# cvangysel/SERT

Hardware: AMD Instinct MI355X
Metric: training_pairs_per_sec (higher is better)
Workload: dtype f32; 1 GPU; C2 LSE: VectorSpaceLanguageModel (NCE z=10, Adam) V_w=100000 V_e=1000 d=128 window=10 batch=65536; global_batch=65536, per_gpu_batch=65536, parallelism=dp1, id_dtype=uint32, seed=0, instance_weights=1, dataset_instances=4194304, dataset_batches=64

## Files before the change

### include/sert_hip_debug.h

```cpp
#ifndef SERT_HIP_DEBUG_H
#define SERT_HIP_DEBUG_H

#include "sert_hip.h"

#ifdef __cplusplus
extern "C" {
#endif

int sert_debug_update_counts(sert_model* m, int64_t* out, int n);

int sert_debug_tail_counts(sert_model* m, int64_t* out, int n);

int sert_debug_poison_scratch(sert_model* m);

int sert_debug_row_lists(const uint32_t* allbits, int world, int rank, int64_t num_batches, int64_t bit_words,
                         int64_t rows_per_rank, int64_t vocab, int64_t batch, int32_t* serve_cnt,
                         int32_t* fetch_cnt, int32_t* serve_rows, int32_t* fetch_rows, int32_t* union_rows,
                         int32_t* ptr, int32_t* ent, int64_t capacity, int64_t* sizes);

int sert_debug_word_index_sum(const void* ids, int id_bytes, int64_t num_batches, int B, int n, int vocab, int row_groups,
                              int dense_heavy, int64_t batch, const float* src, int d, float divisor, float* grad_out,
                              int64_t* stats);

int sert_debug_ll_rank_distributions(int device, const float* P, const int64_t* offsets, int64_t num_queries, int32_t V,
                                     int32_t k, int32_t* idx_out, float* score_out, float* joint_entropy_out,
                                     float* token_entropy_out, int32_t* status_out);

int sert_bench_gemm(int device, int ta, int tb, int epi, int M, int N, int K, int splits,
                    int iters, double* avg_us);

int sert_debug_gemm(int device, int ta, int tb, int epi, int M, int N, int K, const float* A, const float* B,
                    const float* bias, float* C);

int sert_debug_gemm_splitk(int device, int M, int N, int K, int splits, const float* A, const float* B, float* out);

int sert_debug_gemm_longk(int device, int tb, int M, int N, int K, int splits, const float* A, const float* B, float* C);

enum { SERT_MEMBENCH_COPY = 0, SERT_MEMBENCH_READ = 1, SERT_MEMBENCH_GATHER = 2, SERT_MEMBENCH_OPTIMIZER = 3 };
int sert_bench_memory(int device, int kind, size_t bytes, size_t table_bytes, int row_bytes,
                      int window, size_t gap_bytes, int blocks, int iters, double* avg_us);

struct sert_reval;
int sert_debug_reval_chunks(struct sert_reval* r);

#ifdef __cplusplus
}
#endif
#endif
```

### sert_amd/_capi.py

```python
import ctypes
import os

import numpy as np

_HERE = os.path.dirname(os.path.abspath(__file__))
LIB_PATH = os.environ.get('SERT_LIB') or os.path.join(_HERE, 'libsert_hip.so')

KIND_LOGLINEAR, KIND_VECTORSPACE, KIND_VECTORSPACE_SOFTMAX = 0, 1, 2
SPLIT_TRAIN, SPLIT_VALIDATE = 0, 1
LL_STATUS_DEVICE, LL_STATUS_HOST = 0, 1
REVAL_NDCG, REVAL_MAP, REVAL_RECIP_RANK, REVAL_P5, REVAL_NUM_REL_RET, REVAL_NUM_METRICS = 0, 1, 2, 3, 4, 5

T_RW, T_RE, T_W, T_B = 0, 1, 2, 3
T_STATE0_RW, T_STATE0_RE, T_STATE0_W, T_STATE0_B = 4, 5, 6, 7
T_STATE1_RW, T_STATE1_RE, T_STATE1_W, T_STATE1_B = 8, 9, 10, 11
T_GRAD_RW, T_GRAD_RE, T_GRAD_W, T_GRAD_B = 12, 13, 14, 15
T_ACT_H, T_ACT_T, T_ACT_DA, T_ACT_DH, T_ACT_ROWLOSS = 16, 17, 18, 19, 20

COMM_ID_BYTES = 128

EXPORTS = [
    'sert_create', 'sert_destroy', 'sert_last_error', 'sert_device_info', 'sert_device_count',
    'sert_set_tensor', 'sert_get_tensor', 'sert_tensor_size', 'sert_set_step', 'sert_get_step',
    'sert_set_eval_draws', 'sert_get_eval_draws', 'sert_negatives_of_step',
    'sert_upload_dataset', 'sert_train_batch', 'sert_hint_next_batch', 'sert_train_batches',
    'sert_eval_batch', 'sert_eval_batches',
    'sert_predict_project', 'sert_predict_tokens', 'sert_ll_rank_queries', 'sert_score_topk',
    'sert_reval_create', 'sert_reval_run', 'sert_reval_destroy',
    'sert_scorer_create', 'sert_scorer_destroy', 'sert_scorer_topk', 'sert_scorer_scores',
    'sert_host_alloc', 'sert_host_free',
    'sert_comm_unique_id', 'sert_comm_init', 'sert_comm_init_host', 'sert_comm_destroy', 'sert_comm_stats',
    'sert_synchronize', 'sert_timing_enable', 'sert_timing_reset', 'sert_timing_count',
    'sert_timing_name', 'sert_timing_avg_us', 'sert_timing_launches', 'sert_bench_gemm', 'sert_debug_gemm', 'sert_debug_gemm_splitk', 'sert_debug_gemm_longk', 'sert_bench_memory', 'sert_debug_row_lists', 'sert_debug_word_index_sum',
    'sert_debug_update_counts', 'sert_debug_tail_counts', 'sert_debug_poison_scratch', 'sert_debug_ll_rank_distributions', 'sert_debug_reval_chunks',
    'sert_profile_range_push', 'sert_profile_range_pop',
]


_F32P, _I64P = ctypes.POINTER(ctypes.c_float), ctypes.POINTER(ctypes.c_int64)
ALLTOALL_FN = ctypes.CFUNCTYPE(ctypes.c_int, ctypes.c_void_p, _F32P, _I64P, _I64P, _F32P, _I64P, _I64P)


class SertConfig(ctypes.Structure):
    _fields_ = [
        ('struct_size', ctypes.c_uint32),
        ('kind', ctypes.c_int32),
        ('batch_size', ctypes.c_int32),
        ('global_batch_size', ctypes.c_int32),
        ('window_size', ctypes.c_int32),
        ('vocab_size', ctypes.c_int32),
        ('num_entities', ctypes.c_int32),
        ('word_dim', ctypes.c_int32),
        ('entity_dim', ctypes.c_int32),
        ('num_negatives', ctypes.c_int32),
        ('id_bytes', ctypes.c_int32),
        ('device', ctypes.c_int32),
        ('keep_grads', ctypes.c_int32),
        ('deterministic', ctypes.c_int32),
        ('inference_only', ctypes.c_int32),
        ('lambda_', ctypes.c_float),
        ('lr', ctypes.c_float),
        ('beta1', ctypes.c_float),
        ('beta2', ctypes.c_float),
        ('eps', ctypes.c_float),
        ('seed', ctypes.c_uint64),
    ]


class SertError(RuntimeError):
    pass


_lib = None


def load():
    global _lib
    if _lib is not None:
        return _lib
    if not os.path.exists(LIB_PATH):
        raise SertError(
            'libsert_hip.so not found at %s; build it with '
            '`python -m sert_amd._build` (hipcc --offload-arch=gfx950). '
            'There is no CPU fallback.' % LIB_PATH)
    lib = ctypes.CDLL(LIB_PATH)
    vp, i32, i64, sz = ctypes.c_void_p, ctypes.c_int32, ctypes.c_int64, ctypes.c_size_t
    fp = ctypes.c_void_p
    lib.sert_create.argtypes = [ctypes.POINTER(SertConfig), ctypes.POINTER(vp)]
    lib.sert_destroy.argtypes = [vp]
    lib.sert_last_error.restype = ctypes.c_char_p
    lib.sert_device_info.argtypes = [ctypes.c_int, ctypes.c_char_p, sz]
    lib.sert_device_count.argtypes = []
    lib.sert_set_tensor.argtypes = [vp, ctypes.c_int, fp, sz]
    lib.sert_get_tensor.argtypes = [vp, ctypes.c_int, fp, sz]
    lib.sert_tensor_size.argtypes = [vp, ctypes.c_int]
    lib.sert_tensor_size.restype = sz
    lib.sert_set_step.argtypes = [vp, i64]
    lib.sert_get_step.argtypes = [vp]
    lib.sert_get_step.restype = i64
    lib.sert_set_eval_draws.argtypes = [vp, i64]
    lib.sert_get_eval_draws.argtypes = [vp]
    lib.sert_get_eval_draws.restype = i64
    lib.sert_negatives_of_step.argtypes = [vp, i64, ctypes.c_int, vp]
    lib.sert_upload_dataset.argtypes = [vp, ctypes.c_int, fp, fp, fp, fp, fp, fp, i64]
    lib.sert_train_batch.argtypes = [vp, i64, fp, ctypes.POINTER(ctypes.c_float)]
    lib.sert_train_batches.argtypes = [vp, fp, i64, fp]
    lib.sert_hint_next_batch.argtypes = [vp, i64]
    lib.sert_eval_batch.argtypes = [vp, ctypes.c_int, i64, fp, ctypes.POINTER(ctypes.c_float)]
    lib.sert_eval_batches.argtypes = [vp, ctypes.c_int, ctypes.c_void_p, i64, ctypes.c_void_p]
    lib.sert_predict_project.argtypes = [vp, fp, i64, fp]
    lib.sert_predict_tokens.argtypes = [vp, fp, i64, fp]
    lib.sert_ll_rank_queries.argtypes = [vp, fp, fp, i64, i32, fp, fp, fp, fp, fp]
    lib.sert_reval_create.argtypes = [vp, fp, fp, i64, fp, fp, fp, fp, fp, i32, ctypes.POINTER(vp)]
    lib.sert_reval_run.argtypes = [vp, fp, fp, fp, fp]
    lib.sert_reval_destroy.argtypes = [vp]
    lib.sert_score_topk.argtypes = [ctypes.c_int, fp, i64, i32, fp, i64, i32, fp, fp]
    lib.sert_scorer_create.argtypes = [ctypes.c_int, fp, i64, i32, ctypes.POINTER(vp)]
    lib.sert_scorer_destroy.argtypes = [vp]
    lib.sert_scorer_topk.argtypes = [vp, fp, i64, i32, fp, fp]
    lib.sert_scorer_scores.argtypes = [vp, fp, i64, fp]
    lib.sert_host_alloc.argtypes = [ctypes.POINTER(vp), sz]
    lib.sert_host_free.argtypes = [vp]
    lib.sert_comm_unique_id.argtypes = [ctypes.c_char_p]
    lib.sert_comm_init.argtypes = [vp, ctypes.c_char_p, ctypes.c_int, ctypes.c_int]
    lib.sert_comm_destroy.argtypes = [vp]
    lib.sert_comm_init_host.argtypes = [vp, ctypes.c_int, ctypes.c_int, ALLTOALL_FN, vp]
    lib.sert_comm_stats.argtypes = [vp, ctypes.POINTER(ctypes.c_double), ctypes.c_int]
    lib.sert_debug_row_lists.argtypes = [fp, ctypes.c_int, ctypes.c_int, i64, i64, i64, i64, i64] + [fp] * 7 + [i64, fp]
    lib.sert_synchronize.argtypes = [vp]
    lib.sert_profile_range_push.argtypes = [ctypes.c_char_p]
    lib.sert_profile_range_pop.argtypes = []
    lib.sert_timing_enable.argtypes = [vp, ctypes.c_int]
    lib.sert_timing_reset.argtypes = [vp]
    lib.sert_timing_count.argtypes = [vp]
    lib.sert_timing_name.argtypes = [vp, ctypes.c_int]
    lib.sert_timing_name.restype = ctypes.c_char_p
    lib.sert_timing_avg_us.argtypes = [vp, ctypes.c_int]
    lib.sert_timing_avg_us.restype = ctypes.c_double
    lib.sert_timing_launches.argtypes = [vp, ctypes.c_int]
    lib.sert_timing_launches.restype = ctypes.c_double
    lib.sert_bench_gemm.argtypes = [ctypes.c_int] * 9 + [ctypes.POINTER(ctypes.c_double)]
    lib.sert_bench_memory.argtypes = [ctypes.c_int, ctypes.c_int, sz, sz, ctypes.c_int, ctypes.c_int, sz, ctypes.c_int,
                                      ctypes.c_int, ctypes.POINTER(ctypes.c_double)]
    _lib = lib
    return lib


def check(rc):
    if rc != 0:
        raise SertError(load().sert_last_error().decode('utf-8', 'replace'))


def _addr(a):
    return None if a is None else a.ctypes.data


def device_count():
    return load().sert_device_count()


def device_info(device=0):
    buf = ctypes.create_string_buffer(512)
    n = load().sert_device_info(device, buf, 512)
    if n < 0:
        raise SertError(load().sert_last_error().decode())
    return buf.value.decode()


def require_gpu():
    n = device_count()
    if n is None or n <= 0:
        raise SertError('no HIP device visible: sert_amd runs on MI355X (gfx950) only; '
                        'there is no CPU fallback.')
    return n


class Engine(object):

    def __init__(self, **cfg):
        lib = load()
        c = SertConfig()
        c.struct_size = ctypes.sizeof(SertConfig)
        for k, v in cfg.items():
            if not hasattr(c, k):
                raise TypeError('unknown sert_config field %r' % k)
            setattr(c, k, v)
        self.cfg = c
# ... 34 lines not shown
        return int(self._lib.sert_get_step(self._h))

    def set_eval_draws(self, n):
        check(self._lib.sert_set_eval_draws(self._h, int(n)))

    def get_eval_draws(self):
        return int(self._lib.sert_get_eval_draws(self._h))

    def negatives_of_step(self, position, evaluation=False):
        out = np.empty((self.cfg.batch_size, self.cfg.num_negatives), dtype=np.int64)
        check(self._lib.sert_negatives_of_step(self._h, int(position), int(bool(evaluation)), out.ctypes.data))
        return out

    def upload_dataset(self, split, x, y_int=None, csr=None, w=None):
        x = np.ascontiguousarray(x)
        n = x.shape[0]
        keep = [x]
        y_addr = ip = ix = da = None
        if y_int is not None:
            y_int = np.ascontiguousarray(y_int, dtype=np.int32)
            keep.append(y_int)
            y_addr = y_int.ctypes.data
        if csr is not None:
            indptr = np.ascontiguousarray(csr.indptr, dtype=np.int64)
            indices = np.ascontiguousarray(csr.indices, dtype=np.int32)
            data = np.ascontiguousarray(csr.data, dtype=np.float32)
            keep += [indptr, indices, data]
            ip, ix, da = indptr.ctypes.data, indices.ctypes.data, data.ctypes.data
        w_addr = None
        if w is not None:
            w = np.ascontiguousarray(w, dtype=np.float32)
            keep.append(w)
            w_addr = w.ctypes.data
        check(self._lib.sert_upload_dataset(self._h, split, x.ctypes.data if n else None,
                                            y_addr, ip, ix, da, w_addr, n))
        del keep

    def train_batch(self, batch_index, negatives=None):
        loss = ctypes.c_float()
        if negatives is not None:
            negatives = np.ascontiguousarray(negatives, dtype=np.int64)
        check(self._lib.sert_train_batch(self._h, int(batch_index), _addr(negatives),
                                         ctypes.byref(loss)))
        return np.float32(loss.value)

    def hint_next_batch(self, next_batch_index):
        check(self._lib.sert_hint_next_batch(
            self._h, -1 if next_batch_index is None else int(next_batch_index)))

    def train_batches(self, batch_indices):
        idx = np.ascontiguousarray(batch_indices, dtype=np.int64)
        out = np.empty(idx.size, dtype=np.float32)
        check(self._lib.sert_train_batches(self._h, idx.ctypes.data, idx.size, out.ctypes.data))
        return out

    def eval_batch(self, split, batch_index, negatives=None):
        loss = ctypes.c_float()
        if negatives is not None:
            negatives = np.ascontiguousarray(negatives, dtype=np.int64)
        check(self._lib.sert_eval_batch(self._h, split, int(batch_index), _addr(negatives),
                                        ctypes.byref(loss)))
        return np.float32(loss.value)

    def eval_batches(self, split, batch_indices):
        idx = np.ascontiguousarray(batch_indices, dtype=np.int64)
        out = np.empty(idx.shape[0], dtype=np.float32)
        if idx.shape[0]:
            check(self._lib.sert_eval_batches(self._h, split, idx.ctypes.data, idx.shape[0], out.ctypes.data))
        return out

    def predict_project(self, avg):
        avg = np.ascontiguousarray(avg, dtype=np.float32)
        q = avg.shape[0]
        out = np.empty((q, self.cfg.entity_dim), dtype=np.float32)
        check(self._lib.sert_predict_project(self._h, avg.ctypes.data, q, out.ctypes.data))
        return out

    def predict_tokens(self, ids):
        ids = np.ascontiguousarray(ids)
        assert ids.dtype.itemsize == self.cfg.id_bytes
        rows = ids.shape[0]
        out = np.empty((rows, self.cfg.window_size, self.cfg.num_entities), dtype=np.float32)
        check(self._lib.sert_predict_tokens(self._h, ids.ctypes.data, rows, out.ctypes.data))
        return out

    def ll_rank_queries(self, token_lists, k=None):
        tokens, offsets = _concat_queries(token_lists)
        return _ll_rank_call(self.cfg.num_entities, offsets, k, lambda kk, outs: self._lib.sert_ll_rank_queries(
            self._h, tokens.ctypes.data, offsets.ctypes.data, offsets.size - 1, kk, *outs), tokens.size)

    def comm_init(self, unique_id, rank, world):
        assert len(unique_id) == COMM_ID_BYTES
        check(self._lib.sert_comm_init(self._h, unique_id, rank, world))

    def comm_init_host(self, rank, world, alltoall):
        def trampoline(_user, send, soff, scnt, recv, roff, rcnt):
            try:
                so = np.ctypeslib.as_array(soff, shape=(world,))
                sc = np.ctypeslib.as_array(scnt, shape=(world,))
                ro = np.ctypeslib.as_array(roff, shape=(world,))
                rc = np.ctypeslib.as_array(rcnt, shape=(world,))
                ns = int((so + sc).max()) if world else 0
                nr = int((ro + rc).max()) if world else 0
                sbuf = np.ctypeslib.as_array(send, shape=(max(ns, 1),))
                rbuf = np.ctypeslib.as_array(recv, shape=(max(nr, 1),))
                alltoall(sbuf, so, sc, rbuf, ro, rc)
                return 0
            except Exception:
                import traceback
                traceback.print_exc()
                return 1
        self._host_alltoall = ALLTOALL_FN(trampoline)
        check(self._lib.sert_comm_init_host(self._h, rank, world, self._host_alltoall, None))

    def comm_stats(self):
        v = (ctypes.c_double * 8)()
        check(self._lib.sert_comm_stats(self._h, v, 8))
        return {'world': int(v[0]), 'exchange': {0: 'none', 1: 'zero1', 2: 'rows'}[int(v[1])],
                'bytes_per_step': float(v[2]), 'zero1_bytes_per_step': float(v[3]),
                'transport': {0: 'none', 1: 'rccl', 2: 'host'}[int(v[4])], 'steps': int(v[5]),
                'rows_fetched_per_batch': float(v[6]), 'rows_served_per_batch': float(v[7])}

    def synchronize(self):
        check(self._lib.sert_synchronize(self._h))

    def timing_enable(self, on=True):
        check(self._lib.sert_timing_enable(self._h, int(on)))

    def timing_launches(self):
        n = self._lib.sert_timing_count(self._h)
        return {self._lib.sert_timing_name(self._h, i).decode():
                self._lib.sert_timing_launches(self._h, i) for i in range(n)}

    def timing_reset(self):
        check(self._lib.sert_timing_reset(self._h))

    def poison_scratch(self):
        self._lib.sert_debug_poison_scratch.argtypes = [ctypes.c_void_p]
        check(self._lib.sert_debug_poison_scratch(self._h))

    def update_counts(self):
        v = (ctypes.c_int64 * 10)()
        self._lib.sert_debug_update_counts.argtypes = [ctypes.c_void_p, ctypes.POINTER(ctypes.c_int64), ctypes.c_int]
        check(self._lib.sert_debug_update_counts(self._h, v, 10))
        names = ('dense', 'lazy', 'skip_32_1', 'skip_64_1', 'skip_32_3', 'skip_64_2', 'skip_64_3', 'skip_64_4', 'skip_full', 'skip_sparse')
        return dict(zip(names, (int(x) for x in v)))

    def tail_counts(self):
        v = (ctypes.c_int64 * 2)()
        self._lib.sert_debug_tail_counts.argtypes = [ctypes.c_void_p, ctypes.POINTER(ctypes.c_int64), ctypes.c_int]
        check(self._lib.sert_debug_tail_counts(self._h, v, 2))
        return {'alone': int(v[0]), 'in_gather': int(v[1])}

    def timings(self):
        n = self._lib.sert_timing_count(self._h)
        return {self._lib.sert_timing_name(self._h, i).decode():
                self._lib.sert_timing_avg_us(self._h, i) for i in range(n)}


def comm_unique_id():
    buf = ctypes.create_string_buffer(COMM_ID_BYTES)
    check(load().sert_comm_unique_id(buf))
    return buf.raw


def _concat_queries(token_lists):
    lengths = np.fromiter((len(t) for t in token_lists), dtype=np.int64, count=len(token_lists))
    offsets = np.zeros(len(token_lists) + 1, dtype=np.int64)
    np.cumsum(lengths, out=offsets[1:])
    tokens = np.ascontiguousarray(np.concatenate([np.asarray(t, dtype=np.int64) for t in token_lists])
                                  if len(token_lists) else np.zeros(0, np.int64), dtype=np.int32)
    return tokens, offsets


def _ll_rank_call(num_entities, offsets, k, call, num_tokens):
    q = offsets.size - 1
    kk = num_entities if k is None or k >= num_entities else int(k)
    idx = np.empty((q, kk), dtype=np.int32)
    score = np.empty((q, kk), dtype=np.float32)
    joint_h = np.empty(q, dtype=np.float32)
    token_h = np.empty(num_tokens, dtype=np.float32)
    status = np.empty(q, dtype=np.int32)
    outs = [a.ctypes.data for a in (idx, score, joint_h, token_h, status)]
    check(call(-1 if k is None else int(k), outs))
    return idx, score, joint_h, token_h, status, offsets


def debug_ll_rank_distributions(distributions, offsets, k=None, device=0):
    lib = load()
    P = np.ascontiguousarray(distributions, dtype=np.float32)
    offsets = np.ascontiguousarray(offsets, dtype=np.int64)
    assert P.ndim == 2 and P.shape[0] == offsets[-1]
    lib.sert_debug_ll_rank_distributions.argtypes = [ctypes.c_int, ctypes.c_void_p, ctypes.c_void_p, ctypes.c_int64,
                                                     ctypes.c_int32, ctypes.c_int32] + [ctypes.c_void_p] * 5
    return _ll_rank_call(P.shape[1], offsets, k, lambda kk, outs: lib.sert_debug_ll_rank_distributions(
        device, P.ctypes.data, offsets.ctypes.data, offsets.size - 1, P.shape[1], kk, *outs), P.shape[0])


def score_topk(entities, projections, k, device=0):
    e = np.ascontiguousarray(entities, dtype=np.float32)
    p = np.ascontiguousarray(projections, dtype=np.float32)
    assert e.ndim == 2 and p.ndim == 2 and e.shape[1] == p.shape[1]
    q = p.shape[0]
    idx = np.empty((q, k), dtype=np.int32)
    val = np.empty((q, k), dtype=np.float32)
    check(load().sert_score_topk(device, e.ctypes.data, e.shape[0], e.shape[1], p.ctypes.data, q,
                                 k, idx.ctypes.data, val.ctypes.data))
    return idx, val


class PinnedBuffer(object):

    def __init__(self, dtype):
        self.dtype = np.dtype(dtype)
        self._ptr = ctypes.c_void_p()
        self._bytes = 0
        self._lib = load()

    def view(self, shape):
        if os.environ.get('SERT_NO_PINNED'):
            return np.empty(shape, dtype=self.dtype)
        need = int(np.prod(shape)) * self.dtype.itemsize
        if need > self._bytes:
            self.free()
            cap = max(need, 1 << 16)
            check(self._lib.sert_host_alloc(ctypes.byref(self._ptr), cap))
            self._bytes = cap
        raw = (ctypes.c_char * max(need, 1)).from_address(self._ptr.value)
        return np.frombuffer(raw, dtype=self.dtype, count=int(np.prod(shape))).reshape(shape)

    def holds(self, array):
        if not self._ptr.value or not isinstance(array, np.ndarray) or not array.flags['C_CONTIGUOUS']:
            return False
        addr = array.ctypes.data
        return self._ptr.value <= addr and addr + array.nbytes <= self._ptr.value + self._bytes

    def free(self):
        if self._ptr.value:
            self._lib.sert_host_free(self._ptr)
            self._ptr = ctypes.c_void_p()
            self._bytes = 0

    def __del__(self):
        try:
            self.free()
        except Exception:
            pass


class Scorer(object):

    MAX_HOST_SCORES = 1 << 26

    def __init__(self, entities, device=0):
        e = np.ascontiguousarray(entities, dtype=np.float32)
        assert e.ndim == 2
        self.num_entities, self.dim = e.shape
        self._lib = load()
        self._h = ctypes.c_void_p()
        check(self._lib.sert_scorer_create(device, e.ctypes.data, e.shape[0], e.shape[1],
                                           ctypes.byref(self._h)))
        self._pin_q, self._pin_idx, self._pin_val = PinnedBuffer(np.float32), PinnedBuffer(np.int32), PinnedBuffer(np.float32)

    def query_buffer(self, num_queries):
        return self._pin_q.view((num_queries, self.dim))

    def _stage(self, projections):
        p = np.asarray(projections, dtype=np.float32)
        if p.ndim == 1:
            p = p.reshape(1, -1)
        assert p.shape[1] == self.dim
        if self._pin_q.holds(p):
            return p
        staged = self._pin_q.view(p.shape)
        np.copyto(staged, p)
        return staged

    def topk(self, projections, k):
        p = self._stage(projections)
        q = p.shape[0]
        idx = self._pin_idx.view((q, k))
        val = self._pin_val.view((q, k))
        check(self._lib.sert_scorer_topk(self._h, p.ctypes.data, q, k, idx.ctypes.data,
                                         val.ctypes.data))
        return idx, val

    def scores(self, projections):
        p = np.ascontiguousarray(projections, dtype=np.float32)
        if p.ndim == 1:
            p = p.reshape(1, -1)
        assert p.shape[1] == self.dim
        out = np.empty((p.shape[0], self.num_entities), dtype=np.float32)
        check(self._lib.sert_scorer_scores(self._h, p.ctypes.data, p.shape[0], out.ctypes.data))
        return out

    def rank(self, projections, k=None):
        if k is not None and k <= min(self.num_entities, 1024):
            return self.topk(projections, k)
        p = np.asarray(projections, dtype=np.float32)
        if p.ndim == 1:
            p = p.reshape(1, -1)
        keep = self.num_entities if k is None else min(k, self.num_entities)
        step = max(1, self.MAX_HOST_SCORES // self.num_entities)
        idx = np.empty((p.shape[0], keep), dtype=np.int32)
        val = np.empty((p.shape[0], keep), dtype=np.float32)
        for lo in range(0, p.shape[0], step):
# ... 179 lines not shown
```

### sert_amd/csrc/host/api_data_train.inc

```

int sert_upload_dataset(sert_model* m, int split, const void* x, const int32_t* y_int,
                        const int64_t* csr_indptr, const int32_t* csr_indices,
                        const float* csr_data, const float* w, int64_t N) {
    if (!m) SERT_FAIL("null model");
    invalidate_speculation(m);
    m->hint_next = -1;
    if (split != SERT_SPLIT_TRAIN && split != SERT_SPLIT_VALIDATE) SERT_FAIL("bad split");
    if (N < 0) SERT_FAIL("negative instance count");
    if (N > 0 && !x) SERT_FAIL("x is null");
    if (N > 0 && !y_int && !(csr_indptr && csr_indices && csr_data)) SERT_FAIL("no labels given");
    if (is_vs(m) && N > 0 && !y_int) SERT_FAIL("vectorspace requires int labels (models.py:933-934)");
    SERT_HIP(hipSetDevice(m->cfg.device));
    if (N > 0) {
        const size_t toks = (size_t)N * m->cfg.window_size;
        const uint32_t Vw = (uint32_t)m->cfg.vocab_size;
        bool ok = true;
        SERT_ID_DISPATCH(m->cfg.id_bytes, {
            const IdT* xi = (const IdT*)x;
            uint32_t mx = 0;
            for (size_t i = 0; i < toks; ++i) mx = std::max<uint32_t>(mx, (uint32_t)xi[i]);
            ok = mx < Vw;
        });
        if (!ok) SERT_FAIL("token id >= vocab_size in x");
        const int32_t Ve = m->cfg.num_entities;
// ... 10 lines not shown
        }
    }
    DataSplit& d = m->split[split];
    free_split(d);
    d.N = N;
    if (N == 0) return 0;
    hipStream_t s = m->stream;
    const size_t xbytes = (size_t)N * m->cfg.window_size * m->cfg.id_bytes;
    SERT_HIP(hipMalloc(&d.x, xbytes));
    SERT_HIP(hipMemcpyAsync(d.x, x, xbytes, hipMemcpyHostToDevice, s));
    if (y_int) {
        d.max_labels_per_row = 1;
        SERT_TRY(dmalloc(&d.y, (size_t)N));
        SERT_HIP(hipMemcpyAsync(d.y, y_int, N * sizeof(int32_t), hipMemcpyHostToDevice, s));
    } else {
        d.nnz = csr_indptr[N];
        for (int64_t r = 0; r < N; ++r)
            d.max_labels_per_row = std::max<int64_t>(d.max_labels_per_row, csr_indptr[r + 1] - csr_indptr[r]);
        SERT_TRY(dmalloc(&d.csr_indptr, (size_t)N + 1));
        SERT_TRY(dmalloc(&d.csr_indices, (size_t)std::max<int64_t>(1, d.nnz)));
        SERT_TRY(dmalloc(&d.csr_data, (size_t)std::max<int64_t>(1, d.nnz)));
        SERT_HIP(hipMemcpyAsync(d.csr_indptr, csr_indptr, (N + 1) * sizeof(int64_t), hipMemcpyHostToDevice, s));
        if (d.nnz) {
            SERT_HIP(hipMemcpyAsync(d.csr_indices, csr_indices, d.nnz * sizeof(int32_t), hipMemcpyHostToDevice, s));
            SERT_HIP(hipMemcpyAsync(d.csr_data, csr_data, d.nnz * sizeof(float), hipMemcpyHostToDevice, s));
        }
    }
    if (split == SERT_SPLIT_TRAIN) {
        SERT_TRY(dmalloc(&d.w, (size_t)N));
        if (w) {
            SERT_HIP(hipMemcpyAsync(d.w, w, N * sizeof(float), hipMemcpyHostToDevice, s));
        } else {
            std::vector<float> ones((size_t)N, 1.0f);
            SERT_HIP(hipMemcpyAsync(d.w, ones.data(), N * sizeof(float), hipMemcpyHostToDevice, s));
            SERT_HIP(hipStreamSynchronize(s));
        }
    }
    if (split == SERT_SPLIT_TRAIN && !m->cfg.inference_only && !is_vs(m))
        SERT_TRY(dmalloc(&d.labfix, (size_t)std::max<int64_t>(1, y_int ? N : d.nnz)));
    if (split == SERT_SPLIT_TRAIN && !m->cfg.inference_only) {
        const int B = m->cfg.batch_size, n = m->cfg.window_size;
        const int64_t nb = N / B;
        WordIndex wi;
        const bool row_is_pos = !is_vs(m);
        bool vs_heavy = false;
        if (is_vs(m) && m->cfg.word_dim % 4 == 0 && m->cfg.word_dim <= 512) {
            const int d4 = m->cfg.word_dim / 4;
            const bool lpi32 = d4 <= 32 || (d4 > 64 && 64 * cdiv(d4, 64) > 32 * cdiv(d4, 32));
            const bool bundle_on = variant_knob("SERT_SEG_BUNDLE") && atoi(variant_knob("SERT_SEG_BUNDLE")) != 0;
            vs_heavy = knob("SERT_DENSE_HEAVY") ? atoi(knob("SERT_DENSE_HEAVY")) != 0 : (lpi32 && !bundle_on);
        }
        const bool dense_heavy = !variant_knob("SERT_NO_DENSE_HEAVY") && (is_vs(m) ? vs_heavy : (m->cfg.num_entities % 4 == 0));
        int row_groups = 1;
        if (is_vs(m) && m->cfg.word_dim % 4 == 0)
            if (const char* e = variant_knob("SERT_SEG_GROUPS")) row_groups = std::min(std::max(1, atoi(e)), std::max(1, B / 64));
        const bool sort_level0 = is_vs(m) && row_groups == 1 && !(variant_knob("SERT_SEG_BUNDLE") && atoi(variant_knob("SERT_SEG_BUNDLE")) != 0) &&
                                 !variant_knob("SERT_SEG_NO_SORT");
        bool ids_ok = true;
        SERT_ID_DISPATCH(m->cfg.id_bytes,
                         ids_ok = build_word_index<IdT>((const IdT*)x, nb, B, n, m->cfg.vocab_size, row_is_pos, wi,
                                                        !is_vs(m), dense_heavy, row_groups, sort_level0));
        if (!ids_ok) SERT_FAIL("token id >= vocab_size in x");
        if (!is_vs(m) && !wi.slots.empty()) {
            const size_t V = (size_t)m->cfg.num_entities;
            SERT_TRY(dmalloc(&d.idx_uwords, std::max<size_t>(1, wi.uwords.size())));
            SERT_TRY(dmalloc(&d.idx_slots, wi.slots.size()));
            SERT_HIP(hipMemcpyAsync(d.idx_uwords, wi.uwords.data(), wi.uwords.size() * sizeof(int32_t), hipMemcpyHostToDevice, s));
            SERT_HIP(hipMemcpyAsync(d.idx_slots, wi.slots.data(), wi.slots.size() * sizeof(int32_t), hipMemcpyHostToDevice, s));
            SERT_TRY(dmalloc(&d.idx_rows_div, wi.rows_div.size()));
            SERT_HIP(hipMemcpyAsync(d.idx_rows_div, wi.rows_div.data(), wi.rows_div.size() * sizeof(int32_t), hipMemcpyHostToDevice, s));
            SERT_HIP(hipStreamSynchronize(s));
            if ((size_t)wi.max_distinct > m->zu_rows) {
                (void)hipFree(m->Zu); (void)hipFree(m->dZu);
                m->Zu = nullptr; m->dZu = nullptr;
                m->zu_rows = (size_t)wi.max_distinct;
                SERT_TRY(dmalloc(&m->Zu, m->zu_rows * V));
                SERT_TRY(dmalloc(&m->dZu, m->zu_rows * V));
            }
            if ((size_t)wi.max_part_rows + 1 > m->zpart_rows) {
                (void)hipFree(m->zpart);
                m->zpart = nullptr;
                m->zpart_rows = (size_t)wi.max_part_rows + 1;
                SERT_TRY(dmalloc(&m->zpart, m->zpart_rows * V));
            }
        }
        if (!wi.rows.empty()) {
            SERT_TRY(dmalloc(&d.idx_rows, wi.rows.size()));
            SERT_HIP(hipMemcpyAsync(d.idx_rows, wi.rows.data(), wi.rows.size() * sizeof(int32_t), hipMemcpyHostToDevice, s));
            SERT_HIP(hipMalloc((void**)&d.idx_items, std::max<size_t>(1, wi.items.size()) * sizeof(SegItem)));
            SERT_HIP(hipMemcpyAsync(d.idx_items, wi.items.data(), wi.items.size() * sizeof(SegItem), hipMemcpyHostToDevice, s));
            if (!wi.heavy.empty()) {
                SERT_HIP(hipMalloc((void**)&d.idx_heavy, wi.heavy.size() * sizeof(int32_t)));
                SERT_HIP(hipMemcpyAsync(d.idx_heavy, wi.heavy.data(), wi.heavy.size() * sizeof(int32_t), hipMemcpyHostToDevice, s));
            }
            const bool bundle = variant_knob("SERT_SEG_BUNDLE") && atoi(variant_knob("SERT_SEG_BUNDLE")) != 0;
            if (!wi.bundles.empty() && bundle && is_vs(m)) {
                SERT_TRY(dmalloc(&d.idx_bundles, wi.bundles.size()));
                SERT_HIP(hipMemcpyAsync(d.idx_bundles, wi.bundles.data(), wi.bundles.size() * sizeof(int32_t), hipMemcpyHostToDevice, s));
            }
            SERT_HIP(hipStreamSynchronize(s));
        }
        if (!wi.touched_bits.empty()) {
            SERT_TRY(dmalloc(&d.idx_touched_bits, wi.touched_bits.size()));
            SERT_HIP(hipMemcpyAsync(d.idx_touched_bits, wi.touched_bits.data(), wi.touched_bits.size() * sizeof(uint32_t),
                                    hipMemcpyHostToDevice, s));
            SERT_HIP(hipStreamSynchronize(s));
            d.bit_words = wi.bit_words;
        }
        if (is_dp(m)) SERT_TRY(xr_build_lists(m, wi.touched_bits, nb, wi.bit_words));
        if (wi.any_dense) {
            SERT_HIP(hipMalloc((void**)&d.idx_dense_counts, wi.dense_counts.size()));
            SERT_HIP(hipMemcpyAsync(d.idx_dense_counts, wi.dense_counts.data(), wi.dense_counts.size(), hipMemcpyHostToDevice, s));
            std::vector<int32_t> hw((size_t)nb * kHeavyMax, 0);
            for (int64_t b = 0; b < nb; ++b)
                for (int h = 0; h < wi.batches[(size_t)b].dense_cnt; ++h) hw[(size_t)b * kHeavyMax + h] = wi.batches[(size_t)b].dense_word[h];
            if (!wi.dense_tok_slot.empty() && variant_knob("SERT_GATHER_HOT") && atoi(variant_knob("SERT_GATHER_HOT")) != 0) {
                SERT_HIP(hipMalloc((void**)&d.idx_tok_slot, wi.dense_tok_slot.size()));
                SERT_HIP(hipMemcpyAsync(d.idx_tok_slot, wi.dense_tok_slot.data(), wi.dense_tok_slot.size(), hipMemcpyHostToDevice, s));
                d.dense_cnt_of.resize((size_t)nb);
                for (int64_t b = 0; b < nb; ++b) d.dense_cnt_of[(size_t)b] = wi.batches[(size_t)b].dense_cnt;
            }
            SERT_TRY(dmalloc(&d.idx_dense_words, hw.size()));
            SERT_HIP(hipMemcpyAsync(d.idx_dense_words, hw.data(), hw.size() * sizeof(int32_t), hipMemcpyHostToDevice, s));
            SERT_HIP(hipStreamSynchronize(s));
            if (!m->hpart)
                SERT_TRY(dmalloc(&m->hpart, (size_t)std::max(cdiv(B, heavy_rows_fused(B)), cdiv(B, kHeavyRowsPerBlock)) * kHeavyMax *
                                               (size_t)(is_vs(m) ? m->cfg.word_dim : m->cfg.num_entities)));
        } else {
            for (auto& bxx : wi.batches) bxx.dense_cnt = 0;
        }
        d.idx_batches = wi.batches;
        if ((size_t)wi.max_part_rows + 1 > m->wpart_rows) {
            (void)hipFree(m->wpart);
            m->wpart_rows = (size_t)wi.max_part_rows + 1;
            SERT_TRY(dmalloc(&m->wpart, m->wpart_rows * m->cfg.word_dim));
        }
    }
    SERT_HIP(hipStreamSynchronize(s));
    return 0;
}

int sert_train_batch(sert_model* m, int64_t batch_index, const int64_t* negatives, float* loss_out) {
    refresh_gemm_choice();
    if (!m) SERT_FAIL("null model");
    SERT_HIP(hipSetDevice(m->cfg.device));
    static const bool no_spin = variant_knob("SERT_NO_SPIN") != nullptr;
    const int64_t hint = m->hint_next;
    m->hint_next = -1;
    m->lazy_next = hint;
    auto prefetch_next = [&]() -> int {
        const DataSplit& ds = m->split[SERT_SPLIT_TRAIN];
        if (will_run_ahead(m, hint)) {
            bool fused = false;
            SERT_TRY(step_forward_backward(m, ds, hint, nullptr, &fused));
            m->spec_fb_batch = hint;
            m->spec_fb_step = m->step;
            return 0;
        }
        if (hint < 0 || m->timing.enabled || m->cfg.keep_grads) return 0;
        if ((hint + 1) * (int64_t)m->cfg.batch_size > ds.N) return 0;
        if (is_vs(m) && !is_fs(m)) {
            if (m->xr_on) SERT_TRY(xr_fetch_params(m, hint));
            SERT_TRY(vs_project(m, ds, hint));
            m->projected_batch = hint;
        } else if (m->xr_on) {
            SERT_TRY(xr_fetch_params(m, hint));
        }
        return 0;
    };
    if (m->timing.enabled || no_spin) {
        SERT_TRY(train_step_async(m, batch_index, negatives, m->d_loss));
        SERT_HIP(hipMemcpyAsync(m->h_loss, m->d_loss, 3 * sizeof(float), hipMemcpyDeviceToHost, m->stream));
        SERT_HIP(hipEventRecord(m->ev_loss, m->stream));
        SERT_TRY(prefetch_next());
        SERT_HIP(hipEventSynchronize(m->ev_loss));
        timing_collect(m);
        if (loss_out) *loss_out = m->h_loss[0];
        return 0;
    }
    static const bool no_fold = variant_knob("SERT_TAIL_IN_GATHER") && atoi(variant_knob("SERT_TAIL_IN_GATHER")) == 0;
    m->tail_defer = !no_fold && !is_dp(m) && is_vs(m) && !is_fs(m) && will_run_ahead(m, hint);
    int rc = train_step_async(m, batch_index, negatives, m->h_loss_dev, true);
    m->tail_defer = false;
    if (rc == 0) rc = prefetch_next();
    flush_pending_tail(m);
    if (rc != 0) return rc;
    const unsigned want = m->loss_seq;
    volatile unsigned* flag = reinterpret_cast<volatile unsigned*>(m->h_loss + 4);
    {
        const auto t_spin0 = std::chrono::steady_clock::now();
        double next_query_ms = 50.0;
        for (unsigned spins = 1; *flag != want; ++spins) {
            if ((spins & 0xfff) != 0) continue;
            const double waited_ms = std::chrono::duration<double, std::milli>(std::chrono::steady_clock::now() - t_spin0).count();
            if (waited_ms < next_query_ms) continue;
            next_query_ms = waited_ms + 50.0;
            const hipError_t q = hipStreamQuery(m->stream);
            if (q == hipSuccess) {
                if (*flag == want) break;
                SERT_FAIL("training step completed without publishing its loss");
            }
            if (q != hipErrorNotReady) SERT_HIP(q);
        }
    }
    __atomic_thread_fence(__ATOMIC_ACQUIRE);
    if (loss_out) *loss_out = m->h_loss[0];
    return 0;
}

int sert_hint_next_batch(sert_model* m, int64_t next_batch_index) {
    if (!m) SERT_FAIL("null model");
    m->hint_next = next_batch_index;
    return 0;
}

int sert_train_batches(sert_model* m, const int64_t* batch_indices, int64_t count, float* losses_out) {
    refresh_gemm_choice();
    if (!m || !batch_indices || count < 0) SERT_FAIL("bad argument");
    m->hint_next = -1;
    SERT_HIP(hipSetDevice(m->cfg.device));
    if (count == 0) return 0;
    if (m->d_losses_cap < count) {
        (void)hipFree(m->d_losses);
        SERT_TRY(dmalloc(&m->d_losses, (size_t)count * 3));
        m->d_losses_cap = count;
    }
    static const bool report_host = variant_knob("SERT_DEBUG_HOST") != nullptr;
    const auto t_host0 = std::chrono::steady_clock::now();
    for (int64_t i = 0; i < count; ++i) {
        m->lazy_next = i + 1 < count ? batch_indices[i + 1] : -1;
        SERT_TRY(train_step_async(m, batch_indices[i], nullptr, m->d_losses + 3 * i));
        if (m->timing.enabled) {
            SERT_HIP(hipStreamSynchronize(m->stream));
            timing_collect(m);
        }
    }
    if (report_host) {
        const double us = std::chrono::duration<double, std::micro>(std::chrono::steady_clock::now() - t_host0).count();
        fprintf(stderr, "[sert] host enqueue: %.1f us/step over %lld steps\n", us / (double)count, (long long)count);
    }
    std::vector<float> tmp((size_t)count * 3);
    SERT_HIP(hipMemcpyAsync(tmp.data(), m->d_losses, count * 3 * sizeof(float), hipMemcpyDeviceToHost, m->stream));
    SERT_HIP(hipStreamSynchronize(m->stream));
    if (losses_out)
        for (int64_t i = 0; i < count; ++i) losses_out[i] = tmp[3 * i];
    return 0;
}

static int eval_step_async(sert_model* m, const DataSplit& ds, int64_t batch_index, const int64_t* negatives,
                           float* dst) {
    const int B = m->cfg.batch_size;
    SERT_TRY(settle_entity_update(m));
    SERT_TRY(ensure_rw_current(m, -1));
    if (is_fs(m)) {
        SERT_TRY(fs_forward<false>(m, ds, batch_index));
    } else if (is_vs(m)) {
        SERT_TRY(vs_negatives(m, negatives, (uint64_t)(m->eval_draws++) * 2 + 1, m->stream));
        SERT_TRY(vs_project(m, ds, batch_index));
        SERT_TRY(vs_loss<false>(m, ds, batch_index));
    } else {
        SERT_TRY(ll_forward<false>(m, ds, batch_index));
    }
    const int nb = std::min(kOptBlocks, cdiv(B, 256));
    hipLaunchKernelGGL(sum_partial, dim3(nb), dim3(256), 0, m->stream, m->rowloss, (size_t)B, m->red_loss);
    hipLaunchKernelGGL(finalize_loss, dim3(1), dim3(256), 0, m->stream, m->red_loss, nb, m->red_loss, 0,
                       1.0f / (float)B, 0.0f, dst);
    return 0;
}

static int eval_check_args(sert_model* m, int split) {
    if (!m) SERT_FAIL("null model");
    if (split != SERT_SPLIT_TRAIN && split != SERT_SPLIT_VALIDATE) SERT_FAIL("bad split");
    if (m->cfg.inference_only) SERT_FAIL("model was created inference_only");
    return 0;
}

int sert_eval_batch(sert_model* m, int split, int64_t batch_index, const int64_t* negatives, float* loss_out) {
    refresh_gemm_choice();
    SERT_TRY(eval_check_args(m, split));
    invalidate_speculation(m);
    SERT_HIP(hipSetDevice(m->cfg.device));
    SERT_TRY(ensure_full_rw(m));
    const DataSplit& ds = m->split[split];
    const int B = m->cfg.batch_size;
    if (batch_index < 0 || (batch_index + 1) * (int64_t)B > ds.N) SERT_FAIL("batch_index out of range");
    SERT_TRY(eval_step_async(m, ds, batch_index, negatives, m->d_loss));
    SERT_HIP(hipMemcpyAsync(m->h_loss, m->d_loss, 3 * sizeof(float), hipMemcpyDeviceToHost, m->stream));
    SERT_HIP(hipStreamSynchronize(m->stream));
    float v = m->h_loss[0];
    if (is_dp(m)) {
        float* tmp = m->d_loss + 3;
        SERT_HIP(hipMemcpyAsync(tmp, m->d_loss, sizeof(float), hipMemcpyDeviceToDevice, m->stream));
        if (m->host_ar) SERT_TRY(host_allreduce(m, tmp, 1, m->stream));
        else            SERT_NCCL(g_rccl.AllReduce(tmp, tmp, 1, 7, 0, m->comm, m->stream));
        SERT_HIP(hipMemcpyAsync(m->h_loss, tmp, sizeof(float), hipMemcpyDeviceToHost, m->stream));
        SERT_HIP(hipStreamSynchronize(m->stream));
        v = m->h_loss[0] / (float)m->world;
    }
    timing_collect(m);
    if (loss_out) *loss_out = v;
    return 0;
}

int sert_eval_batches(sert_model* m, int split, const int64_t* batch_indices, int64_t count, float* losses_out) {
    refresh_gemm_choice();
    SERT_TRY(eval_check_args(m, split));
    if (!batch_indices || count < 0) SERT_FAIL("bad argument");
// ... 103 lines not shown
```

### sert_amd/csrc/host/api_debug.inc

```

int sert_debug_poison_scratch(sert_model* m) {
    if (!m) SERT_FAIL("null argument");
    if (m->spec_fb_batch >= 0) SERT_FAIL("a run-ahead step is in flight (sert_hint_next_batch): its gradients live in the scratch");
    SERT_HIP(hipSetDevice(m->cfg.device));
    SERT_HIP(hipDeviceSynchronize());
    if (!m->gflat) return 0;
    std::vector<uint32_t> h(m->gflat_alloc, 0x7fc00000u);
    if (m->run_start) {
        const size_t V4 = round_up((size_t)m->cfg.num_entities, 4);
        for (size_t i = 0; i < V4; ++i) { h[m->gflat_count + i] = 0u; h[m->gflat_count + V4 + i] = 1u; }
    }
    SERT_HIP(hipMemcpy(m->gflat, h.data(), h.size() * sizeof(uint32_t), hipMemcpyHostToDevice));
    return 0;
}

int sert_debug_update_counts(sert_model* m, int64_t* out, int n) {
    if (!m || !out || n < 1 || n > 10) SERT_FAIL("bad argument");
    for (int i = 0; i < n; ++i) out[i] = m->upd_counts[i];
    return 0;
}

int sert_debug_tail_counts(sert_model* m, int64_t* out, int n) {
    if (!m || !out || n < 1 || n > 2) SERT_FAIL("bad argument");
    for (int i = 0; i < n; ++i) out[i] = m->tail_counts[i];
    return 0;
}

int sert_debug_row_lists(const uint32_t* allbits, int world, int rank, int64_t num_batches, int64_t bit_words,
                         int64_t rows_per_rank, int64_t vocab, int64_t batch, int32_t* serve_cnt, int32_t* fetch_cnt,
                         int32_t* serve_rows, int32_t* fetch_rows, int32_t* union_rows, int32_t* ptr, int32_t* ent,
                         int64_t capacity, int64_t* sizes) {
    if (!allbits || world < 1 || rank < 0 || rank >= world || batch < 0 || batch >= num_batches || !sizes)
        SERT_FAIL("bad argument");
    RowExchangeLists L;
    build_row_exchange(allbits, world, rank, num_batches, bit_words, rows_per_rank, vocab, L);
    const RowExchangeBatch& xb = L.batches[(size_t)batch];
    sizes[0] = xb.serve_total; sizes[1] = xb.fetch_total; sizes[2] = xb.nunion; sizes[3] = xb.nent; sizes[4] = L.max_xfer_rows;
    if (std::max<int64_t>(std::max(xb.serve_total, xb.fetch_total), std::max(xb.nunion + 1, xb.nent)) > capacity)
        SERT_FAIL("capacity too small");
    for (int q = 0; q < world; ++q) { serve_cnt[q] = xb.serve_cnt[(size_t)q]; fetch_cnt[q] = xb.fetch_cnt[(size_t)q]; }
    std::copy_n(L.serve_rows.begin() + xb.serve_off, xb.serve_total, serve_rows);
    std::copy_n(L.fetch_rows.begin() + xb.fetch_off, xb.fetch_total, fetch_rows);
    std::copy_n(L.union_rows.begin() + xb.union_off, xb.nunion, union_rows);
    std::copy_n(L.ptr.begin() + xb.ptr_off, xb.nunion + 1, ptr);
    std::copy_n(L.ent.begin() + xb.ent_off, xb.nent, ent);
    return 0;
}

int sert_debug_word_index_sum(const void* ids, int id_bytes, int64_t num_batches, int B, int n, int vocab, int row_groups,
                              int dense_heavy, int64_t batch, const float* src, int d, float divisor, float* grad_out,
                              int64_t* stats) {
    if (!ids || !src || !grad_out || !stats || num_batches <= 0 || B <= 0 || n <= 0 || vocab <= 0 || d <= 0 || batch < 0 ||
        batch >= num_batches || (id_bytes != 1 && id_bytes != 2 && id_bytes != 4))
        SERT_FAIL("bad argument");
    WordIndex wi;
    bool ok = true;
    SERT_ID_DISPATCH(id_bytes, ok = build_word_index<IdT>((const IdT*)ids, num_batches, B, n, vocab, false, wi,
                                                          false, (dense_heavy & 1) != 0, row_groups,
                                                          (dense_heavy & 2) != 0));
    if (!ok) SERT_FAIL("token id >= vocab");
    const BatchIndex& bx = wi.batches[(size_t)batch];
    if (((dense_heavy & 2) != 0 && row_groups <= 1 && bx.nlevels >= 1 && bx.item_cnt[0] > 0) != bx.slot_is_row) SERT_FAIL("slot_is_row not as asked");
    if (bx.slot_is_row) {
        const SegItem* l0 = wi.items.data() + bx.item_off[0];
        const int32_t* r0 = wi.rows.data() + bx.rows_off;
        for (int32_t k = 0; k < bx.item_cnt[0]; ++k) {
            if (l0[k].slot != r0[l0[k].begin]) SERT_FAIL("a level-0 item's slot is not its first row");
            if (k > 0 && l0[k].end - l0[k].begin > l0[k - 1].end - l0[k - 1].begin) SERT_FAIL("level 0 is not sorted by length");
        }
    }
    std::fill(grad_out, grad_out + (size_t)vocab * d, 0.f);
    std::vector<float> part((size_t)std::max<int64_t>(1, bx.part_rows) * d, 0.f);
    int64_t items_total = 0, finals = 0;
    for (int l = 0; l < bx.nlevels; ++l) {
        const SegItem* items = wi.items.data() + bx.item_off[l];
        const float* in = l == 0 ? src : part.data() + (size_t)bx.part_off[l - 1] * d;
        const int32_t* rows = l == 0 ? wi.rows.data() + bx.rows_off : nullptr;
        float* pout = part.data() + (size_t)bx.part_off[l] * d;
        std::vector<int32_t> order;
        if (l == 0 && bx.row_groups > 1) {
            for (int x = 0; x < 8; ++x)
                for (int k = 0; k < bx.xcd_cnt[x]; ++k) order.push_back(bx.xcd_off[x] + k);
            if ((int32_t)order.size() != bx.item_cnt[0]) SERT_FAIL("XCD lists do not cover level 0");
        } else {
            for (int32_t k = 0; k < bx.item_cnt[l]; ++k) order.push_back(k);
        }
        for (int32_t k : order) {
            const SegItem& it = items[k];
            if (it.end - it.begin > kSegChunk && l < kSegMaxLevels - 1) SERT_FAIL("an item longer than a chunk");
            ++items_total;
            float* dst = it.dst >= 0 ? grad_out + (size_t)it.dst * d : pout + (size_t)(-(it.dst + 1)) * d;
            if (it.dst >= 0) ++finals;
            for (int c = 0; c < d; ++c) {
                float a = 0.f;
                if (l == 0 && bx.slot_is_row && it.end - it.begin == 1) a += in[(size_t)it.slot * d + c];
                else
                for (int32_t e = it.begin; e < it.end; ++e) a += in[(size_t)(rows ? rows[e] : e) * d + c];
                dst[c] = it.dst >= 0 ? a / divisor : a;
            }
        }
    }
    for (int h = 0; h < bx.dense_cnt; ++h) {
        const uint8_t* dc = wi.dense_counts.data() + (size_t)(batch * B) * kHeavyMax;
        for (int c = 0; c < d; ++c) {
            float a = 0.f;
            for (int i = 0; i < B; ++i) a += (float)dc[(size_t)i * kHeavyMax + h] * src[(size_t)i * d + c];
            grad_out[(size_t)bx.dense_word[h] * d + c] = a / divisor;
        }
    }
    stats[0] = bx.nlevels; stats[1] = items_total; stats[2] = bx.part_rows; stats[3] = finals; stats[4] = bx.dense_cnt;
    stats[5] = bx.row_groups; stats[6] = bx.item_cnt[0]; stats[7] = bx.num_distinct;
    return 0;
}

int sert_profile_range_push(const char* name) {
    roctx_load();
    if (!name) SERT_FAIL("null range name");
    return g_roctx.push ? (g_roctx.push(name) < 0 ? 1 : 0) : 0;
}
int sert_profile_range_pop(void) {
    roctx_load();
    return g_roctx.pop ? (g_roctx.pop() < 0 ? 1 : 0) : 0;
}

int sert_synchronize(sert_model* m) {
    if (!m) SERT_FAIL("null model");
    SERT_HIP(hipSetDevice(m->cfg.device));
    SERT_HIP(hipStreamSynchronize(m->stream));
    SERT_HIP(hipStreamSynchronize(m->stream2));
    if (m->stream3) SERT_HIP(hipStreamSynchronize(m->stream3));
    if (m->comm_stream) SERT_HIP(hipStreamSynchronize(m->comm_stream));
    return 0;
}

int sert_timing_enable(sert_model* m, int on) {
    if (!m) SERT_FAIL("null model");
    if (on < 0 || on > 2) SERT_FAIL("timing mode: 0 = off, 1 = every group alone on one queue, 2 = in the step");
    SERT_HIP(hipSetDevice(m->cfg.device));
    if (m->instep.on && on != 2) {
        SERT_HIP(hipDeviceSynchronize());
        instep_harvest(m, true);
    }
    if (on == 2 && !m->instep.created) {
        for (int i = 0; i < InStep::kRing; ++i)
            for (int k = 0; k < 2; ++k) SERT_HIP(hipEventCreate(&m->instep.ev[i][k]));
        m->instep.created = true;
    }
    m->timing.enabled = on == 1;
    m->instep.on = on == 2;
    m->instep.cur_group = -1;
    return 0;
}
int sert_timing_reset(sert_model* m) {
    if (!m) SERT_FAIL("null model");
    for (int g = 0; g < TG_COUNT; ++g) { m->timing.total_us[g] = 0; m->timing.samples[g] = 0; m->timing.used[g] = false; }
    if (m->instep.created) {
        SERT_HIP(hipSetDevice(m->cfg.device));
        SERT_HIP(hipDeviceSynchronize());
        instep_harvest(m, true);
        for (int g = 0; g < TG_COUNT; ++g) { m->instep.total_us[g] = 0; m->instep.launches[g] = 0; }
        m->instep.steps = 0;
    }
    return 0;
}
int sert_timing_count(sert_model*) { return TG_COUNT; }
const char* sert_timing_name(sert_model*, int i) { return (i >= 0 && i < TG_COUNT) ? kTimingNames[i] : ""; }
double sert_timing_avg_us(sert_model* m, int i) {
    if (!m || i < 0 || i >= TG_COUNT) return 0.0;
    if (m->instep.steps > 0) {
        if (m->instep.head < m->instep.tail) {
            (void)hipSetDevice(m->cfg.device);
            (void)hipDeviceSynchronize();
            instep_harvest(m, true);
        }
        return m->instep.total_us[i] / (double)m->instep.steps;
    }
    if (m->timing.samples[i] == 0) return 0.0;
// ... 233 lines not shown
```

### sert_amd/csrc/host/api_model.inc

```

const char* sert_last_error(void) { return g_last_error.c_str(); }

int sert_device_count(void) {
    int n = 0;
    if (hipGetDeviceCount(&n) != hipSuccess) return -1;
    return n;
}

int sert_device_info(int device, char* buf, size_t buflen) {
    hipDeviceProp_t p;
    if (hipGetDeviceProperties(&p, device) != hipSuccess) {
        g_last_error = "hipGetDeviceProperties failed";
        return -1;
    }
    return snprintf(buf, buflen, "%s %s: %d CUs, %.0f MHz, %.1f GiB, LDS/block %zu KiB", p.name,
                    p.gcnArchName, p.multiProcessorCount, p.clockRate / 1000.0,
                    p.totalGlobalMem / (1024.0 * 1024.0 * 1024.0), p.sharedMemPerBlock / 1024);
}

static int create_resources(sert_model* m);
static int layout_gradients(sert_model* m);

static int shard_setup(sert_model* m) {
    if (m->cfg.inference_only) SERT_FAIL("model was created inference_only");
// ... 5 lines not shown
    SERT_HIP(hipStreamSynchronize(m->stream2));
    if (m->stream3) SERT_HIP(hipStreamSynchronize(m->stream3));
    float** P[4] = {&m->rw, &m->re, &m->W, &m->b};
    float** S0[4] = {&m->s0_rw, &m->s0_re, &m->s0_w, &m->s0_b};
    float** S1[4] = {&m->s1_rw, &m->s1_re, &m->s1_w, &m->s1_b};
    const size_t n[4] = {m->n_rw, m->n_re, m->n_w, m->n_b};
    for (int i = 0; i < 4; ++i) {
        if (!m->pt_big[i]) continue;
        const size_t unit = (size_t)m->world * (size_t)m->ar_chunks;
        size_t sc = round_up((n[i] + unit - 1) / unit, 64);
        if (i == 0 && m->xr_mode) {
            m->xr_rows_per_rank = (int64_t)round_up(cdiv((int64_t)m->cfg.vocab_size, m->world), 16);
            sc = (size_t)m->xr_rows_per_rank * (size_t)m->cfg.word_dim;
        }
        const size_t pad = sc * unit;
        float *np = nullptr, *ns0 = nullptr, *ns1 = nullptr;
        SERT_TRY(dzalloc(&np, pad, s));
        SERT_HIP(hipMemcpyAsync(np, *P[i], n[i] * sizeof(float), hipMemcpyDeviceToDevice, s));
        SERT_TRY(dzalloc(&ns0, sc * m->ar_chunks, s));
        SERT_TRY(dzalloc(&ns1, sc * m->ar_chunks, s));
        for (int c = 0; c < m->ar_chunks; ++c) {
            const size_t off = (size_t)c * sc * m->world + (size_t)m->rank * sc;
            if (off >= n[i]) continue;
            const size_t cnt = std::min(sc, n[i] - off);
            SERT_HIP(hipMemcpyAsync(ns0 + (size_t)c * sc, *S0[i] + off, cnt * sizeof(float), hipMemcpyDeviceToDevice, s));
            SERT_HIP(hipMemcpyAsync(ns1 + (size_t)c * sc, *S1[i] + off, cnt * sizeof(float), hipMemcpyDeviceToDevice, s));
        }
        SERT_HIP(hipStreamSynchronize(s));
        (void)hipFree(*P[i]); (void)hipFree(*S0[i]); (void)hipFree(*S1[i]);
        *P[i] = np; *S0[i] = ns0; *S1[i] = ns1;
        m->pt_pad[i] = pad;
        m->pt_sc[i] = sc;
        m->pt_sharded[i] = true;
    }
    return layout_gradients(m);
}

static int sharded_state_io(sert_model* m, int i, int k, float* host_out, const float* host_in) {
    const ParamTensor t = param_tensor(m, i);
    float* st = k == 0 ? t.s0 : t.s1;
    const size_t sc = m->pt_sc[i], pad = m->pt_pad[i], n = t.n;
    hipStream_t s = m->stream;
    if (host_in) {
        for (int c = 0; c < m->ar_chunks; ++c) {
            const size_t off = piece_off(m, i, c);
            SERT_HIP(hipMemsetAsync(st + (size_t)c * sc, 0, sc * sizeof(float), s));
            if (off < n)
                SERT_HIP(hipMemcpyAsync(st + (size_t)c * sc, host_in + off, std::min(sc, n - off) * sizeof(float),
                                        hipMemcpyHostToDevice, s));
        }
        SERT_HIP(hipStreamSynchronize(s));
        return 0;
    }
    if (m->comm_dead) SERT_FAIL("the communicator of this data-parallel model was destroyed");
    float* full = nullptr;
    SERT_TRY(dzalloc(&full, pad, s));
    for (int c = 0; c < m->ar_chunks; ++c)
        SERT_HIP(hipMemcpyAsync(full + piece_off(m, i, c), st + (size_t)c * sc, sc * sizeof(float), hipMemcpyDeviceToDevice, s));
    int rc = 0;
    if (m->host_ar) {
        for (int c = 0; c < m->ar_chunks && rc == 0; ++c) rc = host_allgather(m, full + (size_t)c * slab_elems(m, i), sc, s);
    } else {
        for (int c = 0; c < m->ar_chunks && rc == 0; ++c)
            if (g_rccl.AllGather(full + piece_off(m, i, c), full + (size_t)c * slab_elems(m, i), sc, 7, m->comm, s) != 0)
                rc = fail(__FILE__, __LINE__, "ncclAllGather failed (optimiser state)");
    }
    if (rc == 0 && hipMemcpyAsync(host_out, full, n * sizeof(float), hipMemcpyDeviceToHost, s) != hipSuccess)
        rc = fail(__FILE__, __LINE__, "copy of the gathered optimiser state failed");
    (void)hipStreamSynchronize(s);
    (void)hipFree(full);
    return rc;
}

static int create_intra_events(sert_model* m, bool device_scope) {
    hipEvent_t* evs[] = {&m->ev_join3, &m->ev_step_done, &m->ev_neg, &m->ev_opt_fork,
                         &m->ev_dense, &m->ev_small, &m->ev_re, &m->ev_fork, &m->ev_join};
    const unsigned flags = hipEventDisableTiming | (device_scope ? (unsigned)hipEventDisableSystemFence : 0u);
    for (hipEvent_t* e : evs) {
        if (*e) { SERT_HIP(hipEventDestroy(*e)); *e = nullptr; }
        SERT_HIP(hipEventCreateWithFlags(e, flags));
    }
    m->events_device_scope = device_scope;
    return 0;
}

int sert_create(const sert_config* cfg, sert_model** out) {
    if (!cfg || !out) SERT_FAIL("null argument");
    if (cfg->struct_size != sizeof(sert_config)) SERT_FAIL("sert_config size mismatch (ABI)");
    if (cfg->kind != SERT_KIND_LOGLINEAR && cfg->kind != SERT_KIND_VECTORSPACE &&
        cfg->kind != SERT_KIND_VECTORSPACE_SOFTMAX)
        SERT_FAIL("bad kind");
    if (cfg->batch_size <= 0 || cfg->window_size <= 0 || cfg->vocab_size <= 0 ||
        cfg->num_entities <= 0 || cfg->word_dim <= 0)
        SERT_FAIL("sizes must be positive");
    if (cfg->global_batch_size < cfg->batch_size) SERT_FAIL("global_batch_size < batch_size");
    if (cfg->id_bytes != 1 && cfg->id_bytes != 2 && cfg->id_bytes != 4) SERT_FAIL("id_bytes must be 1, 2 or 4");
    if (cfg->kind != SERT_KIND_LOGLINEAR) {
        if (cfg->entity_dim <= 0 || cfg->entity_dim > 512) SERT_FAIL("entity_dim must be in [1, 512]");
        if (cfg->num_negatives < 0) SERT_FAIL("num_negatives must be >= 0");
    }
    SERT_HIP(hipSetDevice(cfg->device));
    sert_model* m = new sert_model();
    m->cfg = *cfg;
    const int rc = create_resources(m);
    if (rc != 0) {
        const std::string why = g_last_error;
        sert_destroy(m);
        g_last_error = why;
        return rc;
    }
    *out = m;
    return 0;
}

static int layout_gradients(sert_model* m) {
    const bool vs = is_vs(m);
    const size_t V = m->cfg.num_entities;
    size_t off[5];
    size_t cur = 0;
    auto place = [&](int i) { off[i] = cur; cur += round_up(m->pt_pad[i], 4); };
    place(0);
    m->ar_split = cur;
    for (int i = 1; i < 4; ++i) if (m->pt_sharded[i]) place(i);
    m->rest_off = m->pt_sharded[0] ? cur : 0;
    for (int i = 1; i < 4; ++i) if (!m->pt_sharded[i]) place(i);
    off[4] = cur;
    m->gflat_count = off[4] + 4;
    m->gflat_alloc = m->gflat_count + (vs ? 2 * round_up(V, 4) : 0);
    if (m->gflat) { SERT_HIP(hipStreamSynchronize(m->stream)); (void)hipFree(m->gflat); m->gflat = nullptr; }
    SERT_TRY(dzalloc(&m->gflat, m->gflat_alloc, m->stream));
    if (vs) {
        m->run_start = (int32_t*)(m->gflat + m->gflat_count);
        m->run_end = m->run_start + round_up(V, 4);
    }
    m->g_rw = m->gflat + off[0];
    m->g_re = m->n_re ? m->gflat + off[1] : nullptr;
    m->g_w = m->gflat + off[2];
    m->g_b = m->gflat + off[3];
    m->g_loss = m->gflat + off[4];
    m->g_sq = m->g_loss + 1;
    return 0;
}

static int create_resources(sert_model* m) {
    const auto& c = m->cfg;
    SERT_HIP(hipStreamCreateWithFlags(&m->stream, hipStreamNonBlocking));
    SERT_HIP(hipStreamCreateWithFlags(&m->stream2, hipStreamNonBlocking));
    {
        const char* e3 = knob("SERT_STREAMS");
        if (e3 && atoi(e3) >= 3) SERT_HIP(hipStreamCreateWithFlags(&m->stream3, hipStreamNonBlocking));
    }
    m->proj_fused = variant_knob("SERT_PROJ_FUSED") && atoi(variant_knob("SERT_PROJ_FUSED")) != 0;
    m->lazy_skip = !(knob("SERT_LAZY_SKIP") && atoi(knob("SERT_LAZY_SKIP")) == 0);
    m->lazy_max = knob("SERT_LAZY_MAX") ? (float)atof(knob("SERT_LAZY_MAX")) : 0.5f;
    {
        int cus = 0;
        if (hipDeviceGetAttribute(&cus, hipDeviceAttributeMultiprocessorCount, m->cfg.device) != hipSuccess || cus <= 0) cus = 256;
        m->num_cus = cus;
    }
    const char* fence_env = knob("SERT_EVENT_FENCE");
    SERT_TRY(create_intra_events(m, !(fence_env && !strcmp(fence_env, "system"))));
    SERT_HIP(hipEventCreateWithFlags(&m->ev_loss, hipEventDisableTiming));
    const size_t B = c.batch_size, n = c.window_size, dw = c.word_dim, V = c.num_entities;
    const bool vs = is_vs(m);
    const size_t de = vs ? c.entity_dim : 0;
    m->n_rw = (size_t)c.vocab_size * dw;
    m->n_re = vs ? V * de : 0;
    m->n_w = vs ? dw * de : dw * V;
    m->n_b = vs ? de : V;
    hipStream_t s = m->stream;
    {
        const size_t n[4] = {m->n_rw, m->n_re, m->n_w, m->n_b};
        for (int i = 0; i < 4; ++i) {
            m->pt_pad[i] = n[i];
            m->pt_big[i] = n[i] > 0 && (i == 0 || (i < 3 && n[i] > ((size_t)1 << 22)));
            m->pt_sharded[i] = false;
        }
    }
    SERT_TRY(dzalloc(&m->rw, m->n_rw, s));  SERT_TRY(dzalloc(&m->re, m->n_re, s));
    SERT_TRY(dzalloc(&m->W, m->n_w, s));    SERT_TRY(dzalloc(&m->b, m->n_b, s));
    if (!c.inference_only) {
        SERT_TRY(dzalloc(&m->s0_rw, m->n_rw, s)); SERT_TRY(dzalloc(&m->s0_re, m->n_re, s));
        SERT_TRY(dzalloc(&m->s0_w, m->n_w, s));   SERT_TRY(dzalloc(&m->s0_b, m->n_b, s));
        SERT_TRY(dzalloc(&m->s1_rw, m->n_rw, s)); SERT_TRY(dzalloc(&m->s1_re, m->n_re, s));
        SERT_TRY(dzalloc(&m->s1_w, m->n_w, s));   SERT_TRY(dzalloc(&m->s1_b, m->n_b, s));
        static const bool no_lazy = variant_knob("SERT_NO_LAZY") != nullptr;
        if (!no_lazy && c.word_dim % 4 == 0) {
            SERT_TRY(dzalloc(&m->rw_last[0], (size_t)c.vocab_size, s));
            SERT_TRY(dzalloc(&m->rw_last[1], (size_t)c.vocab_size, s));
            m->rw_pred_stride = (unsigned)round_up((size_t)c.vocab_size, 64);
            SERT_TRY(dzalloc(&m->rw_pred, (size_t)kLazyK * m->rw_pred_stride, s));
        }
        SERT_TRY(layout_gradients(m));
        SERT_TRY(dzalloc(&m->rowloss, B, s));
        size_t part = 0;
        if (vs) {
            SERT_TRY(dzalloc(&m->H, B * dw, s));  SERT_TRY(dzalloc(&m->T, B * de, s));
            if (c.kind == SERT_KIND_VECTORSPACE && !c.inference_only) SERT_TRY(dzalloc(&m->T_alt, B * de, s));
            SERT_TRY(dzalloc(&m->DA, B * de, s)); SERT_TRY(dzalloc(&m->DH, B * dw, s));
            SERT_TRY(dzalloc(&m->neg, std::max<size_t>(4, B * c.num_negatives), s));
            SERT_TRY(dzalloc(&m->neg_alt, std::max<size_t>(4, B * c.num_negatives), s));
            SERT_TRY(dzalloc(&m->neg_stage, std::max<size_t>(4, B * c.num_negatives), s));
            part = (size_t)1024 * (dw * de + de);
            if (c.kind == SERT_KIND_VECTORSPACE_SOFTMAX) {
                {
                    const char* em = variant_knob("SERT_FS_TILE_MB");
                    const size_t cap = (size_t)(em && atoi(em) > 0 ? atoi(em) : 1700) << 20;
                    size_t tile = B;
                    if (B * V * sizeof(float) > cap) tile = std::max<size_t>(256, (cap / (V * sizeof(float))) / 256 * 256);
                    const char* er = knob("SERT_FS_TILE_ROWS");
                    if (er && atoi(er) > 0) tile = (size_t)atoi(er);
                    m->fs_tile = (int)std::min<size_t>(B, tile);
                }
                SERT_TRY(dzalloc(&m->Z, (size_t)m->fs_tile * V, s));
                SERT_TRY(dzalloc(&m->DH2, B * de, s));
                const size_t tiles = (size_t)cdiv(de, GN) * cdiv(V, GM);
                const size_t sp = std::max<size_t>(1, cdiv(1024, tiles)) + 1;
                part = std::max(part, sp * V * de);
            }
            const size_t total = B * (c.num_negatives + 1);
            {
                const bool force_sort = knob("SERT_EGRAD_SORT") && atoi(knob("SERT_EGRAD_SORT")) != 0;
                m->egrad_force_sort = force_sort;
                m->egrad_ranges = variant_knob("SERT_EGRAD_RANGES") && atoi(variant_knob("SERT_EGRAD_RANGES")) != 0;
                const size_t c1 = c.num_negatives + 1;
                if (!force_sort && c.kind == SERT_KIND_VECTORSPACE && V <= 2048 && de % 4 == 0 && de <= 128 &&
                    total < ((size_t)1 << 27) && c1 <= (size_t)kElSubPairs) {
                    m->eg_er_shift = 4;
                    m->eg_ranges = cdiv(V, 16);
                    m->eg_sub_rows = (int)std::min<size_t>(256, kElSubPairs / c1);
                    while (m->eg_sub_rows > 32 && (size_t)B < (size_t)64 * m->eg_sub_rows) m->eg_sub_rows /= 2;
                    m->eg_num_sub = cdiv(B, m->eg_sub_rows);
                    m->eg_subs_per_group = (int)std::max<size_t>(1, (((size_t)2 << 20) / (de * sizeof(float))) / m->eg_sub_rows);
                    static const int want_groups = variant_knob("SERT_EG_GROUPS") ? std::max(1, atoi(variant_knob("SERT_EG_GROUPS"))) : 16;
                    m->eg_subs_per_group = std::max(1, std::min(m->eg_subs_per_group, m->eg_num_sub / want_groups));
                    m->eg_groups = cdiv(m->eg_num_sub, m->eg_subs_per_group);
                }
                if (m->eg_groups > 0) {
                    SERT_TRY(dzalloc(&m->epart, (size_t)m->eg_groups * V * de, s));
                    SERT_TRY(dzalloc(&m->eg_entries, total, s));
                    SERT_TRY(dzalloc(&m->eg_offs, (size_t)m->eg_num_sub * (m->eg_ranges + 1), s));
                }
            }
            SERT_TRY(dzalloc(&m->cand, total, s));        SERT_TRY(dzalloc(&m->cand_sorted, total + 1, s));
            SERT_TRY(dzalloc(&m->cand_early, total, s));
            SERT_TRY(dzalloc(&m->pair_sorted, total, s));
            SERT_TRY(dzalloc(&m->coef, total, s));
            const size_t chunks = (total + kEChunk - 1) / kEChunk;
            SERT_TRY(dzalloc(&m->ehead, chunks * de, s)); SERT_TRY(dzalloc(&m->etail, chunks * de, s));
            m->sort_bits = 1;
            while ((1ll << m->sort_bits) < (long long)V) ++m->sort_bits;
            const size_t tiles = (total + kSortTile - 1) / kSortTile;
            SERT_TRY(dzalloc(&m->sort_hist, (size_t)kSortMaxBins * tiles, s));
            SERT_TRY(dzalloc(&m->sort_bin_total, (size_t)kSortMaxBins, s));
            if (m->sort_bits > kSortMaxBits) {
                SERT_TRY(dzalloc(&m->sort_k_tmp, total, s));
                SERT_TRY(dzalloc(&m->sort_v_tmp, total, s));
            }
        } else {
#define SERT_LL_ATTR(NT)                                                                                  \
    SERT_HIP(hipFuncSetAttribute((const void*)ll_fused_row<true, NT>, hipFuncAttributeMaxDynamicSharedMemorySize, 150 * 1024)); \
    SERT_HIP(hipFuncSetAttribute((const void*)ll_fused_row<false, NT>, hipFuncAttributeMaxDynamicSharedMemorySize, 150 * 1024))
            SERT_LL_ATTR(512);
            SERT_HIP(hipFuncSetAttribute((const void*)ll_row_from_table<512>, hipFuncAttributeMaxDynamicSharedMemorySize, 150 * 1024));
#undef SERT_LL_ATTR
            SERT_TRY(dzalloc(&m->G, B * n * dw, s));  SERT_TRY(dzalloc(&m->Z, B * n * V, s));
            SERT_TRY(dzalloc(&m->J, B * V, s));       SERT_TRY(dzalloc(&m->DG, B * n * dw, s));
            const size_t nseg = cdiv(V, kLlSeg);
            SERT_TRY(dzalloc(&m->ll_tokstat, B * n * nseg, s)); SERT_TRY(dzalloc(&m->ll_lse, B * n, s));
            SERT_TRY(dzalloc(&m->ll_jstat, B * nseg, s));       SERT_TRY(dzalloc(&m->ll_rowinfo, B, s));
            SERT_TRY(dzalloc(&m->ll_rpart, B * n * nseg, s));   SERT_TRY(dzalloc(&m->ll_r, B * n, s));
            SERT_TRY(dzalloc(&m->ll_rsum, B * n, s));
            const size_t tiles = (size_t)cdiv(V, GN) * cdiv(dw, GM);
            const size_t splits = std::max<size_t>(1, cdiv(1024, tiles)) + 1;
            part = splits * (dw * V + V);
        }
        m->part_count = part;
        SERT_TRY(dzalloc(&m->part, part, s));
        SERT_TRY(dzalloc(&m->red_loss, std::max<size_t>((size_t)kOptBlocks, (B + 15) / 16), s));
        SERT_TRY(dzalloc(&m->red_sq, (size_t)8 * kOptBlocks, s));
        SERT_TRY(dzalloc(&m->re_sq, (size_t)4 * kOptBlocks, s));
        SERT_TRY(dzalloc(&m->sq_scratch, (size_t)8 * kOptBlocks, s));
        SERT_TRY(dzalloc(&m->d_loss, (size_t)4, s));
        if (vs) {
            SERT_TRY(dzalloc(&m->tail_blk, (size_t)4 * (cdiv((int64_t)(m->n_w + m->n_b), 64) + 1), s));
        }
    }
    SERT_HIP(hipHostMalloc((void**)&m->h_loss, 8 * sizeof(float), hipHostMallocMapped | hipHostMallocCoherent));
    memset(m->h_loss, 0, 8 * sizeof(float));
    SERT_HIP(hipHostGetDevicePointer((void**)&m->h_loss_dev, m->h_loss, 0));
    {
        const char* e = knob("SERT_STREAMS");
        const int v = e ? atoi(e) : 0;
        if (v >= 1 && v <= 3) m->nstreams = v;
    }
    for (int g = 0; g < TG_COUNT; ++g)
        for (int k = 0; k < 2; ++k) SERT_HIP(hipEventCreate(&m->timing.ev[g][k]));
    m->timing.created = true;
    SERT_HIP(hipStreamSynchronize(s));
    return 0;
}

static void free_split(DataSplit& d) {
    (void)hipFree(d.x); (void)hipFree(d.y); (void)hipFree(d.csr_indptr);
    (void)hipFree(d.csr_indices); (void)hipFree(d.csr_data); (void)hipFree(d.w); (void)hipFree(d.labfix);
    (void)hipFree(d.idx_rows); (void)hipFree(d.idx_items);
// ... 149 lines not shown
```

### sert_amd/csrc/host/lazy_segsum.inc

```

static void optimizer_args(const sert_model* m, int64_t t, AdamArgs* aa, AdadeltaArgs* da);
static LazyArgs lazy_args(sert_model* m, int64_t t_prev, int update) {
    LazyArgs lz;
    lz.last_in = m->rw_stale ? m->rw_last[m->rw_last_cur] : nullptr;
    lz.last_out = m->rw_last[m->rw_last_cur ^ 1];
    lz.next_bits = nullptr;
    lz.t_prev = (int)t_prev;
    lz.write_all = 1;
    lz.update = update;
    for (int k = 0; k <= kLazyK; ++k) {
        AdamArgs aa; AdadeltaArgs da;
        optimizer_args(m, std::max<int64_t>(1, t_prev + 1 - k), &aa, &da);
        lz.a_of[k] = aa.a_t;
    }
    return lz;
}
static int ensure_rw_current(sert_model* m, int64_t batch, int64_t t_applied) {
    if (!m->rw_stale) return 0;
    if (batch >= 0 && batch == m->rw_ready_batch) return 0;
    if (t_applied < 0) t_applied = m->step;
    AdamArgs aa; AdadeltaArgs da;
    optimizer_args(m, std::max<int64_t>(1, t_applied), &aa, &da);
    const LazyArgs lz = lazy_args(m, t_applied, 0);
    const int64_t max_nb = m->n_rw >= ((size_t)1 << 24) ? 2 * kOptBlocks : kOptBlocks;
    const int nb = (int)std::min<int64_t>(max_nb, cdiv(cdiv(m->n_rw, 4), 256));
    if (is_vs(m))
        hipLaunchKernelGGL((dense_update_lazy<true>), dim3(nb), dim3(256), 0, m->stream, m->rw, (const float*)m->g_rw, m->s0_rw, m->s1_rw,
                           m->n_rw, aa, da, m->sq_scratch, (const uint32_t*)nullptr, (unsigned)m->cfg.word_dim, lz);
    else
        hipLaunchKernelGGL((dense_update_lazy<false>), dim3(nb), dim3(256), 0, m->stream, m->rw, (const float*)m->g_rw, m->s0_rw, m->s1_rw,
                           m->n_rw, aa, da, m->sq_scratch, (const uint32_t*)nullptr, (unsigned)m->cfg.word_dim, lz);
    m->rw_last_cur ^= 1;
    m->rw_stale = false;
    m->rw_ready_batch = -1;
    return 0;
}

static int settle_entity_update(sert_model* m) {
    if (m->re_pending) {
        SERT_HIP(hipStreamWaitEvent(m->stream, m->ev_re, 0));
        m->re_pending = false;
    }
    return 0;
}

struct TensorRef {
    float* ptr;
    size_t count;
};
static TensorRef tensor_ref(sert_model* m, int which) {
    const size_t B = m->cfg.batch_size;
    switch (which) {
        case SERT_T_RW: return {m->rw, m->n_rw};
        case SERT_T_RE: return {m->re, m->n_re};
        case SERT_T_W: return {m->W, m->n_w};
        case SERT_T_B: return {m->b, m->n_b};
        case SERT_T_STATE0_RW: return {m->s0_rw, m->n_rw};
        case SERT_T_STATE0_RE: return {m->s0_re, m->n_re};
        case SERT_T_STATE0_W: return {m->s0_w, m->n_w};
        case SERT_T_STATE0_B: return {m->s0_b, m->n_b};
        case SERT_T_STATE1_RW: return {m->s1_rw, m->n_rw};
        case SERT_T_STATE1_RE: return {m->s1_re, m->n_re};
        case SERT_T_STATE1_W: return {m->s1_w, m->n_w};
        case SERT_T_STATE1_B: return {m->s1_b, m->n_b};
        case SERT_T_GRAD_RW: return {m->g_rw, m->n_rw};
        case SERT_T_GRAD_RE: return {m->g_re, m->n_re};
        case SERT_T_GRAD_W: return {m->g_w, m->n_w};
        case SERT_T_GRAD_B: return {m->g_b, m->n_b};
        case SERT_T_ACT_H: return {m->H, m->H ? B * m->cfg.word_dim : 0};
        case SERT_T_ACT_T: return {m->T, m->T ? B * m->cfg.entity_dim : 0};
        case SERT_T_ACT_DA: return {m->DA, m->DA ? B * m->cfg.entity_dim : 0};
        case SERT_T_ACT_DH: return {m->DH, m->DH ? B * m->cfg.word_dim : 0};
        case SERT_T_ACT_ROWLOSS: return {m->rowloss, B};
        default: return {nullptr, 0};
    }
}

#define SERT_ID_DISPATCH(id_bytes, ...)                                  \
    do {                                                                 \
        if ((id_bytes) == 1) { typedef uint8_t IdT; __VA_ARGS__; }       \
        else if ((id_bytes) == 2) { typedef uint16_t IdT; __VA_ARGS__; } \
        else { typedef uint32_t IdT; __VA_ARGS__; }                      \
    } while (0)


static int word_grad_segsum(sert_model* m, const DataSplit& ds, int64_t batch_index,
                            const float* src, float divisor) {
    const int d = m->cfg.word_dim;
    if ((size_t)batch_index >= ds.idx_batches.size()) SERT_FAIL("batch has no word index");
    const BatchIndex& bx = ds.idx_batches[(size_t)batch_index];
    unsigned char* touched = nullptr;
    static const bool no_fused_upper = variant_knob("SERT_SEG_NO_FUSED_UPPER") != nullptr;
    const bool fused_upper = !no_fused_upper && bx.fused_upper_ok && ds.idx_heavy && d % 4 == 0 &&
                             bx.nlevels == 3 && bx.item_cnt[1] > 0;
    bool heavy_fused = false, heavy_combined = false;
    PlusJob hjob = PlusJob();
    if (bx.dense_cnt > 0 && is_vs(m) && d % 4 == 0) {
        const int B = m->cfg.batch_size, d4 = d / 4;
        static const bool no_fuse = variant_knob("SERT_HEAVY_NO_FUSE") != nullptr;
        const bool lpi32 = d4 <= 32 || (d4 > 64 && 64 * cdiv(d4, 64) > 32 * cdiv(d4, 32));
        const bool bundled = bx.bundle_cnt > 0 && ds.idx_bundles;
        heavy_fused = !no_fuse && lpi32 && bx.nlevels >= 1 && bx.item_cnt[0] > 0 && bx.row_groups == 1 && !bundled;
        const uint4* cnt = ds.idx_dense_counts + (size_t)batch_index * B;
        if (heavy_fused) {
            hjob.kind = 1; hjob.rpb = heavy_rows_fused(B); hjob.extra = cdiv(B, hjob.rpb); hjob.src = src; hjob.cnt16 = cnt; hjob.part = m->hpart;
            hjob.words = (const int32_t*)ds.idx_dense_words + (size_t)batch_index * kHeavyMax;
            hjob.nheavy = bx.dense_cnt; hjob.nblocks = hjob.extra; hjob.B = B;
        } else {
        const int nblk = cdiv(B, kHeavyRowsPerBlock);
        const size_t lds = (size_t)4 * kHeavyMax * 32 * sizeof(float4);
        hipLaunchKernelGGL(segsum_heavy, dim3(nblk * cdiv(d4, 32)), dim3(1024), lds, m->stream, src, cnt, B, d, m->hpart);
        hipLaunchKernelGGL(segsum_heavy_combine, dim3(bx.dense_cnt, cdiv(d4, 32)), dim3(256), 0, m->stream,
                           (const float*)m->hpart, nblk, d, (const int32_t*)ds.idx_dense_words + (size_t)batch_index * kHeavyMax,
                           bx.dense_cnt, m->g_rw, divisor);
        }
    }
    auto heavy_combine_job = [&]() { PlusJob j = hjob; j.kind = 2; j.extra = bx.dense_cnt; j.src = m->hpart; return j; };
    for (int l = 0; l < bx.nlevels; ++l) {
        const int nitems = bx.item_cnt[l];
        if (nitems == 0) continue;
        if (fused_upper && l == 1) {
            const int nb_normal = cdiv(nitems, 32);
            hipLaunchKernelGGL(segsum_upper_fused, dim3(nb_normal + bx.heavy_cnt, cdiv(d / 4, 32)), dim3(1024), 0, m->stream,
                               m->wpart + (size_t)bx.part_off[0] * d, ds.idx_items + bx.item_off[1], nitems, nb_normal,
                               ds.idx_heavy + bx.heavy_off, m->g_rw, d, divisor);
            break;
        }
        const float* in = (l == 0) ? src : m->wpart + (size_t)bx.part_off[l - 1] * d;
        const int32_t* rows = (l == 0) ? ds.idx_rows + bx.rows_off : nullptr;
        const int4* items = ds.idx_items + bx.item_off[l];
        float* pout = m->wpart + (size_t)bx.part_off[l] * d;
        if (heavy_fused && l <= 1) {
            PlusJob j = l == 0 ? hjob : heavy_combine_job();
            j.slot_is_row = (l == 0 && bx.slot_is_row) ? 1 : 0;
            hipLaunchKernelGGL(segsum_rows_plus, dim3(j.extra + cdiv(nitems, 8), cdiv(d / 4, 32)), dim3(256), 0, m->stream, in, rows, items,
                               nitems, m->g_rw, pout, d, divisor, j);
            if (l == 1) heavy_combined = true;
            continue;
        }
#ifdef SERT_VARIANTS
        if (l == 0 && d % 4 == 0 && bx.bundle_cnt > 0 && ds.idx_bundles && bx.row_groups == 1) {
            hipLaunchKernelGGL(segsum_rows_bundled, dim3(cdiv(bx.bundle_cnt, 8), cdiv(d / 4, 32)), dim3(256), 0, m->stream, in, rows,
                               items, (const int32_t*)ds.idx_bundles + bx.bundle_off, (int)bx.bundle_cnt, m->g_rw, pout, d, divisor);
            continue;
        }
#endif
        if (d % 4 == 0) {
            const int ch = d / 4;
            const bool seg32y = ch > 64 && ch * (64 * cdiv(ch, 64)) > ch * (32 * cdiv(ch, 32));
            XcdLists xl = XcdLists();
            xl.slot_is_row = (l == 0 && bx.slot_is_row) ? 1 : 0;
            int longest = 0;
            if (l == 0 && bx.row_groups > 1) {
                xl.on = 1;
                for (int x = 0; x < 8; ++x) { xl.off[x] = bx.xcd_off[x]; xl.cnt[x] = bx.xcd_cnt[x]; longest = std::max(longest, bx.xcd_cnt[x]); }
            }
            const int ipb = (d / 4 <= 32 || seg32y) ? 8 : 4;
            const int gx = xl.on ? 8 * cdiv(longest, ipb) : cdiv(nitems, ipb);
            if (d / 4 <= 32)
                hipLaunchKernelGGL((segsum_rows<32>), dim3(gx), dim3(256), 0, m->stream,
                                   in, rows, items, nitems, m->g_rw, pout, d, divisor, touched, 1, nullptr, nullptr, DenseSlots(), xl);
            else if (seg32y)
                hipLaunchKernelGGL((segsum_rows<32>), dim3(gx, cdiv(d / 4, 32)), dim3(256), 0, m->stream,
                                   in, rows, items, nitems, m->g_rw, pout, d, divisor, touched, 1, nullptr, nullptr, DenseSlots(), xl);
            else
                hipLaunchKernelGGL((segsum_rows<64>), dim3(gx, cdiv(d / 4, 64)), dim3(256), 0, m->stream,
                                   in, rows, items, nitems, m->g_rw, pout, d, divisor, touched, 1, nullptr, nullptr, DenseSlots(), xl);
        } else {
            hipLaunchKernelGGL((segsum_rows_scalar<false>), dim3(cdiv(nitems, 4), cdiv(d, 64)), dim3(256), 0, m->stream, in,
                               rows, items, nitems, m->g_rw, pout, d, divisor, touched);
        }
    }
    if (heavy_fused && !heavy_combined) {
        const PlusJob j = heavy_combine_job();
        hipLaunchKernelGGL(segsum_rows_plus, dim3(j.extra, cdiv(d / 4, 32)), dim3(256), 0, m->stream, (const float*)nullptr,
                           (const int32_t*)nullptr, (const int4*)nullptr, 0, m->g_rw, (float*)nullptr, d, divisor, j);
    }
    return 0;
}

static int dzu_from_dj(sert_model* m, const DataSplit& ds, int64_t batch_index) {
    const int V = m->cfg.num_entities;
    const BatchIndex& bx = ds.idx_batches[(size_t)batch_index];
    static const bool split_odd = variant_knob("SERT_LL_DZU_SPLIT") != nullptr;
    const bool fused_odd = V % 4 != 0 && !split_odd;
    for (int l = 0; l < bx.nlevels && !fused_odd; ++l) {
        const int nitems = bx.item_cnt[l];
        if (nitems == 0) continue;
        const int32_t* rows = (l == 0) ? ds.idx_rows + bx.rows_off : nullptr;
        const int4* items = ds.idx_items + bx.item_off[l];
        const float* in = (l == 0) ? m->ll_r : m->ll_rpart + (size_t)bx.part_off[l - 1];
        float* pout = m->ll_rpart + (size_t)bx.part_off[l];
        hipLaunchKernelGGL(segsum_scalar_wave, dim3(cdiv(nitems, 4)), dim3(256), 0, m->stream, in, rows, items, nitems,
                           m->ll_rsum, pout);
    }
    static const bool ll_no_fuse = variant_knob("SERT_HEAVY_NO_FUSE") != nullptr;
    const bool ll_heavy_fused = !ll_no_fuse && V % 4 == 0 && bx.dense_cnt > 0 && bx.nlevels >= 1 && bx.item_cnt[0] > 0;
    bool ll_heavy_combined = false;
    PlusJobLL ll_job = PlusJobLL();
    if (ll_heavy_fused) {
        const int B = m->cfg.batch_size;
        ll_job.j.kind = 1; ll_job.j.rpb = heavy_rows_fused(B); ll_job.j.extra = cdiv(B, ll_job.j.rpb); ll_job.j.src = m->J;
        ll_job.j.cnt16 = ds.idx_dense_counts + (size_t)batch_index * B; ll_job.j.part = m->hpart;
        ll_job.j.nheavy = bx.dense_cnt; ll_job.j.nblocks = ll_job.j.extra; ll_job.j.B = B;
        ll_job.logp = m->Zu; ll_job.rsum = m->ll_rsum;
    }
    for (int l = 0; l < bx.nlevels; ++l) {
        const int nitems = bx.item_cnt[l];
        if (nitems == 0) continue;
        const int32_t* rows = (l == 0) ? ds.idx_rows_div + bx.rows_off : nullptr;
        const int4* items = ds.idx_items + bx.item_off[l];
        const float* in = (l == 0) ? m->J : m->zpart + (size_t)bx.part_off[l - 1] * V;
        float* pout = m->zpart + (size_t)bx.part_off[l] * V;
        if (V % 4 == 0 && bx.dense_cnt > 0) {
            DenseSlots dsl;
            dsl.n = bx.dense_cnt;
            for (int h = 0; h < kHeavyMax; ++h) dsl.slot[h] = h < bx.dense_cnt ? bx.dense_slot[h] : -2;
            if (ll_heavy_fused && l <= 1) {
                PlusJobLL j = ll_job;
                j.dense = dsl;
                if (l == 1) { j.j.kind = 2; j.j.extra = bx.dense_cnt; j.j.src = m->hpart; ll_heavy_combined = true; }
                hipLaunchKernelGGL(segsum_rows_plus_ll, dim3(j.j.extra + cdiv(nitems, 4), cdiv(V / 4, 64)), dim3(256), 0, m->stream, in,
                                   rows, items, nitems, m->dZu, pout, V, dsl, j);
                continue;
            }
            hipLaunchKernelGGL((segsum_rows<64, true, true, true>), dim3(cdiv(nitems, 4), cdiv(V / 4, 64)), dim3(256), 0,
                               m->stream, in, rows, items, nitems, m->dZu, pout, V, 1.0f,
                               (unsigned char*)nullptr, 1, (const float*)m->Zu,
                               (const float*)m->ll_rsum, dsl);
        } else if (V % 4 == 0) {
            hipLaunchKernelGGL((segsum_rows<64, true, true>), dim3(cdiv(nitems, 4), cdiv(V / 4, 64)), dim3(256), 0,
                               m->stream, in, rows, items, nitems, m->dZu, pout, V, 1.0f,
                               (unsigned char*)nullptr, 1, (const float*)m->Zu,
                               (const float*)m->ll_rsum);
        } else if (fused_odd) {
            hipLaunchKernelGGL((segsum_rows_scalar<true, true>), dim3(cdiv(nitems, 4), cdiv(V, 64)), dim3(256), 0, m->stream, in,
                               rows, items, nitems, m->dZu, pout, V, 1.0f, (unsigned char*)nullptr, 1, (const float*)m->Zu,
                               (const float*)((l == 0) ? m->ll_r : m->ll_rpart + (size_t)bx.part_off[l - 1]),
                               (l == 0) ? (const int32_t*)(ds.idx_rows + bx.rows_off) : (const int32_t*)nullptr,
                               m->ll_rsum, m->ll_rpart + (size_t)bx.part_off[l]);
        } else {
            hipLaunchKernelGGL((segsum_rows_scalar<true>), dim3(cdiv(nitems, 4), cdiv(V, 64)), dim3(256), 0, m->stream, in,
                               rows, items, nitems, m->dZu, pout, V, 1.0f, (unsigned char*)nullptr, 1);
        }
    }
    if (ll_heavy_fused && !ll_heavy_combined) {
        PlusJobLL j = ll_job;
        j.dense.n = bx.dense_cnt;
        for (int h = 0; h < kHeavyMax; ++h) j.dense.slot[h] = h < bx.dense_cnt ? bx.dense_slot[h] : -2;
        j.j.kind = 2; j.j.extra = bx.dense_cnt; j.j.src = m->hpart;
        hipLaunchKernelGGL(segsum_rows_plus_ll, dim3(j.j.extra, cdiv(V / 4, 64)), dim3(256), 0, m->stream, (const float*)nullptr,
                           (const int32_t*)nullptr, (const int4*)nullptr, 0, m->dZu, (float*)nullptr, V, j.dense, j);
    }
    if (V % 4 == 0 && bx.dense_cnt > 0 && !ll_heavy_fused) {
        const int B = m->cfg.batch_size, d4 = V / 4;
        const int nblk = cdiv(B, kHeavyRowsPerBlock);
        const uint4* cnt = ds.idx_dense_counts + (size_t)batch_index * B;
        static const bool attr_set = hipFuncSetAttribute((const void*)segsum_heavy_wide, hipFuncAttributeMaxDynamicSharedMemorySize,
                                                         2 * kHeavyMax * 128 * (int)sizeof(float4)) == hipSuccess;
        if (!attr_set) SERT_FAIL("cannot reserve the LDS of segsum_heavy_wide");
        hipLaunchKernelGGL(segsum_heavy_wide, dim3(nblk * cdiv(d4, 128)), dim3(512), (size_t)2 * kHeavyMax * 128 * sizeof(float4), m->stream,
                           (const float*)m->J, cnt, B, V, m->hpart);
        DenseSlots dsl;
        dsl.n = bx.dense_cnt;
        for (int h = 0; h < kHeavyMax; ++h) dsl.slot[h] = h < bx.dense_cnt ? bx.dense_slot[h] : -2;
        hipLaunchKernelGGL(segsum_heavy_combine_ll, dim3(bx.dense_cnt, cdiv(d4, 32)), dim3(256), 0, m->stream,
                           (const float*)m->hpart, nblk, V, dsl, m->dZu, (const float*)m->Zu, (const float*)m->ll_rsum);
    }
    if (V % 4 != 0 && !fused_odd)
        hipLaunchKernelGGL(ll_dzu_combine, dim3(grid_for((int64_t)m->ll_U * V)), dim3(256), 0, m->stream, m->dZu,
                           (const float*)m->Zu, (const float*)m->ll_rsum, (int64_t)m->ll_U, V);
    return 0;
}

static int entity_key_sort(sert_model* m, int total, hipStream_t st, const int32_t* keys = nullptr) {
    const int tiles = cdiv(total, kSortTile);
    const int bits = m->sort_bits;
    const int passes = cdiv(bits, kSortMaxBits);
    const int width = cdiv(bits, passes);
    const int32_t* kin = keys ? keys : m->cand;
    const int32_t* vin = nullptr;
    for (int p = 0; p < passes; ++p) {
        const int shift = p * width;
        const int nb = std::min(width, bits - shift);
        const bool to_final = ((passes - 1 - p) % 2) == 0;
        int32_t* kout = to_final ? m->cand_sorted : m->sort_k_tmp;
        int32_t* vout = to_final ? m->pair_sorted : m->sort_v_tmp;
        hipLaunchKernelGGL(csort_hist, dim3(tiles), dim3(256), 0, st, kin, total, shift, 1 << nb,
                           tiles, m->sort_hist, p == 0 ? m->run_start : (int32_t*)nullptr,
                           p == 0 ? (int)(2 * round_up(m->cfg.num_entities, 4)) : 0);
        hipLaunchKernelGGL(csort_scan_bins, dim3(cdiv(1 << nb, 4)), dim3(256), 0, st,
                           m->sort_hist, 1 << nb, tiles, m->sort_bin_total);
        hipLaunchKernelGGL(csort_scatter, dim3(tiles), dim3(256), 0, st, kin, vin, kout, vout,
                           total, shift, nb, tiles, m->sort_hist, m->sort_bin_total);
        kin = kout;
        vin = vout;
    }
    return 0;
}

template <bool TA, bool TB>
static int gemm_long_k(sert_model* m, hipStream_t s, const float* A, const float* Bm, float* C, int M,
                       int N, int K, int lda, int ldb, const int32_t* rowmap = nullptr, float* mapped_C = nullptr,
                       bool* mapped = nullptr) {
    if (mapped) *mapped = false;
    const int tiles = cdiv(M, GM) * cdiv(N, GN);
    int splits = 1;
    if (tiles < 512 && K >= 4096) splits = std::min(cdiv(1024, tiles), K / 1024);
    else if (tiles < 256 && K >= 512) splits = std::min(cdiv(1024, tiles), K / 128);
    if (!TA && K >= 4096 && gemm_x3_enabled()) {
        const int t3 = cdiv(M, N <= 128 ? 128 : 256) * cdiv(N, N <= 128 ? 128 : 320);
        const int s3 = std::max(1, std::min(cdiv(512, t3), K / 1024));
        if (s3 > 1 && x3_shape_ok(false, TB, A, Bm, M, N, K, lda, ldb, s3)) splits = s3;
    }
    if (splits <= 1) {
        launch_gemm<TA, TB, EPI_STORE>(s, A, Bm, C, nullptr, M, N, K, lda, ldb, N, 1, 0, 0, nullptr, nullptr, 0, rowmap, mapped_C,
                                       mapped);
        return 0;
    }
    const int kper = (int)round_up(cdiv(K, splits), GK);
    splits = cdiv(K, kper);
    const size_t mn = (size_t)M * N;
    if (mn * splits > m->skbuf_count) {
        SERT_HIP(hipStreamSynchronize(s));
        if (m->skbuf) (void)hipFree(m->skbuf);
        m->skbuf = nullptr;
        m->skbuf_count = mn * splits;
        SERT_TRY(dmalloc(&m->skbuf, m->skbuf_count));
    }
// ... 8 lines not shown
```

### sert_amd/csrc/host/optimizer_and_loss.inc

```

static int reduce_rowloss(sert_model* m, hipStream_t st) {
    const int B = m->cfg.batch_size;
    int nb = std::min(kOptBlocks, cdiv(B, 256));
    m->loss_from_rows = false;
    if (is_vs(m) && !is_fs(m) && m->nce_loss_partials > 0) nb = m->nce_loss_partials;
    else if (!is_dp(m) && B <= 8192) {
        m->loss_from_rows = true;
        nb = B;
    } else hipLaunchKernelGGL(sum_partial, dim3(nb), dim3(256), 0, st, m->rowloss, (size_t)B, m->red_loss);
    if (is_dp(m))
        hipLaunchKernelGGL(partials_to_scalar, dim3(1), dim3(256), 0, st, m->red_loss, nb, m->g_loss);
    m->n_loss_partials = nb;
    return 0;
}

static void launch_stream_opt(sert_model* m, hipStream_t st, float* p, float* g, float* s0, float* s1, size_t count,
                              int nb, const AdamArgs& aa, const AdadeltaArgs& da, float* sq,
                              const uint32_t* bits, unsigned row_len, float* sq_new = nullptr) {
    const bool keep = m->cfg.keep_grads != 0;
    const int rows_mode = kRowsAll;
    if (is_vs(m)) {
        if (keep) hipLaunchKernelGGL((adam_l2<true>), dim3(nb), dim3(256), 0, st, p, g, s0, s1, count, aa, sq, bits, row_len, rows_mode, sq_new);
        else      hipLaunchKernelGGL((adam_l2<false>), dim3(nb), dim3(256), 0, st, p, g, s0, s1, count, aa, sq, bits, row_len, rows_mode, sq_new);
    } else {
        if (keep) hipLaunchKernelGGL((adadelta_l2<true>), dim3(nb), dim3(256), 0, st, p, g, s0, s1, count, da, sq, bits, row_len, rows_mode);
        else      hipLaunchKernelGGL((adadelta_l2<false>), dim3(nb), dim3(256), 0, st, p, g, s0, s1, count, da, sq, bits, row_len, rows_mode);
    }
}

static void optimizer_args(const sert_model* m, int64_t t, AdamArgs* aa, AdadeltaArgs* da) {
    const auto& c = m->cfg;
    const float l2k = c.lambda_ > 0.f ? c.lambda_ / (float)c.global_batch_size : 0.f;
    *aa = AdamArgs{l2k, 0.f, c.beta1, c.beta2, c.eps};
    *da = AdadeltaArgs{l2k, c.lr, c.beta1, c.eps};
    if (is_vs(m)) {
        const float tf = (float)t;
        aa->a_t = c.lr * sqrtf(1.0f - powf(c.beta2, tf)) / (1.0f - powf(c.beta1, tf));
    }
}

static int launch_lazy_word_update(sert_model* m, const ParamTensor& t, const uint32_t* tf, const uint32_t* next_bits, const int nb,
                                   const AdamArgs& aa, const AdadeltaArgs& da, float* sq) {
    const auto& c = m->cfg;
    LazyArgs lz = lazy_args(m, m->step - 1, 1);
    int nb_skip = 0;
    lz.next_bits = next_bits;
    lz.write_all = (next_bits == nullptr || m->step % kLazyK == 0) ? 1 : 0;
    const unsigned d4 = (unsigned)c.word_dim / 4;
    if (m->lazy_skip && m->rw_pred && d4 <= 256) {
        const int64_t u = m->step;
        const bool sparse = next_bits && m->rw_pred_ok && u < m->rw_pred_T;
        lz.write_all = sparse ? 0 : 1;
        if (!sparse) m->rw_pred_T = u + kLazyK;
        SkipArgs sk;
        sk.pred = m->rw_pred;
        sk.stride = m->rw_pred_stride;
        sk.npred = next_bits ? (int)(m->rw_pred_T - 1 - u) : 0;
        for (int j = 0; j < kLazyK; ++j) {
            AdamArgs a2; AdadeltaArgs d2;
            optimizer_args(m, u + 1 + j, &a2, &d2);
            sk.a_fut[j] = a2.a_t;
        }
        m->rw_pred_ok = next_bits != nullptr;
        const unsigned nrows = (unsigned)c.vocab_size;
        static const int skip_blocks_knob = variant_knob("SERT_SKIP_BLOCKS") ? atoi(variant_knob("SERT_SKIP_BLOCKS")) : 0;
        const int nb_dense = nb;
        const int nb = std::max(1, std::min<int>(skip_blocks_knob > 0 ? std::min(skip_blocks_knob, 4 * kOptBlocks) : nb_dense,
                                                 (int)cdiv(nrows, 8u)));
        nb_skip = nb;
#define SERT_SKIP_LAUNCH(ADAM, LPR, CPL)                                                                                   \
    hipLaunchKernelGGL((dense_update_skip<ADAM, LPR, CPL>), dim3(nb), dim3(256), 0, m->stream, t.p, (const float*)t.g, t.s0, \
           t.s1, nrows, aa, da, sq, tf, (unsigned)c.word_dim, lz, sk)
        static const int skip_32x3_knob = variant_knob("SERT_SKIP_32X3") ? atoi(variant_knob("SERT_SKIP_32X3")) : -1;
        const bool skip_32x3 = skip_32x3_knob >= 0 ? skip_32x3_knob != 0 : t.n < ((size_t)1 << 26);
#define SERT_SKIP_SHAPE(ADAM)                                                                   \
    do {                                                                                        \
        if (d4 <= 32) { SERT_SKIP_LAUNCH(ADAM, 32, 1); ++m->upd_counts[2]; }                    \
        else if (d4 <= 64) { SERT_SKIP_LAUNCH(ADAM, 64, 1); ++m->upd_counts[3]; }               \
        else if (d4 <= 96 && skip_32x3) { SERT_SKIP_LAUNCH(ADAM, 32, 3); ++m->upd_counts[4]; }  \
        else if (d4 <= 128) { SERT_SKIP_LAUNCH(ADAM, 64, 2); ++m->upd_counts[5]; }              \
        else if (d4 <= 192) { SERT_SKIP_LAUNCH(ADAM, 64, 3); ++m->upd_counts[6]; }              \
        else { SERT_SKIP_LAUNCH(ADAM, 64, 4); ++m->upd_counts[7]; }                             \
        ++m->upd_counts[sparse ? 9 : 8];                                                        \
    } while (0)
        if (is_vs(m)) SERT_SKIP_SHAPE(true);
        else SERT_SKIP_SHAPE(false);
#undef SERT_SKIP_SHAPE
#undef SERT_SKIP_LAUNCH
    } else {
    ++m->upd_counts[1];
    if (is_vs(m))
        hipLaunchKernelGGL((dense_update_lazy<true>), dim3(nb), dim3(256), 0, m->stream, t.p, (const float*)t.g, t.s0, t.s1, t.n,
                           aa, da, sq, tf, (unsigned)c.word_dim, lz);
    else
        hipLaunchKernelGGL((dense_update_lazy<false>), dim3(nb), dim3(256), 0, m->stream, t.p, (const float*)t.g, t.s0, t.s1, t.n,
                           aa, da, sq, tf, (unsigned)c.word_dim, lz);
    }
    m->rw_last_cur ^= 1;
    m->rw_stale = !lz.write_all;
    m->rw_ready_batch = lz.write_all ? -1 : m->lazy_next;
    return nb_skip > 0 ? nb_skip : nb;
}

static int optimizer_and_loss(sert_model* m, float* loss_dst, bool publish = false,
                              const uint32_t* bits = nullptr, const uint32_t* next_bits = nullptr) {
    const int n_loss_partials = m->n_loss_partials;
    const auto& c = m->cfg;
    const float l2k = c.lambda_ > 0.f ? c.lambda_ / (float)c.global_batch_size : 0.f;
    m->step += 1;
    AdamArgs aa; AdadeltaArgs da;
    optimizer_args(m, m->step, &aa, &da);
    int n_sq = 0;
    const bool exchanged = m->comm && !m->timing.enabled;
    const bool side_small = !is_dp(m) && !m->timing.enabled && m->nstreams >= 2 && (is_vs(m) || m->ll_dw_side);
    hipStream_t ss = side_small ? m->stream2 : m->stream;
    if (side_small && m->lazy_join && fork_late_mode(m)) {
    } else if (side_small && m->lazy_join) {
        SERT_HIP(hipStreamWaitEvent(ss, m->ev_dense, 0));
    } else if (side_small) {
        SERT_HIP(hipEventRecord(m->ev_opt_fork, m->stream));
        SERT_HIP(hipStreamWaitEvent(ss, m->ev_opt_fork, 0));
    }
    bool any_ag = false;
    const int tail_splits = m->tail_splits;
    m->tail_splits = 0;
    static const bool no_defer = knob("SERT_RE_DEFER") && atoi(knob("SERT_RE_DEFER")) == 0;
    const bool defer_re = !no_defer && m->side_heavy && side_small && tail_splits > 0 && m->pt_big[1] && is_vs(m) && !c.keep_grads;
    const bool defer_small = !no_defer && !defer_re && side_small && tail_splits > 0 && !m->pt_big[1] && is_vs(m) && !is_fs(m) &&
                             !c.keep_grads && m->lazy_join && fork_late_mode(m) && m->n_re > 0;
    const int re_cur = (int)(m->step & 1), re_nxt = re_cur ^ 1;
    const size_t re_cap = (size_t)2 * kOptBlocks;
    bool small_needs_join = !defer_small;
    int re_sq_lo = 0, re_nb = 0;
    for (int i = 0; i < 4; ++i) {
        if (!m->pt_big[i]) continue;
        const ParamTensor t = param_tensor(m, i);
        if (t.n == 0) continue;
        const int tg = i == 0 ? TG_OPT_WORD : TG_OPTIMIZER;
        if (i == 1 && defer_re) {
            const int64_t max_nb = t.n >= ((size_t)1 << 24) ? 2 * kOptBlocks : kOptBlocks;
            re_nb = (int)std::min<int64_t>(max_nb, cdiv(cdiv(t.n, 4), 256));
            re_sq_lo = n_sq;
            n_sq += re_nb;
            continue;
        }
        if (!(is_dp(m) && m->pt_sharded[i])) {
            ScopedTimer tm(m, tg);
            const int64_t max_nb = t.n >= ((size_t)1 << 24) ? 2 * kOptBlocks : kOptBlocks;
            const int nb = (int)std::min<int64_t>(max_nb, cdiv(cdiv(t.n, 4), 256));
            const uint32_t* tf = (i == 0 && m->use_touched) ? bits : nullptr;
            const float lazy_max = (next_bits && m->lazy_skip) ? m->lazy_max : std::min(m->lazy_max, 0.35f);
            static const bool lazy_small = variant_knob("SERT_LAZY_SMALL_TABLES") != nullptr;
            if (i == 0 && tf && m->rw_last[0] && !c.keep_grads && c.word_dim % 4 == 0 &&
                m->cur_touched_frac <= lazy_max && (t.n >= ((size_t)1 << 22) || lazy_small)) {
                n_sq += launch_lazy_word_update(m, t, tf, next_bits, nb, aa, da, m->red_sq + n_sq);
                continue;
            }
            if (i == 0) m->rw_pred_ok = false;
            if (i == 0) ++m->upd_counts[0];
            if (i == 0) SERT_TRY(ensure_rw_current(m, -1, m->step - 1));
            const bool on_side = side_small && ((i == 1 && m->side_heavy) || (i >= 2 && m->ll_dw_side));
            launch_stream_opt(m, on_side ? ss : m->stream, t.p, t.g, t.s0, t.s1, t.n, nb, aa, da,
                              m->red_sq + n_sq, tf,
                              i == 0 ? (unsigned)c.word_dim : 1u);
            n_sq += nb;
            continue;
        }
        const size_t sc = m->pt_sc[i];
        const int nch = m->ar_chunks;
        const bool by_rows = (i == 0) && m->xr_on;
        {
            ScopedTimer tm(m, tg);
            for (int ch = 0; ch < nch; ++ch) {
                if (exchanged && m->rs_issued[i]) SERT_HIP(hipStreamWaitEvent(m->stream, m->ev_rs_done[i][by_rows ? 0 : ch], 0));
                const size_t off = piece_off(m, i, ch);
                const int nb = (int)std::min<int64_t>(std::max(1, kOptBlocks / nch), cdiv(cdiv(sc, 4), 256));
                const uint32_t* ub = by_rows ? m->xr_ubits + (size_t)m->xr_batch * (size_t)m->xr->owned_bit_words : nullptr;
                launch_stream_opt(m, m->stream, t.p + off, t.g + off, t.s0 + (size_t)ch * sc, t.s1 + (size_t)ch * sc, sc,
                                  nb, aa, da, m->sq_scratch, ub, by_rows ? (unsigned)c.word_dim : 1u);
                if (by_rows) {
                    if (m->ev_word_updated) SERT_HIP(hipEventRecord(m->ev_word_updated, m->stream));
                    m->rw_full = false;
                    m->xr_fetched_batch = -1;
                    continue;
                }
                m->comm_bytes_moved += 8.0 * (double)sc * (double)(m->world - 1);
                if (exchanged) {
                    SERT_HIP(hipEventRecord(m->ev_opt_done[i][ch], m->stream));
                    SERT_HIP(hipStreamWaitEvent(m->comm_stream, m->ev_opt_done[i][ch], 0));
                    SERT_NCCL(g_rccl.AllGather(t.p + off, t.p + (size_t)ch * slab_elems(m, i), sc,  7,
                                               m->comm, m->comm_stream));
                    any_ag = true;
                }
            }
        }
        m->rs_issued[i] = false;
        if (by_rows) {
        } else if (m->host_ar) {
            ScopedTimer tm(m, TG_ALLGATHER);
            for (int ch = 0; ch < nch; ++ch) SERT_TRY(host_allgather(m, t.p + (size_t)ch * slab_elems(m, i), sc, m->stream));
        } else if (m->comm && m->timing.enabled) {
            ScopedTimer tm(m, TG_ALLGATHER);
            for (int ch = 0; ch < nch; ++ch)
                SERT_NCCL(g_rccl.AllGather(t.p + piece_off(m, i, ch), t.p + (size_t)ch * slab_elems(m, i), sc, 7, m->comm,
                                           m->stream));
        }
    }
    if (exchanged) SERT_HIP(hipStreamWaitEvent(m->stream, m->ev_ar_done, 0));
    if (side_small && egrad_writes_every_row(m) && c.kind == SERT_KIND_VECTORSPACE && !is_fs(m) && c.num_negatives > 0 && !c.keep_grads &&
        m->neg_alt_step != m->step) {
        const int64_t count = (int64_t)c.batch_size * c.num_negatives;
        hipLaunchKernelGGL(vs_sample_negatives, dim3(grid_for((count + 3) / 4)), dim3(256), 0, ss, m->neg_alt, count,
                           (int64_t)m->rank * count, (uint32_t)c.num_entities, c.seed, (uint64_t)m->step * 2);
        m->neg_alt_step = m->step;
    }
    const bool split_small = side_small && m->lazy_join && fork_late_mode(m);
    auto small_tensors = [&](hipStream_t ss, unsigned mask) {
        ScopedTimer t(m, TG_OPTIMIZER);
        SmallTensors st;
        int k = 0, blocks = 0;
        for (int i = 1; i < 4; ++i) {
            const ParamTensor t2 = param_tensor(m, i);
            if (m->pt_big[i] || t2.n == 0 || !((mask >> i) & 1u)) continue;
            st.p[k] = t2.p; st.g[k] = t2.g; st.s0[k] = t2.s0; st.s1[k] = t2.s1; st.count[k] = t2.n;
            const bool parts = (i == 1) && m->re_in_parts;
            st.gparts[k] = parts ? m->epart : nullptr;
            st.ngroups[k] = parts ? m->eg_groups : 0;
            st.gstride[k] = parts ? (unsigned long long)m->n_re : 0ull;
            st.l2k[k] = t2.l2 ? l2k : 0.f;
            st.first_block[k] = blocks;
            blocks += (int)std::min<int64_t>(512, cdiv(t2.n, 256));
            ++k;
        }
        for (int i = k; i < 3; ++i) { st.p[i] = st.g[i] = st.s0[i] = st.s1[i] = nullptr; st.count[i] = 0; st.l2k[i] = 0.f; st.gparts[i] = nullptr; st.ngroups[i] = 0; st.gstride[i] = 0; }
        for (int i = k; i <= 3; ++i) st.first_block[i] = blocks;
        float* sq = m->red_sq + n_sq;
        float* sq_new = nullptr;
        if (defer_small && mask == 0x2u && blocks > 0) {
            re_sq_lo = n_sq;
            re_nb = blocks;
            sq_new = m->re_sq + re_nxt * re_cap;
            if (m->re_sq_for[re_cur] != m->step) {
                hipLaunchKernelGGL(sumsq_like_small, dim3(blocks), dim3(256), 0, ss, (const float*)m->re, m->n_re, l2k,
                                   m->re_sq + re_cur * re_cap);
                m->re_sq_for[re_cur] = m->step;
                small_needs_join = true;
            }
        }
        if (blocks > 0) {
            const bool keep = c.keep_grads != 0;
            if (is_vs(m) && sq_new) {
                hipLaunchKernelGGL((optimizer_small<true, false>), dim3(blocks), dim3(256), 0, ss, st, aa, da, sq, sq_new);
            } else if (is_vs(m)) {
                if (keep) hipLaunchKernelGGL((optimizer_small<true, true>), dim3(blocks), dim3(256), 0, ss, st, aa, da, sq);
                else      hipLaunchKernelGGL((optimizer_small<true, false>), dim3(blocks), dim3(256), 0, ss, st, aa, da, sq);
            } else {
                if (keep) hipLaunchKernelGGL((optimizer_small<false, true>), dim3(blocks), dim3(256), 0, ss, st, aa, da, sq);
                else      hipLaunchKernelGGL((optimizer_small<false, false>), dim3(blocks), dim3(256), 0, ss, st, aa, da, sq);
            }
        }
        n_sq += blocks;
    };
    if (tail_splits > 0) {
        small_tensors(ss, 0x2u);
    } else if (split_small) {
        small_tensors(m->stream, 0xCu);
        small_tensors(ss, 0x2u);
    } else {
        small_tensors(ss, 0xEu);
    }
    if (defer_re && m->re_sq_for[re_cur] != m->step) {
        hipLaunchKernelGGL(sumsq_like_adam, dim3(re_nb), dim3(256), 0, ss, (const float*)m->re, m->n_re, m->re_sq + re_cur * re_cap);
        m->re_sq_for[re_cur] = m->step;
    }
    if (side_small && small_needs_join) {
        SERT_HIP(hipEventRecord(m->ev_small, ss));
        SERT_HIP(hipStreamWaitEvent(m->stream, m->ev_small, 0));
    }
    if (defer_small && re_nb > 0) {
        m->re_sq_for[re_nxt] = m->step + 1;
        SERT_HIP(hipEventRecord(m->ev_re, ss));
        m->re_pending = true;
    }
    if (defer_re) {
        const ParamTensor t = param_tensor(m, 1);
        launch_stream_opt(m, ss, t.p, t.g, t.s0, t.s1, t.n, re_nb, aa, da, m->red_sq + re_sq_lo, nullptr, 1u,
                          m->re_sq + re_nxt * re_cap);
        m->re_sq_for[re_nxt] = m->step + 1;
        SERT_HIP(hipEventRecord(m->ev_re, ss));
        m->re_pending = true;
    }
    {
        ScopedTimer t(m, TG_FINALIZE);
        const float inv_batch = 1.0f / (float)c.global_batch_size;
        const float reg_scale = c.lambda_ > 0.f ? c.lambda_ / (2.0f * (float)c.global_batch_size) : 0.f;
        const float* lp = is_dp(m) ? m->g_loss : (m->loss_from_rows ? m->rowloss : m->red_loss);
        const int nl = is_dp(m) ? 1 : n_loss_partials;
        unsigned* flag = publish ? reinterpret_cast<unsigned*>(loss_dst + 4) : nullptr;
        if (tail_splits > 0) {
            if (m->dw_side_first) SERT_HIP(hipStreamWaitEvent(m->stream, m->ev_dense, 0));
            TailArgs ta;
            ta.part = m->part; ta.splits = tail_splits; ta.stride = m->tail_stride;
            ta.W = m->W; ta.b = m->b; ta.s0_w = m->s0_w; ta.s1_w = m->s1_w; ta.s0_b = m->s0_b; ta.s1_b = m->s1_b;
            ta.g_w = m->g_w; ta.g_b = m->g_b;
            ta.n_w = (unsigned)m->n_w; ta.n_b = (unsigned)m->n_b;
            ta.aa = aa;
            ta.loss_partials = lp; ta.n_loss = nl;
            ta.sq_partials = m->red_sq; ta.n_sq = n_sq;
            const bool alt = defer_re || (defer_small && re_nb > 0);
            ta.sq_alt = alt ? m->re_sq + re_cur * re_cap : nullptr;
// ... 168 lines not shown
```

### sert_amd/csrc/kernels_opt.h

```cpp
#pragma once
#include "common.h"

namespace sert {

#ifndef SERT_OPT_BLOCKS
#define SERT_OPT_BLOCKS 2048
#endif
constexpr int kOptBlocks = SERT_OPT_BLOCKS;

struct AdamArgs {
    float l2k;
    float a_t;
    float b1, b2, eps;
};

__device__ __forceinline__ float sq_acc(float acc, float x) { return __builtin_fmaf(x, x, acc); }

__device__ __forceinline__ void adam_elem(float& p, float& g, float& m, float& v, const AdamArgs& a,
                                          float omb1, float omb2, float& ss, float& ss_new) {
#pragma clang fp contract(off)
    const float pv = p;
    const float l2 = a.l2k * pv;
    const float gv = g + l2;
    ss = sq_acc(ss, pv);
// ... 144 lines not shown
                                                   float* __restrict__ delta, size_t count,
                                                   AdadeltaArgs a,
                                                   float* __restrict__ sumsq_partial,
                                                   const uint32_t* __restrict__ bits = nullptr,
                                                   unsigned row_len = 1, int rows_mode = kRowsAll) {
    __shared__ float red[4];
    float ss = 0.f;
    const float omr = 1.0f - a.rho;
    const size_t n4 = count >> 2;
    float4* p4 = reinterpret_cast<float4*>(p);
    float4* g4 = reinterpret_cast<float4*>(g);
    float4* a4 = reinterpret_cast<float4*>(accu);
    float4* d4 = reinterpret_cast<float4*>(delta);
    const size_t per = (n4 + gridDim.x - 1) / gridDim.x;
    const size_t lo = (size_t)blockIdx.x * per;
    const size_t hi = lo + per < n4 ? lo + per : n4;
    for (size_t i = lo + threadIdx.x; i < hi; i += blockDim.x) {
        const bool hit = !bits || row_bit(bits, ((unsigned)i << 2) / row_len);
        if (rows_mode != kRowsAll && hit != (rows_mode == kRowsTouched)) continue;
        float4 pp = p4[i], aa = a4[i], dd = d4[i];
        float4 gg = make_float4(0.f, 0.f, 0.f, 0.f);
        if (hit) gg = g4[i];
        adadelta_elem(pp.x, gg.x, aa.x, dd.x, a, omr, ss);
        adadelta_elem(pp.y, gg.y, aa.y, dd.y, a, omr, ss);
        adadelta_elem(pp.z, gg.z, aa.z, dd.z, a, omr, ss);
        adadelta_elem(pp.w, gg.w, aa.w, dd.w, a, omr, ss);
        p4[i] = pp; a4[i] = aa; d4[i] = dd;
        if (STORE_G) g4[i] = gg;
    }
    if (blockIdx.x == 0 && !bits) {
        const size_t i = (n4 << 2) + threadIdx.x;
        if (i < count) {
            float pp = p[i], gg = g[i], aa = accu[i], dd = delta[i];
            adadelta_elem(pp, gg, aa, dd, a, omr, ss);
            p[i] = pp; accu[i] = aa; delta[i] = dd;
            if (STORE_G) g[i] = gg;
        }
    }
    const float tot = block_sum_256(ss, red);
    if (threadIdx.x == 0) sumsq_partial[blockIdx.x] = tot;
}

#ifndef SERT_LAZY_K
#define SERT_LAZY_K 4
#endif
constexpr int kLazyK = SERT_LAZY_K;
struct LazyArgs {
    const int32_t* last_in;
    int32_t* last_out;
    const uint32_t* next_bits;
    int t_prev;
    int write_all;
    int update;
    float a_of[kLazyK + 1];
};
__device__ __forceinline__ float lazy_step_size(const LazyArgs& lz, int k) {
    float r = lz.a_of[1];
#pragma unroll
    for (int j = 2; j <= kLazyK; ++j) r = (k == j) ? lz.a_of[j] : r;
    return r;
}

template <bool ADAM>
__global__ __launch_bounds__(256) void dense_update_lazy(float* __restrict__ p, const float* __restrict__ g,
                                                         float* __restrict__ s0, float* __restrict__ s1, size_t count,
                                                         AdamArgs a, AdadeltaArgs da, float* __restrict__ sumsq_partial,
                                                         const uint32_t* __restrict__ bits, unsigned row_len, const LazyArgs lz) {
    __shared__ float red[4];
    float ss = 0.f;
    const float omb1 = 1.0f - a.b1, omb2 = 1.0f - a.b2, omr = 1.0f - da.rho;
    const size_t n4 = count >> 2;
    float4* p4 = reinterpret_cast<float4*>(p);
    const float4* g4 = reinterpret_cast<const float4*>(g);
    typedef float nt_f4 __attribute__((ext_vector_type(4)));
    const size_t per = (n4 + gridDim.x - 1) / gridDim.x;
    const size_t lo = (size_t)blockIdx.x * per;
    const size_t hi = lo + per < n4 ? lo + per : n4;
    for (size_t i = lo + threadIdx.x; i < hi; i += blockDim.x) {
        const unsigned e0 = (unsigned)i << 2;
        const unsigned row = e0 / row_len;
        const bool first_piece = e0 - row * row_len == 0u;
        const int last = lz.last_in ? lz.last_in[row] : lz.t_prev;
        const int lag = lz.t_prev - last;
        const bool hit = lz.update && row_bit(bits, row);
        const bool need = lz.update ? (hit || lz.write_all || (lz.next_bits && row_bit(lz.next_bits, row))) : (lag > 0);
        if (first_piece) lz.last_out[row] = lz.update ? (need ? lz.t_prev + 1 : last) : lz.t_prev;
        if (!lz.update && lag == 0) continue;
        float4 pp = p4[i];
        const nt_f4 mr = __builtin_nontemporal_load(reinterpret_cast<const nt_f4*>(s0) + i);
        const nt_f4 vr = __builtin_nontemporal_load(reinterpret_cast<const nt_f4*>(s1) + i);
        float4 mm = make_float4(mr.x, mr.y, mr.z, mr.w), vv = make_float4(vr.x, vr.y, vr.z, vr.w);
        for (int k = lag; k >= 1; --k) {
            float z0 = 0.f, z1 = 0.f, z2 = 0.f, z3 = 0.f, sd = 0.f, sn = 0.f;
            if (ADAM) {
                AdamArgs ak = a;
                ak.a_t = lazy_step_size(lz, k);
                adam_elem(pp.x, z0, mm.x, vv.x, ak, omb1, omb2, sd, sn);
                adam_elem(pp.y, z1, mm.y, vv.y, ak, omb1, omb2, sd, sn);
                adam_elem(pp.z, z2, mm.z, vv.z, ak, omb1, omb2, sd, sn);
                adam_elem(pp.w, z3, mm.w, vv.w, ak, omb1, omb2, sd, sn);
            } else {
                adadelta_elem(pp.x, z0, mm.x, vv.x, da, omr, sd);
                adadelta_elem(pp.y, z1, mm.y, vv.y, da, omr, sd);
                adadelta_elem(pp.z, z2, mm.z, vv.z, da, omr, sd);
                adadelta_elem(pp.w, z3, mm.w, vv.w, da, omr, sd);
            }
        }
        if (lz.update && !need) {
            ss = sq_acc(ss, pp.x);
            ss = sq_acc(ss, pp.y);
            ss = sq_acc(ss, pp.z);
            ss = sq_acc(ss, pp.w);
            continue;
        }
        if (lz.update) {
            float4 gg = make_float4(0.f, 0.f, 0.f, 0.f);
            if (hit) gg = g4[i];
            float sn = 0.f;
            if (ADAM) {
                AdamArgs ak = a;
                ak.a_t = lz.a_of[0];
                adam_elem(pp.x, gg.x, mm.x, vv.x, ak, omb1, omb2, ss, sn);
                adam_elem(pp.y, gg.y, mm.y, vv.y, ak, omb1, omb2, ss, sn);
                adam_elem(pp.z, gg.z, mm.z, vv.z, ak, omb1, omb2, ss, sn);
                adam_elem(pp.w, gg.w, mm.w, vv.w, ak, omb1, omb2, ss, sn);
            } else {
                adadelta_elem(pp.x, gg.x, mm.x, vv.x, da, omr, ss);
                adadelta_elem(pp.y, gg.y, mm.y, vv.y, da, omr, ss);
                adadelta_elem(pp.z, gg.z, mm.z, vv.z, da, omr, ss);
                adadelta_elem(pp.w, gg.w, mm.w, vv.w, da, omr, ss);
            }
        }
        p4[i] = pp;
        { nt_f4 t; t.x = mm.x; t.y = mm.y; t.z = mm.z; t.w = mm.w; __builtin_nontemporal_store(t, reinterpret_cast<nt_f4*>(s0) + i); }
        { nt_f4 t; t.x = vv.x; t.y = vv.y; t.z = vv.z; t.w = vv.w; __builtin_nontemporal_store(t, reinterpret_cast<nt_f4*>(s1) + i); }
    }
    if (lz.update) {
        const float tot = block_sum_256(ss, red);
        if (threadIdx.x == 0) sumsq_partial[blockIdx.x] = tot;
    }
}

#ifndef SERT_SKIP_PF
#define SERT_SKIP_PF 1
#endif
constexpr bool kSkipPrefetchAdam = SERT_SKIP_PF != 0;
#ifndef SERT_SKIP_WAVES
#define SERT_SKIP_WAVES(CPL) 1
#endif
struct SkipArgs {
    float* pred;
    unsigned stride;
    int npred;
    float a_fut[kLazyK];
};

template <int LPR>
__device__ __forceinline__ float lane_group_sum(float v, int lane) {
    v = row16_sum(v);
    const float lo = read_lane(v, 0) + read_lane(v, 16), hi = read_lane(v, 32) + read_lane(v, 48);
    if (LPR == 64) return lo + hi;
    return lane < 32 ? lo : hi;
}

template <bool ADAM, int LPR, int CPL>
__global__ __launch_bounds__(256, SERT_SKIP_WAVES(CPL)) void dense_update_skip(float* __restrict__ p, const float* __restrict__ g,
                                                         float* __restrict__ s0, float* __restrict__ s1, unsigned nrows,
                                                         AdamArgs a, AdadeltaArgs da, float* __restrict__ sumsq_partial,
                                                         const uint32_t* __restrict__ bits, unsigned row_len, const LazyArgs lz,
                                                         const SkipArgs sk) {
    constexpr int GPB = 256 / LPR;
    constexpr bool kSkipPrefetch = kSkipPrefetchAdam && ADAM;
    __shared__ float red[GPB];
    const int lane = threadIdx.x & 63, l = threadIdx.x & (LPR - 1), grp = threadIdx.x / LPR;
    const float omb1 = 1.0f - a.b1, omb2 = 1.0f - a.b2, omr = 1.0f - da.rho;
    const unsigned d4 = row_len >> 2;
    const unsigned per = (nrows + gridDim.x - 1) / gridDim.x;
    const unsigned lo = blockIdx.x * per;
    const unsigned hi = lo + per < nrows ? lo + per : nrows;
    const int slot_now = (lz.t_prev + 1) % kLazyK;
    typedef float nt_f4 __attribute__((ext_vector_type(4)));
    float4* p4 = reinterpret_cast<float4*>(p);
    const float4* g4 = reinterpret_cast<const float4*>(g);
    float acc = 0.f;
    const unsigned cnt = hi > lo + grp ? (hi - lo - grp + GPB - 1) / GPB : 0u;
    const unsigned cnt_w = (unsigned)__builtin_amdgcn_readfirstlane((int)cnt);
    for (unsigned j0 = 0; j0 < cnt_w; j0 += LPR) {
        const unsigned jm = j0 + l;
        const unsigned row_m = lo + grp + jm * GPB;
        int flags_m = 0, last_m = lz.t_prev;
        float pred_m = 0.f;
        if (jm < cnt) {
            last_m = lz.last_in ? lz.last_in[row_m] : lz.t_prev;
            const bool hit_m = row_bit(bits, row_m);
            const bool need_m = hit_m || lz.write_all || (lz.next_bits && row_bit(lz.next_bits, row_m));
            lz.last_out[row_m] = need_m ? lz.t_prev + 1 : last_m;
            if (!need_m) pred_m = sk.pred[(size_t)slot_now * sk.stride + row_m];
            flags_m = 1 | (hit_m ? 2 : 0) | (need_m ? 4 : 0);
        }
        const unsigned trips = cnt_w - j0 < (unsigned)LPR ? cnt_w - j0 : (unsigned)LPR;
        struct RowRegs { float4 p[CPL], m[CPL], v[CPL], g[CPL]; };
        auto fetch = [&](unsigned jj, RowRegs& r) {
            const int flags = __shfl(flags_m, (int)jj, LPR);
            const bool hit = flags & 2, proc = (flags & 5) == 5;
            const unsigned row = lo + grp + (j0 + jj) * GPB;
#pragma unroll
            for (int c = 0; c < CPL; ++c) {
                r.p[c] = r.m[c] = r.v[c] = r.g[c] = make_float4(0.f, 0.f, 0.f, 0.f);
                if (proc && (unsigned)(l + c * LPR) < d4) {
                    const size_t i = (size_t)row * d4 + l + c * LPR;
                    r.p[c] = p4[i];
                    const nt_f4 mr = __builtin_nontemporal_load(reinterpret_cast<const nt_f4*>(s0) + i);
                    const nt_f4 vr = __builtin_nontemporal_load(reinterpret_cast<const nt_f4*>(s1) + i);
                    r.m[c] = make_float4(mr.x, mr.y, mr.z, mr.w);
                    r.v[c] = make_float4(vr.x, vr.y, vr.z, vr.w);
                    if (hit) r.g[c] = g4[i];
                }
            }
        };
        RowRegs nxt;
        if (kSkipPrefetch && trips > 0) fetch(0, nxt);
        for (unsigned jj = 0; jj < trips; ++jj) {
            const int flags = __shfl(flags_m, (int)jj, LPR);
            const int last = __shfl(last_m, (int)jj, LPR);
            const float predv = __shfl(pred_m, (int)jj, LPR);
            const bool valid = flags & 1, proc = (flags & 5) == 5;
            RowRegs cur;
            if (kSkipPrefetch) {
                cur = nxt;
                if (jj + 1 < trips) fetch(jj + 1, nxt);
            }
            if (!__any(proc)) {
                if (valid) acc += predv;
                continue;
            }
            if (!kSkipPrefetch) fetch(jj, cur);
            const unsigned row = lo + grp + (j0 + jj) * GPB;
            const int lag = proc ? lz.t_prev - last : 0;
            bool on[CPL];
#pragma unroll
            for (int c = 0; c < CPL; ++c) on[c] = proc && (unsigned)(l + c * LPR) < d4;
            float4 (&pp)[CPL] = cur.p;
            float4 (&mm)[CPL] = cur.m;
            float4 (&vv)[CPL] = cur.v;
            auto advance = [&](float at, float& s) {
                float sn = 0.f;
#pragma unroll
                for (int c = 0; c < CPL; ++c) {
                    if (!on[c]) continue;
                    float z0 = 0.f, z1 = 0.f, z2 = 0.f, z3 = 0.f;
                    if (ADAM) {
                        AdamArgs ak = a;
                        ak.a_t = at;
                        adam_elem(pp[c].x, z0, mm[c].x, vv[c].x, ak, omb1, omb2, s, sn);
                        adam_elem(pp[c].y, z1, mm[c].y, vv[c].y, ak, omb1, omb2, s, sn);
                        adam_elem(pp[c].z, z2, mm[c].z, vv[c].z, ak, omb1, omb2, s, sn);
                        adam_elem(pp[c].w, z3, mm[c].w, vv[c].w, ak, omb1, omb2, s, sn);
                    } else {
                        adadelta_elem(pp[c].x, z0, mm[c].x, vv[c].x, da, omr, s);
                        adadelta_elem(pp[c].y, z1, mm[c].y, vv[c].y, da, omr, s);
                        adadelta_elem(pp[c].z, z2, mm[c].z, vv[c].z, da, omr, s);
                        adadelta_elem(pp[c].w, z3, mm[c].w, vv[c].w, da, omr, s);
                    }
                }
            };
            for (int k = kLazyK; k >= 1; --k) {
                if (k <= lag) { float sd = 0.f; advance(lazy_step_size(lz, k), sd); }
            }
            float s = 0.f;
            {
                float sn = 0.f;
#pragma unroll
                for (int c = 0; c < CPL; ++c) {
                    if (!on[c]) continue;
                    const size_t i = (size_t)row * d4 + l + c * LPR;
                    float4 gg = cur.g[c];
                    if (ADAM) {
                        AdamArgs ak = a;
                        ak.a_t = lz.a_of[0];
                        adam_elem(pp[c].x, gg.x, mm[c].x, vv[c].x, ak, omb1, omb2, s, sn);
                        adam_elem(pp[c].y, gg.y, mm[c].y, vv[c].y, ak, omb1, omb2, s, sn);
                        adam_elem(pp[c].z, gg.z, mm[c].z, vv[c].z, ak, omb1, omb2, s, sn);
                        adam_elem(pp[c].w, gg.w, mm[c].w, vv[c].w, ak, omb1, omb2, s, sn);
                    } else {
                        adadelta_elem(pp[c].x, gg.x, mm[c].x, vv[c].x, da, omr, s);
                        adadelta_elem(pp[c].y, gg.y, mm[c].y, vv[c].y, da, omr, s);
                        adadelta_elem(pp[c].z, gg.z, mm[c].z, vv[c].z, da, omr, s);
                        adadelta_elem(pp[c].w, gg.w, mm[c].w, vv[c].w, da, omr, s);
                    }
                    p4[i] = pp[c];
                    { nt_f4 t; t.x = mm[c].x; t.y = mm[c].y; t.z = mm[c].z; t.w = mm[c].w; __builtin_nontemporal_store(t, reinterpret_cast<nt_f4*>(s0) + i); }
                    { nt_f4 t; t.x = vv[c].x; t.y = vv[c].y; t.z = vv[c].z; t.w = vv[c].w; __builtin_nontemporal_store(t, reinterpret_cast<nt_f4*>(s1) + i); }
                }
            }
            const float rowsum = lane_group_sum<LPR>(s, lane);
            if (valid) acc += proc ? rowsum : predv;
            for (int q = 1; q <= sk.npred; ++q) {
                float s2 = 0.f;
                if (q < sk.npred) {
                    advance(sk.a_fut[q - 1], s2);
                } else {
#pragma unroll
                    for (int c = 0; c < CPL; ++c) {
                        if (!on[c]) continue;
                        s2 = sq_acc(s2, pp[c].x); s2 = sq_acc(s2, pp[c].y); s2 = sq_acc(s2, pp[c].z); s2 = sq_acc(s2, pp[c].w);
                    }
                }
                const float r = lane_group_sum<LPR>(s2, lane);
                if (proc && l == 0) sk.pred[(size_t)((lz.t_prev + 1 + q) % kLazyK) * sk.stride + row] = r;
            }
        }
    }
    if (l == 0) red[grp] = acc;
    __syncthreads();
    if (threadIdx.x == 0) {
        float t = red[0];
#pragma unroll
        for (int i = 1; i < GPB; ++i) t += red[i];
        sumsq_partial[blockIdx.x] = t;
    }
}

struct SmallTensors {
    float* p[3];
    float* g[3];
    float* s0[3];
    float* s1[3];
    unsigned long long count[3];
    int first_block[4];
    float l2k[3];
    const float* gparts[3];
    int ngroups[3];
    unsigned long long gstride[3];
};

template <bool ADAM, bool STORE_G>
__global__ __launch_bounds__(256) void optimizer_small(SmallTensors t, AdamArgs aa, AdadeltaArgs da,
                                                       float* __restrict__ sumsq_partial,
                                                       float* __restrict__ sumsq_new_partial = nullptr) {
    __shared__ float red[4];
    int i = 0;
    if ((int)blockIdx.x >= t.first_block[1]) i = 1;
    if ((int)blockIdx.x >= t.first_block[2]) i = 2;
    const int nb = t.first_block[i + 1] - t.first_block[i];
    const int b = blockIdx.x - t.first_block[i];
    float *p = t.p[i], *g = t.g[i], *s0 = t.s0[i], *s1 = t.s1[i];
    const size_t count = (size_t)t.count[i];
    aa.l2k = t.l2k[i];
    da.l2k = t.l2k[i];
    const float omb1 = 1.0f - aa.b1, omb2 = 1.0f - aa.b2, omr = 1.0f - da.rho;
    float ss = 0.f, ssn = 0.f;
    const float* parts = t.gparts[i];
    const int ngroups = t.ngroups[i];
    const size_t gstride = (size_t)t.gstride[i];
    for (size_t k = (size_t)b * 256 + threadIdx.x; k < count; k += (size_t)nb * 256) {
        float pp = p[k], a0 = s0[k], a1 = s1[k];
        float gg;
        if (parts) {
            gg = parts[k];
            for (int q = 1; q < ngroups; ++q) gg += parts[(size_t)q * gstride + k];
            if (!STORE_G) g[k] = gg;
        } else {
            gg = g[k];
        }
        if (ADAM) adam_elem(pp, gg, a0, a1, aa, omb1, omb2, ss, ssn);
        else { adadelta_elem(pp, gg, a0, a1, da, omr, ss); ssn = sq_acc(ssn, pp); }
        p[k] = pp; s0[k] = a0; s1[k] = a1;
        if (STORE_G) g[k] = gg;
    }
    const float tot = block_sum_256(ss, red);
    if (threadIdx.x == 0) sumsq_partial[blockIdx.x] = (t.l2k[i] != 0.f) ? tot : 0.f;
    if (sumsq_new_partial) {
        __syncthreads();
        const float tn = block_sum_256(ssn, red);
        if (threadIdx.x == 0) sumsq_new_partial[blockIdx.x] = (t.l2k[i] != 0.f) ? tn : 0.f;
    }
}

__global__ __launch_bounds__(256) void sumsq_like_small(const float* __restrict__ p, size_t count, float l2k,
                                                        float* __restrict__ partial) {
    __shared__ float red[4];
    float ss = 0.f;
    for (size_t k = (size_t)blockIdx.x * 256 + threadIdx.x; k < count; k += (size_t)gridDim.x * 256) ss = sq_acc(ss, p[k]);
    const float tot = block_sum_256(ss, red);
    if (threadIdx.x == 0) partial[blockIdx.x] = (l2k != 0.f) ? tot : 0.f;
}

__global__ __launch_bounds__(256) void sum_partial(const float* __restrict__ in, size_t count,
                                                   float* __restrict__ partial) {
    __shared__ float red[4];
    float s = 0.f;
    for (size_t i = blockIdx.x * (size_t)blockDim.x + threadIdx.x; i < count;
         i += (size_t)gridDim.x * blockDim.x)
        s += in[i];
    const float tot = block_sum_256(s, red);
    if (threadIdx.x == 0) partial[blockIdx.x] = tot;
}

__global__ __launch_bounds__(256) void sumsq_pieces(const float* __restrict__ p, size_t sc, size_t slab,
                                                    int nch, float* __restrict__ partial) {
    __shared__ float red[4];
    float ss = 0.f;
    const size_t sc4 = sc >> 2, total4 = sc4 * (size_t)nch;
    for (size_t j = blockIdx.x * (size_t)blockDim.x + threadIdx.x; j < total4; j += (size_t)gridDim.x * blockDim.x) {
        const size_t c = j / sc4, o = j - c * sc4;
        const float4 v = reinterpret_cast<const float4*>(p + c * slab)[o];
        ss += (v.x * v.x + v.y * v.y) + (v.z * v.z + v.w * v.w);
    }
    const float tot = block_sum_256(ss, red);
    if (threadIdx.x == 0) partial[blockIdx.x] = tot;
}

__global__ __launch_bounds__(256) void partials_to_scalar(const float* __restrict__ partials, int n,
                                                          float* __restrict__ out) {
    __shared__ double red[256];
    double a = 0.0;
    for (int i = threadIdx.x; i < n; i += 256) a += (double)partials[i];
    red[threadIdx.x] = a;
    __syncthreads();
    for (int s = 128; s > 0; s >>= 1) {
        if (threadIdx.x < s) red[threadIdx.x] += red[threadIdx.x + s];
        __syncthreads();
    }
    if (threadIdx.x == 0) out[0] = (float)red[0];
}

__global__ __launch_bounds__(256) void finalize_loss(const float* __restrict__ loss_partials,
                                                     int n_loss,
                                                     const float* __restrict__ sq_partials,
                                                     int n_sq, float inv_batch, float reg_scale,
                                                     float* __restrict__ out,
                                                     unsigned* __restrict__ host_flag = nullptr,
                                                     unsigned seq = 0,
                                                     const float* __restrict__ extra_sq = nullptr) {
    __shared__ double red[2][4];
    auto strided_sum = [](const float* __restrict__ x, int n) {
        double acc = 0.0;
        for (int i0 = threadIdx.x; i0 < n; i0 += 8 * 256) {
            float v[8];
#pragma unroll
            for (int q = 0; q < 8; ++q) v[q] = (i0 + q * 256 < n) ? x[i0 + q * 256] : 0.f;
#pragma unroll
            for (int q = 0; q < 8; ++q) acc += (double)v[q];
        }
        return acc;
    };
    double a = strided_sum(loss_partials, n_loss);
    double b = strided_sum(sq_partials, n_sq);
#pragma unroll
    for (int off = 32; off > 0; off >>= 1) {
        a += __shfl_xor(a, off);
        b += __shfl_xor(b, off);
    }
    if ((threadIdx.x & 63) == 0) { red[0][threadIdx.x >> 6] = a; red[1][threadIdx.x >> 6] = b; }
    __syncthreads();
    const double loss_sum = (red[0][0] + red[0][1]) + (red[0][2] + red[0][3]);
    const double sq_sum = (red[1][0] + red[1][1]) + (red[1][2] + red[1][3]);
    if (threadIdx.x == 0) {
        const float data = (float)loss_sum * inv_batch;
        const float reg = reg_scale * (float)(sq_sum + (extra_sq ? (double)extra_sq[0] : 0.0));
        out[0] = data + reg;
        out[1] = data;
        out[2] = reg;
        if (host_flag) __hip_atomic_store(host_flag, seq, __ATOMIC_RELEASE, __HIP_MEMORY_SCOPE_SYSTEM);
    }
}

struct TailArgs {
    const float* part;
    int splits;
    unsigned long long stride;
    float *W, *b, *s0_w, *s1_w, *s0_b, *s1_b, *g_w, *g_b;
    unsigned n_w, n_b;
// ... 133 lines not shown
```

### sert_amd/csrc/kernels_seg.h

```cpp
#pragma once
#include "common.h"
#include "word_index.h"

namespace sert {

struct DenseSlots {
    int n;
    int slot[kHeavyMax];
};
struct XcdLists {
    int on;
    int off[8];
    int cnt[8];
    int slot_is_row;
};

template <int LPI, bool DST_SLOT, bool LL_FINAL, bool SKIP_DENSE>
__device__ __forceinline__ void segsum_rows_body(const int bx_, const int by_, const int gy_,
                                                   const float* __restrict__ src,
                                                   const int32_t* __restrict__ rows,
                                                   const int4* __restrict__ items, int nitems,
                                                   float* __restrict__ final_dst,
                                                   float* __restrict__ partial_dst, int d,
                                                   float divisor,
// ... 387 lines not shown
                    x0.x += o0.x; x0.y += o0.y; x0.z += o0.z; x0.w += o0.w;
                    x1.x += o1.x; x1.y += o1.y; x1.z += o1.z; x1.w += o1.w;
                }
                slot[h * 128 + lane] = x0;
                slot[h * 128 + 64 + lane] = x1;
            }
        }
        __syncthreads();
    }
    for (int k = threadIdx.x; k < kHeavyMax * 128; k += 512) {
        const int h = k >> 7, cl = k & 127;
        const int ch = slab * 128 + cl;
        if (ch >= d4) continue;
        const float4 p0 = hv_lds[k], p1 = hv_lds[kHeavyMax * 128 + k];
        reinterpret_cast<float4*>(part)[((size_t)rblk * kHeavyMax + h) * d4 + ch] =
            make_float4(p0.x + p1.x, p0.y + p1.y, p0.z + p1.z, p0.w + p1.w);
    }
}

__global__ __launch_bounds__(256) void segsum_heavy_combine(const float* __restrict__ part, int nblocks, int d,
                                                            const int32_t* __restrict__ words, int nheavy,
                                                            float* __restrict__ final_dst, float divisor) {
    __shared__ float4 hc_lds[8][32];
    const int h = blockIdx.x;
    if (h >= nheavy) return;
    const int d4 = d >> 2;
    const int l = threadIdx.x & 31, g = threadIdx.x >> 5;
    const int ch = blockIdx.y * 32 + l;
    const float4* p4 = reinterpret_cast<const float4*>(part);
    float4 a = make_float4(0.f, 0.f, 0.f, 0.f);
    if (ch < d4) {
#pragma unroll 8
        for (int b = g; b < nblocks; b += 8) {
            const float4 v = p4[((size_t)b * kHeavyMax + h) * d4 + ch];
            a.x += v.x; a.y += v.y; a.z += v.z; a.w += v.w;
        }
    }
    hc_lds[g][l] = a;
    __syncthreads();
    if (g == 0 && ch < d4) {
        a = hc_lds[0][l];
#pragma unroll
        for (int q = 1; q < 8; ++q) { const float4 v = hc_lds[q][l]; a.x += v.x; a.y += v.y; a.z += v.z; a.w += v.w; }
        a.x /= divisor; a.y /= divisor; a.z /= divisor; a.w /= divisor;
        reinterpret_cast<float4*>(final_dst)[(size_t)words[h] * d4 + ch] = a;
    }
}

constexpr int kHeavyRowsFusedMin = 64, kHeavyRowsFusedMax = 256;
inline int heavy_rows_fused(int B) {
    int r = kHeavyRowsFusedMin;
    while (r < kHeavyRowsFusedMax && B / (2 * r) >= 256) r *= 2;
    return r;
}
struct PlusJob {
    int kind;
    int extra;
    const float* src;
    const uint4* cnt16;
    float* part;
    const int32_t* words;
    int nheavy;
    int nblocks;
    int B;
    int slot_is_row;
    int rpb;
};

__device__ __forceinline__ void heavy_rows_body(const int rblk, const int slab, const PlusJob& job, int d, float4 (*lds)[8][32]) {
    const int l = threadIdx.x & 31, wv = threadIdx.x >> 6, half = wv >> 1;
    const int rs = (wv & 1) * 2 + ((threadIdx.x >> 5) & 1);
    const int d4 = d >> 2, ch = slab * 32 + l;
    const bool on = ch < d4;
    typedef float f32x2 __attribute__((ext_vector_type(2)));
    f32x2 acc2[8][2];
#pragma unroll
    for (int h = 0; h < 8; ++h) { acc2[h][0] = (f32x2)(0.f); acc2[h][1] = (f32x2)(0.f); }
    const int row0 = rblk * job.rpb + rs;
    const uint2* cnt8 = reinterpret_cast<const uint2*>(job.cnt16) + half;
#pragma unroll 1
    for (int t = 0; t < job.rpb / 16; ++t) {
        uint2 c[4];
        float4 v[4];
#pragma unroll
        for (int q = 0; q < 4; ++q) {
            const int r = row0 + (t * 4 + q) * 4;
            const int i = min(r, job.B - 1);
            c[q] = cnt8[2 * (size_t)i];
            if (r >= job.B) c[q] = make_uint2(0u, 0u);
            v[q] = on ? *reinterpret_cast<const float4*>(job.src + (size_t)i * d + 4 * ch) : make_float4(0.f, 0.f, 0.f, 0.f);
        }
#pragma unroll
        for (int q = 0; q < 4; ++q) {
            const unsigned cw[2] = {c[q].x, c[q].y};
            f32x2 lo, hi;
            lo.x = v[q].x; lo.y = v[q].y; hi.x = v[q].z; hi.y = v[q].w;
#pragma unroll
            for (int h = 0; h < 8; ++h) {
                const f32x2 ff = (f32x2)((float)((cw[h >> 2] >> (8 * (h & 3))) & 0xffu));
                acc2[h][0] = __builtin_elementwise_fma(ff, lo, acc2[h][0]);
                acc2[h][1] = __builtin_elementwise_fma(ff, hi, acc2[h][1]);
            }
        }
    }
    float4 acc[8];
#pragma unroll
    for (int h = 0; h < 8; ++h) {
        acc[h] = make_float4(acc2[h][0].x, acc2[h][0].y, acc2[h][1].x, acc2[h][1].y);
        acc[h].x += __shfl_xor(acc[h].x, 32); acc[h].y += __shfl_xor(acc[h].y, 32);
        acc[h].z += __shfl_xor(acc[h].z, 32); acc[h].w += __shfl_xor(acc[h].w, 32);
    }
    if ((wv & 1) && (threadIdx.x & 63) < 32) {
#pragma unroll
        for (int h = 0; h < 8; ++h) lds[half][h][l] = acc[h];
    }
    __syncthreads();
    if (!(wv & 1) && (threadIdx.x & 63) < 32 && on) {
#pragma unroll
        for (int h = 0; h < 8; ++h) {
            const float4 o = lds[half][h][l];
            float4 a = acc[h];
            a.x += o.x; a.y += o.y; a.z += o.z; a.w += o.w;
            reinterpret_cast<float4*>(job.part)[((size_t)rblk * kHeavyMax + half * 8 + h) * d4 + ch] = a;
        }
    }
}

__device__ __forceinline__ void heavy_combine_body(const int h, const int slab, const PlusJob& job, int d, float* __restrict__ final_dst,
                                                   float divisor, float4 (*lds)[32]) {
    if (h >= job.nheavy) return;
    const int d4 = d >> 2;
    const int l = threadIdx.x & 31, g = threadIdx.x >> 5;
    const int ch = slab * 32 + l;
    const float4* p4 = reinterpret_cast<const float4*>(job.src);
    float4 a = make_float4(0.f, 0.f, 0.f, 0.f);
    if (ch < d4) {
#pragma unroll 8
        for (int b = g; b < job.nblocks; b += 8) {
            const float4 v = p4[((size_t)b * kHeavyMax + h) * d4 + ch];
            a.x += v.x; a.y += v.y; a.z += v.z; a.w += v.w;
        }
    }
    lds[g][l] = a;
    __syncthreads();
    if (g == 0 && ch < d4) {
        a = lds[0][l];
#pragma unroll
        for (int q = 1; q < 8; ++q) { const float4 v = lds[q][l]; a.x += v.x; a.y += v.y; a.z += v.z; a.w += v.w; }
        a.x /= divisor; a.y /= divisor; a.z /= divisor; a.w /= divisor;
        reinterpret_cast<float4*>(final_dst)[(size_t)job.words[h] * d4 + ch] = a;
    }
}

__global__ __launch_bounds__(256) void segsum_rows_plus(const float* __restrict__ src, const int32_t* __restrict__ rows,
                                                        const int4* __restrict__ items, int nitems, float* __restrict__ final_dst,
                                                        float* __restrict__ partial_dst, int d, float divisor, const PlusJob job) {
    __shared__ float4 plus_lds[2][8][32];
    if ((int)blockIdx.x < job.extra) {
        if (job.kind == 1) heavy_rows_body((int)blockIdx.x, (int)blockIdx.y, job, d, plus_lds);
        else heavy_combine_body((int)blockIdx.x, (int)blockIdx.y, job, d, final_dst, divisor, plus_lds[0]);
        return;
    }
    XcdLists xl = XcdLists();
    xl.slot_is_row = job.slot_is_row;
    segsum_rows_body<32, false, false, false>((int)blockIdx.x - job.extra, (int)blockIdx.y, (int)gridDim.y, src, rows, items, nitems,
                                              final_dst, partial_dst, d, divisor, nullptr, 1, nullptr, nullptr, DenseSlots(), xl);
}

struct PlusJobLL {
    PlusJob j;
    DenseSlots dense;
    const float* logp;
    const float* rsum;
};

__device__ __forceinline__ void heavy_rows_body64(const int rblk, const int slab, const PlusJob& job, int d, float4 (*lds)[8][64]) {
    const int lane = threadIdx.x & 63, wv = threadIdx.x >> 6, half = wv >> 1, rs = wv & 1;
    const int d4 = d >> 2, ch = slab * 64 + lane;
    const bool on = ch < d4;
    typedef float f32x2 __attribute__((ext_vector_type(2)));
    f32x2 acc2[8][2];
#pragma unroll
    for (int h = 0; h < 8; ++h) { acc2[h][0] = (f32x2)(0.f); acc2[h][1] = (f32x2)(0.f); }
    const int row0 = rblk * job.rpb + rs;
    const uint2* cnt8 = reinterpret_cast<const uint2*>(job.cnt16) + half;
#pragma unroll 1
    for (int t = 0; t < job.rpb / 8; ++t) {
        uint2 c[4];
        float4 v[4];
#pragma unroll
        for (int q = 0; q < 4; ++q) {
            const int r = row0 + (t * 4 + q) * 2;
            const int i = __builtin_amdgcn_readfirstlane(min(r, job.B - 1));
            c[q] = cnt8[2 * (size_t)i];
            if (r >= job.B) c[q] = make_uint2(0u, 0u);
            v[q] = on ? *reinterpret_cast<const float4*>(job.src + (size_t)i * d + 4 * ch) : make_float4(0.f, 0.f, 0.f, 0.f);
        }
#pragma unroll
        for (int q = 0; q < 4; ++q) {
            const unsigned cw[2] = {(unsigned)__builtin_amdgcn_readfirstlane((int)c[q].x), (unsigned)__builtin_amdgcn_readfirstlane((int)c[q].y)};
            f32x2 lo, hi;
            lo.x = v[q].x; lo.y = v[q].y; hi.x = v[q].z; hi.y = v[q].w;
#pragma unroll
            for (int h = 0; h < 8; ++h) {
                const unsigned byte = (cw[h >> 2] >> (8 * (h & 3))) & 0xffu;
                if (byte != 0u) {
                    const f32x2 ff = (f32x2)((float)byte);
                    acc2[h][0] = __builtin_elementwise_fma(ff, lo, acc2[h][0]);
                    acc2[h][1] = __builtin_elementwise_fma(ff, hi, acc2[h][1]);
                }
            }
        }
    }
    if (rs) {
#pragma unroll
        for (int h = 0; h < 8; ++h) lds[half][h][lane] = make_float4(acc2[h][0].x, acc2[h][0].y, acc2[h][1].x, acc2[h][1].y);
    }
    __syncthreads();
    if (!rs && on) {
#pragma unroll
        for (int h = 0; h < 8; ++h) {
            const float4 o = lds[half][h][lane];
            reinterpret_cast<float4*>(job.part)[((size_t)rblk * kHeavyMax + half * 8 + h) * d4 + ch] =
                make_float4(acc2[h][0].x + o.x, acc2[h][0].y + o.y, acc2[h][1].x + o.z, acc2[h][1].y + o.w);
        }
    }
}

__device__ __forceinline__ void heavy_combine_ll_body64(const int h, const int slab, const PlusJobLL& job, int d,
                                                        float* __restrict__ final_dst, float4 (*lds)[64]) {
    if (h >= job.j.nheavy) return;
    const int d4 = d >> 2;
    const int lane = threadIdx.x & 63, wv = threadIdx.x >> 6;
    const int ch = slab * 64 + lane;
    const float4* p4 = reinterpret_cast<const float4*>(job.j.src);
    float4 a = make_float4(0.f, 0.f, 0.f, 0.f);
    if (ch < d4) {
#pragma unroll 8
        for (int b = wv; b < job.j.nblocks; b += 4) {
            const float4 v = p4[((size_t)b * kHeavyMax + h) * d4 + ch];
            a.x += v.x; a.y += v.y; a.z += v.z; a.w += v.w;
        }
    }
    lds[wv][lane] = a;
    __syncthreads();
    if (wv == 0 && ch < d4) {
        a = lds[0][lane];
#pragma unroll
        for (int q = 1; q < 4; ++q) { const float4 v = lds[q][lane]; a.x += v.x; a.y += v.y; a.z += v.z; a.w += v.w; }
        const int slot = job.dense.slot[h];
        const float rs = job.rsum[slot];
        const float LOGLO = logf(SERT_CLIP_LO), LOGHI = logf(SERT_CLIP_HI);
        const size_t o = (size_t)slot * d + 4 * ch;
        const float4 lp = *reinterpret_cast<const float4*>(job.logp + o);
        a.x = ((lp.x >= LOGLO && lp.x <= LOGHI) ? a.x : 0.f) - __expf(lp.x) * rs;
        a.y = ((lp.y >= LOGLO && lp.y <= LOGHI) ? a.y : 0.f) - __expf(lp.y) * rs;
        a.z = ((lp.z >= LOGLO && lp.z <= LOGHI) ? a.z : 0.f) - __expf(lp.z) * rs;
        a.w = ((lp.w >= LOGLO && lp.w <= LOGHI) ? a.w : 0.f) - __expf(lp.w) * rs;
        *reinterpret_cast<float4*>(final_dst + o) = a;
    }
}

__global__ __launch_bounds__(256) void segsum_rows_plus_ll(const float* __restrict__ src, const int32_t* __restrict__ rows,
                                                           const int4* __restrict__ items, int nitems, float* __restrict__ final_dst,
                                                           float* __restrict__ partial_dst, int d, const DenseSlots dense,
                                                           const PlusJobLL job) {
    __shared__ float4 plus_lds[2][8][64];
    if ((int)blockIdx.x < job.j.extra) {
        if (job.j.kind == 1) heavy_rows_body64((int)blockIdx.x, (int)blockIdx.y, job.j, d, plus_lds);
        else heavy_combine_ll_body64((int)blockIdx.x, (int)blockIdx.y, job, d, final_dst, plus_lds[0]);
        return;
    }
    segsum_rows_body<64, true, true, true>((int)blockIdx.x - job.j.extra, (int)blockIdx.y, (int)gridDim.y, src, rows, items, nitems,
                                           final_dst, partial_dst, d, 1.0f, nullptr, 1, job.logp, job.rsum, dense, XcdLists());
}

__global__ __launch_bounds__(256) void segsum_heavy_combine_ll(const float* __restrict__ part, int nblocks, int d,
                                                               const DenseSlots dense, float* __restrict__ final_dst,
                                                               const float* __restrict__ logp, const float* __restrict__ rsum) {
    __shared__ float4 hc_lds[8][32];
    const int h = blockIdx.x;
    if (h >= dense.n) return;
    const int d4 = d >> 2;
    const int l = threadIdx.x & 31, g = threadIdx.x >> 5;
    const int ch = blockIdx.y * 32 + l;
    const float4* p4 = reinterpret_cast<const float4*>(part);
    float4 a = make_float4(0.f, 0.f, 0.f, 0.f);
    if (ch < d4) {
#pragma unroll 8
        for (int b = g; b < nblocks; b += 8) {
            const float4 v = p4[((size_t)b * kHeavyMax + h) * d4 + ch];
            a.x += v.x; a.y += v.y; a.z += v.z; a.w += v.w;
        }
    }
    hc_lds[g][l] = a;
    __syncthreads();
    const int slot = dense.slot[h];
    const float rs = rsum[slot];
    const float LOGLO = logf(SERT_CLIP_LO), LOGHI = logf(SERT_CLIP_HI);
    if (g == 0 && ch < d4) {
        a = hc_lds[0][l];
#pragma unroll
        for (int q = 1; q < 8; ++q) { const float4 v = hc_lds[q][l]; a.x += v.x; a.y += v.y; a.z += v.z; a.w += v.w; }
        const size_t o = (size_t)slot * d + 4 * ch;
        const float4 lp = *reinterpret_cast<const float4*>(logp + o);
        a.x = ((lp.x >= LOGLO && lp.x <= LOGHI) ? a.x : 0.f) - __expf(lp.x) * rs;
        a.y = ((lp.y >= LOGLO && lp.y <= LOGHI) ? a.y : 0.f) - __expf(lp.y) * rs;
        a.z = ((lp.z >= LOGLO && lp.z <= LOGHI) ? a.z : 0.f) - __expf(lp.z) * rs;
        a.w = ((lp.w >= LOGLO && lp.w <= LOGHI) ? a.w : 0.f) - __expf(lp.w) * rs;
        *reinterpret_cast<float4*>(final_dst + o) = a;
    }
}

}
```

### sert_amd/csrc/model.h

```cpp
#pragma once
#include <vector>
#include <string>
#include "common.h"
#include "word_index.h"
#include "kernels_xchg.h"
#include "kernels_opt.h"
#include "../../include/sert_hip.h"
#include "../../include/sert_hip_debug.h"

namespace sert {

struct DataSplit {
    int64_t N = 0;
    void* x = nullptr;
    int32_t* y = nullptr;
    int64_t* csr_indptr = nullptr;
    int32_t* csr_indices = nullptr;
    float* csr_data = nullptr;
    int64_t nnz = 0;
    int64_t max_labels_per_row = 0;
    float* w = nullptr;
    float* labfix = nullptr;
    int32_t* idx_rows = nullptr;
    int4* idx_items = nullptr;
    int4* idx_heavy = nullptr;
    int32_t* idx_bundles = nullptr;
    int32_t* idx_uwords = nullptr;
    int32_t* idx_slots = nullptr;
    int32_t* idx_rows_div = nullptr;
    uint32_t* idx_touched_bits = nullptr;
    uint4* idx_dense_counts = nullptr;
    int32_t* idx_dense_words = nullptr;
    uint8_t* idx_tok_slot = nullptr;
    std::vector<int32_t> dense_cnt_of;
    int64_t bit_words = 0;
    std::vector<BatchIndex> idx_batches;
};

enum TimingGroup {
    TG_GATHER = 0,
    TG_GEMM_FWD,
    TG_LOSS,
    TG_SORT,
    TG_EGRAD,
    TG_EFIX,
    TG_GEMM_DW,
    TG_SPLITK,
    TG_GEMM_DX,
    TG_SCATTER,
    TG_ALLREDUCE,
    TG_REDUCE_SCATTER,
    TG_ALLGATHER,
    TG_OPT_WORD,
    TG_OPTIMIZER,
    TG_FINALIZE,
    TG_COUNT
};

struct Timing {
    bool enabled = false;
    hipEvent_t ev[TG_COUNT][2] = {};
    bool created = false;
    bool used[TG_COUNT] = {};
    double total_us[TG_COUNT] = {};
    int64_t samples[TG_COUNT] = {};
};

struct InStep {
    static constexpr int kRing = 1024;
    bool on = false;
    bool created = false;
    hipEvent_t ev[kRing][2] = {};
    int group[kRing] = {};
    int64_t head = 0, tail = 0;
    int cur_group = -1;
    double total_us[TG_COUNT] = {};
    int64_t launches[TG_COUNT] = {};
    int64_t steps = 0;
};

}

struct sert_model {
    sert_config cfg;
    hipStream_t stream = nullptr;
    hipStream_t stream2 = nullptr;
    hipEvent_t ev_fork = nullptr, ev_join = nullptr, ev_join3 = nullptr;
    hipStream_t stream3 = nullptr;
    hipEvent_t ev_step_done = nullptr, ev_neg = nullptr, ev_opt_fork = nullptr, ev_small = nullptr;
    hipEvent_t ev_loss = nullptr;
    hipEvent_t ev_dense = nullptr;
    bool step_done_pending = false;
    bool re_in_parts = false;
    bool fork_bound = false;
    bool egrad_ranges = false;
    bool egrad_force_sort = false;
    bool events_device_scope = false;
    bool lazy_join = false;
    int num_cus = 256;
    bool proj_fused = false;
    bool ll_dw_side = false;
    bool dw_side_first = false;
    bool dp_late_join = false;
    bool side_heavy = false;
    hipEvent_t ev_re = nullptr;
    bool re_pending = false;
    float* re_sq = nullptr;
    int64_t re_sq_for[2] = {-1, -1};
    int n_loss_partials = 0;
    bool loss_from_rows = false;
    int nce_loss_partials = 0;
    int nstreams = 2;
    int64_t hint_next = -1;
    bool neg_side_ready = false;
    bool sort_early = false;
    bool bucket_early = false;
    int32_t* rw_last[2] = {nullptr, nullptr};
    int rw_last_cur = 0;
    bool rw_stale = false;
    int64_t rw_ready_batch = -1;
    int64_t lazy_next = -1;
    float cur_touched_frac = 1.f;
    float* rw_pred = nullptr;
    unsigned rw_pred_stride = 0;
    bool rw_pred_ok = false;
    int64_t rw_pred_T = 0;
    bool lazy_skip = true;
    float lazy_max = 0.5f;
    int64_t upd_counts[10] = {0, 0, 0, 0, 0, 0, 0, 0, 0, 0};
    int64_t projected_batch = -1;
    int64_t spec_fb_batch = -1;
    int64_t spec_fb_step = -1;
    unsigned loss_seq = 0;
    float* h_loss_dev = nullptr;

    size_t n_rw = 0, n_re = 0, n_w = 0, n_b = 0;

    float *rw = nullptr, *re = nullptr, *W = nullptr, *b = nullptr;
    float *s0_rw = nullptr, *s0_re = nullptr, *s0_w = nullptr, *s0_b = nullptr;
    float *s1_rw = nullptr, *s1_re = nullptr, *s1_w = nullptr, *s1_b = nullptr;

    float* gflat = nullptr;
    size_t gflat_count = 0;
    float *g_re = nullptr, *g_rw = nullptr, *g_w = nullptr, *g_b = nullptr, *g_loss = nullptr;
    size_t gflat_alloc = 0;
    int32_t *run_start = nullptr, *run_end = nullptr;

    float *H = nullptr, *T = nullptr, *DA = nullptr, *DH = nullptr, *rowloss = nullptr;
    float* T_alt = nullptr;
    float* DH2 = nullptr;
    int fs_tile = 0;
    int32_t* neg = nullptr;
    int32_t* neg_alt = nullptr;
    int64_t neg_alt_step = -1;
    int64_t* neg_stage = nullptr;
    int32_t *cand = nullptr, *cand_sorted = nullptr, *pair_sorted = nullptr;
    int32_t* cand_early = nullptr;
    float* coef = nullptr;
    float *ehead = nullptr, *etail = nullptr;
    float* epart = nullptr;
    int32_t *eg_entries = nullptr, *eg_offs = nullptr;
    int eg_sub_rows = 0, eg_num_sub = 0, eg_subs_per_group = 0, eg_groups = 0, eg_ranges = 0, eg_er_shift = 0;
    int32_t *sort_hist = nullptr, *sort_bin_total = nullptr;
    int32_t *sort_k_tmp = nullptr, *sort_v_tmp = nullptr;
    int sort_bits = 1;
    float *G = nullptr;
    float *Z = nullptr;
    float *J = nullptr;
    float *DG = nullptr;

    float* wpart = nullptr;
    float* hpart = nullptr;
    size_t wpart_rows = 0;
    float* part = nullptr;
    size_t part_count = 0;
    float2* ll_tokstat = nullptr; float* ll_lse = nullptr; float2* ll_jstat = nullptr;
    float4* ll_rowinfo = nullptr; float* ll_rpart = nullptr; float* ll_r = nullptr;
    bool use_touched = false;

    float* Zu = nullptr;
    float* dZu = nullptr;
    size_t zu_rows = 0;
    float* zpart = nullptr;
    size_t zpart_rows = 0;
    bool ll_dedup = false;
    float* ll_rsum = nullptr;
    int ll_U = 0;
    float* skbuf = nullptr;
    size_t skbuf_count = 0;
    unsigned long long* tail_blk = nullptr;
    unsigned tail_launch_seq = 0;
    int tail_splits = 0;
    size_t tail_stride = 0;
    bool tail_defer = false;
    bool tail_pending = false;
    sert::TailArgs tail_args;
    int tail_nb = 0;
    int64_t tail_counts[2] = {0, 0};
    float* red_loss = nullptr;
    float* red_sq = nullptr;
    float* d_loss = nullptr;
    float* h_loss = nullptr;
    float* d_losses = nullptr;
    int64_t d_losses_cap = 0;

    float *pred_a = nullptr, *pred_b = nullptr;
    void* pred_ids = nullptr;
    size_t pred_a_cap = 0, pred_b_cap = 0, pred_ids_cap = 0;

    sert::DataSplit split[2];

    int64_t step = 0;
    int64_t eval_draws = 0;

    size_t pt_pad[4] = {0, 0, 0, 0};
    size_t pt_sc[4] = {0, 0, 0, 0};
    bool pt_big[4] = {false, false, false, false};
    bool pt_sharded[4] = {false, false, false, false};
    size_t ar_split = 0;
    size_t rest_off = 0;
    float* g_sq = nullptr;
    float* sq_scratch = nullptr;

    int rank = 0, world = 1;
    void* comm = nullptr;
    bool comm_dead = false;
    sert_alltoall_fn host_ar = nullptr;
    void* host_ar_user = nullptr;
    float *host_send = nullptr, *host_recv = nullptr;
    size_t host_send_cap = 0, host_recv_cap = 0;

    bool xr_mode = false;
    bool xr_on = false;
    int64_t xr_rows_per_rank = 0;
    sert::RowExchangeLists* xr = nullptr;
    int32_t *xr_serve = nullptr, *xr_fetch = nullptr, *xr_union = nullptr, *xr_ent = nullptr, *xr_ptr = nullptr;
    uint32_t* xr_ubits = nullptr;
    float *xr_send = nullptr, *xr_recv = nullptr;
    bool rw_full = true;
    int64_t xr_fetched_batch = -1;
    int64_t xr_batch = -1;
    hipEvent_t ev_params_ready = nullptr, ev_word_updated = nullptr;
    double comm_bytes_moved = 0.0;
    int64_t comm_steps = 0;
    hipStream_t comm_stream = nullptr;
    hipEvent_t ev_rest_ready = nullptr, ev_ar_done = nullptr;
    static constexpr int kMaxArChunks = 16;
    int ar_chunks = 1;
    hipEvent_t ev_grad_ready[4] = {};
    hipEvent_t ev_rs_done[4][kMaxArChunks] = {};
    hipEvent_t ev_opt_done[4][kMaxArChunks] = {};
    hipEvent_t ev_ag_done = nullptr;
    bool rs_issued[4] = {false, false, false, false};
    hipStream_t sq_stream = nullptr;

    sert::Timing timing;
    sert::InStep instep;
};

struct sert_scorer {
    int device = 0;
    hipStream_t stream = nullptr;
    int64_t V = 0;
    int dim = 0;
    float* E = nullptr;
    float* P = nullptr;
    float* S = nullptr;
    hipStream_t stream2 = nullptr;
    hipEvent_t ev_ready = nullptr, ev_done = nullptr;
    float* val = nullptr;
    int32_t* idx = nullptr;
    int64_t cap_q = 0, cap_qk = 0, cap_s = 0;
    float* Ss = nullptr; float* thr = nullptr;
    unsigned long long* cand = nullptr; unsigned char* cnt = nullptr;
    int* nflag = nullptr; int* flag_list = nullptr;
    float* Pc = nullptr; int32_t* idx_c = nullptr; float* val_c = nullptr;
    int64_t cap_ss = 0, cap_ft = 0, cap_cand = 0, cap_flag = 0, cap_c = 0, cap_ck = 0;
    bool bf16 = false, bf16_demoted = false;
    int kp = 0;
    uint16_t* E16 = nullptr; uint16_t* P16 = nullptr;
    int64_t cap_p16 = 0;
};
// ... 1 lines not shown
```

Baseline: 305.2 million pairs/s.

## Run untouched-row lazy Adam work early inside the segment-sum kernel

Adds an early word-table update path. Extra blocks in the fused segsum_rows_plus launch handle the rows that need a lazy Adam catch-up but are not touched by the current batch, and write their predicted squared-norm contributions. This overlaps optimizer work with the backward gradient reduction and leaves less for the later dense_update_skip pass. It adds planning state shared across stages (WordUpdatePlan), a template split of the skip kernel, and more complex correctness coupling between the two launches.

```diff
diff --git a/include/sert_hip_debug.h b/include/sert_hip_debug.h
--- a/include/sert_hip_debug.h
+++ b/include/sert_hip_debug.h
@@ -10,6 +10,8 @@
 int sert_debug_update_counts(sert_model* m, int64_t* out, int n);
 
 int sert_debug_tail_counts(sert_model* m, int64_t* out, int n);
+
+int sert_debug_early_counts(sert_model* m, int64_t* out, int n);
 
 int sert_debug_poison_scratch(sert_model* m);
 
diff --git a/sert_amd/_capi.py b/sert_amd/_capi.py
--- a/sert_amd/_capi.py
+++ b/sert_amd/_capi.py
@@ -32,7 +32,7 @@
     'sert_comm_unique_id', 'sert_comm_init', 'sert_comm_init_host', 'sert_comm_destroy', 'sert_comm_stats',
     'sert_synchronize', 'sert_timing_enable', 'sert_timing_reset', 'sert_timing_count',
     'sert_timing_name', 'sert_timing_avg_us', 'sert_timing_launches', 'sert_bench_gemm', 'sert_debug_gemm', 'sert_debug_gemm_splitk', 'sert_debug_gemm_longk', 'sert_bench_memory', 'sert_debug_row_lists', 'sert_debug_word_index_sum',
-    'sert_debug_update_counts', 'sert_debug_tail_counts', 'sert_debug_poison_scratch', 'sert_debug_ll_rank_distributions', 'sert_debug_reval_chunks',
+    'sert_debug_update_counts', 'sert_debug_tail_counts', 'sert_debug_early_counts', 'sert_debug_poison_scratch', 'sert_debug_ll_rank_distributions', 'sert_debug_reval_chunks',
     'sert_profile_range_push', 'sert_profile_range_pop',
 ]
 
@@ -373,6 +373,12 @@
         check(self._lib.sert_debug_tail_counts(self._h, v, 2))
         return {'alone': int(v[0]), 'in_gather': int(v[1])}
 
+    def early_counts(self):
+        v = (ctypes.c_int64 * 2)()
+        self._lib.sert_debug_early_counts.argtypes = [ctypes.c_void_p, ctypes.POINTER(ctypes.c_int64), ctypes.c_int]
+        check(self._lib.sert_debug_early_counts(self._h, v, 2))
+        return {'sparse': int(v[0]), 'full': int(v[1])}
+
     def timings(self):
         n = self._lib.sert_timing_count(self._h)
         return {self._lib.sert_timing_name(self._h, i).decode():
diff --git a/sert_amd/csrc/host/api_data_train.inc b/sert_amd/csrc/host/api_data_train.inc
--- a/sert_amd/csrc/host/api_data_train.inc
+++ b/sert_amd/csrc/host/api_data_train.inc
@@ -186,7 +186,10 @@
         const DataSplit& ds = m->split[SERT_SPLIT_TRAIN];
         if (will_run_ahead(m, hint)) {
             bool fused = false;
-            SERT_TRY(step_forward_backward(m, ds, hint, nullptr, &fused));
+            m->in_run_ahead = true;
+            const int rc_fb = step_forward_backward(m, ds, hint, nullptr, &fused);
+            m->in_run_ahead = false;
+            if (rc_fb != 0) return rc_fb;
             m->spec_fb_batch = hint;
             m->spec_fb_step = m->step;
             return 0;
diff --git a/sert_amd/csrc/host/api_debug.inc b/sert_amd/csrc/host/api_debug.inc
--- a/sert_amd/csrc/host/api_debug.inc
+++ b/sert_amd/csrc/host/api_debug.inc
@@ -23,6 +23,12 @@
 int sert_debug_tail_counts(sert_model* m, int64_t* out, int n) {
     if (!m || !out || n < 1 || n > 2) SERT_FAIL("bad argument");
     for (int i = 0; i < n; ++i) out[i] = m->tail_counts[i];
+    return 0;
+}
+
+int sert_debug_early_counts(sert_model* m, int64_t* out, int n) {
+    if (!m || !out || n < 1 || n > 2) SERT_FAIL("bad argument");
+    for (int i = 0; i < n; ++i) out[i] = m->early_counts[i];
     return 0;
 }
 
diff --git a/sert_amd/csrc/host/api_model.inc b/sert_amd/csrc/host/api_model.inc
--- a/sert_amd/csrc/host/api_model.inc
+++ b/sert_amd/csrc/host/api_model.inc
@@ -181,6 +181,7 @@
     }
     m->proj_fused = variant_knob("SERT_PROJ_FUSED") && atoi(variant_knob("SERT_PROJ_FUSED")) != 0;
     m->lazy_skip = !(knob("SERT_LAZY_SKIP") && atoi(knob("SERT_LAZY_SKIP")) == 0);
+    m->early_update = !(knob("SERT_EARLY_UPDATE") && atoi(knob("SERT_EARLY_UPDATE")) == 0);
     m->lazy_max = knob("SERT_LAZY_MAX") ? (float)atof(knob("SERT_LAZY_MAX")) : 0.5f;
     {
         int cus = 0;
diff --git a/sert_amd/csrc/host/lazy_segsum.inc b/sert_amd/csrc/host/lazy_segsum.inc
--- a/sert_amd/csrc/host/lazy_segsum.inc
+++ b/sert_amd/csrc/host/lazy_segsum.inc
@@ -15,6 +15,80 @@
     }
     return lz;
 }
+static bool lazy_word_update_applies(const sert_model* m, const uint32_t* tf, const uint32_t* next_bits, float touched_frac) {
+    const auto& c = m->cfg;
+    const float lazy_max = (next_bits && m->lazy_skip) ? m->lazy_max : std::min(m->lazy_max, 0.35f);
+    static const bool lazy_small = variant_knob("SERT_LAZY_SMALL_TABLES") != nullptr;
+    return tf && m->rw_last[0] && !c.keep_grads && c.word_dim % 4 == 0 && touched_frac <= lazy_max &&
+           (m->n_rw >= ((size_t)1 << 22) || lazy_small);
+}
+
+static WordUpdatePlan plan_lazy_word_update(sert_model* m, int64_t u, const uint32_t* next_bits) {
+    WordUpdatePlan pl = WordUpdatePlan();
+    pl.valid = true;
+    pl.u = u;
+    pl.lz = lazy_args(m, u - 1, 1);
+    pl.lz.next_bits = next_bits;
+    pl.lz.write_all = (next_bits == nullptr || u % kLazyK == 0) ? 1 : 0;
+    const unsigned d4 = (unsigned)m->cfg.word_dim / 4;
+    pl.skip = m->lazy_skip && m->rw_pred && d4 <= 256;
+    if (!pl.skip) return pl;
+    pl.sparse = next_bits && m->rw_pred_ok && u < m->rw_pred_T;
+    pl.lz.write_all = pl.sparse ? 0 : 1;
+    if (!pl.sparse) m->rw_pred_T = u + kLazyK;
+    pl.sk.pred = m->rw_pred;
+    pl.sk.stride = m->rw_pred_stride;
+    pl.sk.npred = next_bits ? (int)(m->rw_pred_T - 1 - u) : 0;
+    pl.sk.early = 0;
+    for (int j = 0; j < kLazyK; ++j) {
+        AdamArgs a2; AdadeltaArgs d2;
+        optimizer_args(m, u + 1 + j, &a2, &d2);
+        pl.sk.a_fut[j] = a2.a_t;
+    }
+    m->rw_pred_ok = next_bits != nullptr;
+    return pl;
+}
+
+static inline bool is_dp(const sert_model* m);
+static bool plan_early_word_update(sert_model* m, const DataSplit& ds, int64_t batch_index, EarlyJob* ej) {
+    const auto& c = m->cfg;
+    m->wu_plan.valid = false;
+    if (!m->early_update || m->in_run_ahead || is_dp(m) || !is_vs(m) || !m->pt_big[0] || m->n_rw == 0) return false;
+    if (!m->use_touched || !ds.idx_touched_bits || (size_t)batch_index >= ds.idx_batches.size()) return false;
+    const unsigned d4 = (unsigned)c.word_dim / 4;
+    if (!(m->lazy_skip && m->rw_pred) || c.word_dim % 4 != 0) return false;
+    const bool form_32x3 = d4 > 64 && d4 <= 96 && m->n_rw < ((size_t)1 << 26);
+#ifdef SERT_VARIANTS
+    if (variant_knob("SERT_SKIP_32X3") || variant_knob("SERT_SKIP_BLOCKS")) return false;
+#endif
+    if (!(d4 <= 32 || form_32x3)) return false;
+    const int B = c.batch_size;
+    const uint32_t* tf = ds.idx_touched_bits + (size_t)batch_index * ds.bit_words;
+    const uint32_t* next_bits = nullptr;
+    if (m->lazy_next >= 0 && (m->lazy_next + 1) * (int64_t)B <= ds.N) next_bits = ds.idx_touched_bits + (size_t)m->lazy_next * ds.bit_words;
+    const float frac = (float)ds.idx_batches[(size_t)batch_index].num_distinct / (float)c.vocab_size;
+    if (!lazy_word_update_applies(m, tf, next_bits, frac)) return false;
+    const int64_t u = m->step + 1;
+    m->wu_plan = plan_lazy_word_update(m, u, next_bits);
+    if (!m->wu_plan.skip) return false;
+    m->wu_plan.sk.early = 1;
+    AdamArgs aa; AdadeltaArgs da;
+    optimizer_args(m, u, &aa, &da);
+    static const int blocks_knob = variant_knob("SERT_EARLY_BLOCKS") ? atoi(variant_knob("SERT_EARLY_BLOCKS")) : 0;
+    static const int behind_knob = variant_knob("SERT_EARLY_BEHIND") ? atoi(variant_knob("SERT_EARLY_BEHIND")) : 0;
+    const unsigned nrows = (unsigned)c.vocab_size;
+    *ej = EarlyJob();
+    ej->nblk = std::max(1, std::min<int>(blocks_knob > 0 ? std::min(blocks_knob, 4 * kOptBlocks) : kEarlyBlocks, (int)cdiv(nrows, 8u)));
+    ej->behind = behind_knob != 0;
+    ej->p = m->rw; ej->s0 = m->s0_rw; ej->s1 = m->s1_rw;
+    ej->nrows = nrows; ej->row_len = (unsigned)c.word_dim;
+    ej->bits = tf;
+    ej->a = aa;
+    ej->lz = m->wu_plan.lz;
+    ej->sk = m->wu_plan.sk;
+    return true;
+}
+
 static int ensure_rw_current(sert_model* m, int64_t batch, int64_t t_applied) {
     if (!m->rw_stale) return 0;
     if (batch >= 0 && batch == m->rw_ready_batch) return 0;
@@ -95,6 +169,17 @@
                              bx.nlevels == 3 && bx.item_cnt[1] > 0;
     bool heavy_fused = false, heavy_combined = false;
     PlusJob hjob = PlusJob();
+    EarlyJob ej = EarlyJob();
+    bool early = false;
+    {
+        const int d4 = d / 4;
+        const bool lpi32 = d % 4 == 0 && (d4 <= 32 || (d4 > 64 && 64 * cdiv(d4, 64) > 32 * cdiv(d4, 32)));
+        const bool bundled = bx.bundle_cnt > 0 && ds.idx_bundles;
+        static const bool no_fuse = variant_knob("SERT_HEAVY_NO_FUSE") != nullptr;
+        if (src == m->DH && lpi32 && !no_fuse && bx.nlevels >= 1 && bx.item_cnt[0] > 0 && bx.row_groups == 1 && !bundled)
+            early = plan_early_word_update(m, ds, batch_index, &ej);
+        else m->wu_plan.valid = false;
+    }
     if (bx.dense_cnt > 0 && is_vs(m) && d % 4 == 0) {
         const int B = m->cfg.batch_size, d4 = d / 4;
         static const bool no_fuse = variant_knob("SERT_HEAVY_NO_FUSE") != nullptr;
@@ -130,11 +215,22 @@
         const int32_t* rows = (l == 0) ? ds.idx_rows + bx.rows_off : nullptr;
         const int4* items = ds.idx_items + bx.item_off[l];
         float* pout = m->wpart + (size_t)bx.part_off[l] * d;
+        if (l == 0 && early) {
+            PlusJob j = heavy_fused ? hjob : PlusJob();
+            j.slot_is_row = bx.slot_is_row ? 1 : 0;
+            const dim3 grid(j.extra + ej.nblk + cdiv(nitems, 8), cdiv(d / 4, 32));
+            if (d / 4 <= 32)
+                hipLaunchKernelGGL((segsum_rows_plus<1>), grid, dim3(256), 0, m->stream, in, rows, items, nitems, m->g_rw, pout, d, divisor, j, ej);
+            else
+                hipLaunchKernelGGL((segsum_rows_plus<3>), grid, dim3(256), 0, m->stream, in, rows, items, nitems, m->g_rw, pout, d, divisor, j, ej);
+            ++m->early_counts[m->wu_plan.sparse ? 0 : 1];
+            continue;
+        }
         if (heavy_fused && l <= 1) {
             PlusJob j = l == 0 ? hjob : heavy_combine_job();
             j.slot_is_row = (l == 0 && bx.slot_is_row) ? 1 : 0;
-            hipLaunchKernelGGL(segsum_rows_plus, dim3(j.extra + cdiv(nitems, 8), cdiv(d / 4, 32)), dim3(256), 0, m->stream, in, rows, items,
-                               nitems, m->g_rw, pout, d, divisor, j);
+            hipLaunchKernelGGL((segsum_rows_plus<0>), dim3(j.extra + cdiv(nitems, 8), cdiv(d / 4, 32)), dim3(256), 0, m->stream, in, rows, items,
+                               nitems, m->g_rw, pout, d, divisor, j, EarlyJob());
             if (l == 1) heavy_combined = true;
             continue;
         }
@@ -173,8 +269,8 @@
     }
     if (heavy_fused && !heavy_combined) {
         const PlusJob j = heavy_combine_job();
-        hipLaunchKernelGGL(segsum_rows_plus, dim3(j.extra, cdiv(d / 4, 32)), dim3(256), 0, m->stream, (const float*)nullptr,
-                           (const int32_t*)nullptr, (const int4*)nullptr, 0, m->g_rw, (float*)nullptr, d, divisor, j);
+        hipLaunchKernelGGL((segsum_rows_plus<0>), dim3(j.extra, cdiv(d / 4, 32)), dim3(256), 0, m->stream, (const float*)nullptr,
+                           (const int32_t*)nullptr, (const int4*)nullptr, 0, m->g_rw, (float*)nullptr, d, divisor, j, EarlyJob());
     }
     return 0;
 }
diff --git a/sert_amd/csrc/host/optimizer_and_loss.inc b/sert_amd/csrc/host/optimizer_and_loss.inc
--- a/sert_amd/csrc/host/optimizer_and_loss.inc
+++ b/sert_amd/csrc/host/optimizer_and_loss.inc
@@ -42,26 +42,14 @@
 static int launch_lazy_word_update(sert_model* m, const ParamTensor& t, const uint32_t* tf, const uint32_t* next_bits, const int nb,
                                    const AdamArgs& aa, const AdadeltaArgs& da, float* sq) {
     const auto& c = m->cfg;
-    LazyArgs lz = lazy_args(m, m->step - 1, 1);
+    const WordUpdatePlan pl = (m->wu_plan.valid && m->wu_plan.u == m->step) ? m->wu_plan : plan_lazy_word_update(m, m->step, next_bits);
+    m->wu_plan.valid = false;
+    const LazyArgs lz = pl.lz;
     int nb_skip = 0;
-    lz.next_bits = next_bits;
-    lz.write_all = (next_bits == nullptr || m->step % kLazyK == 0) ? 1 : 0;
     const unsigned d4 = (unsigned)c.word_dim / 4;
-    if (m->lazy_skip && m->rw_pred && d4 <= 256) {
-        const int64_t u = m->step;
-        const bool sparse = next_bits && m->rw_pred_ok && u < m->rw_pred_T;
-        lz.write_all = sparse ? 0 : 1;
-        if (!sparse) m->rw_pred_T = u + kLazyK;
-        SkipArgs sk;
-        sk.pred = m->rw_pred;
-        sk.stride = m->rw_pred_stride;
-        sk.npred = next_bits ? (int)(m->rw_pred_T - 1 - u) : 0;
-        for (int j = 0; j < kLazyK; ++j) {
-            AdamArgs a2; AdadeltaArgs d2;
-            optimizer_args(m, u + 1 + j, &a2, &d2);
-            sk.a_fut[j] = a2.a_t;
-        }
-        m->rw_pred_ok = next_bits != nullptr;
+    if (pl.skip) {
+        const bool sparse = pl.sparse;
+        const SkipArgs sk = pl.sk;
         const unsigned nrows = (unsigned)c.vocab_size;
         static const int skip_blocks_knob = variant_knob("SERT_SKIP_BLOCKS") ? atoi(variant_knob("SERT_SKIP_BLOCKS")) : 0;
         const int nb_dense = nb;
@@ -149,13 +137,11 @@
             const int64_t max_nb = t.n >= ((size_t)1 << 24) ? 2 * kOptBlocks : kOptBlocks;
             const int nb = (int)std::min<int64_t>(max_nb, cdiv(cdiv(t.n, 4), 256));
             const uint32_t* tf = (i == 0 && m->use_touched) ? bits : nullptr;
-            const float lazy_max = (next_bits && m->lazy_skip) ? m->lazy_max : std::min(m->lazy_max, 0.35f);
-            static const bool lazy_small = variant_knob("SERT_LAZY_SMALL_TABLES") != nullptr;
-            if (i == 0 && tf && m->rw_last[0] && !c.keep_grads && c.word_dim % 4 == 0 &&
-                m->cur_touched_frac <= lazy_max && (t.n >= ((size_t)1 << 22) || lazy_small)) {
+            if (i == 0 && lazy_word_update_applies(m, tf, next_bits, m->cur_touched_frac)) {
                 n_sq += launch_lazy_word_update(m, t, tf, next_bits, nb, aa, da, m->red_sq + n_sq);
                 continue;
             }
+            if (i == 0 && m->wu_plan.valid && m->wu_plan.u == m->step) SERT_FAIL("a planned lazy word-table update was not launched");
             if (i == 0) m->rw_pred_ok = false;
             if (i == 0) ++m->upd_counts[0];
             if (i == 0) SERT_TRY(ensure_rw_current(m, -1, m->step - 1));
diff --git a/sert_amd/csrc/kernels_opt.h b/sert_amd/csrc/kernels_opt.h
--- a/sert_amd/csrc/kernels_opt.h
+++ b/sert_amd/csrc/kernels_opt.h
@@ -320,6 +320,7 @@
     float* pred;
     unsigned stride;
     int npred;
+    int early;
     float a_fut[kLazyK];
 };
 
@@ -331,20 +332,19 @@
     return lane < 32 ? lo : hi;
 }
 
-template <bool ADAM, int LPR, int CPL>
-__global__ __launch_bounds__(256, SERT_SKIP_WAVES(CPL)) void dense_update_skip(float* __restrict__ p, const float* __restrict__ g,
-                                                         float* __restrict__ s0, float* __restrict__ s1, unsigned nrows,
-                                                         AdamArgs a, AdadeltaArgs da, float* __restrict__ sumsq_partial,
-                                                         const uint32_t* __restrict__ bits, unsigned row_len, const LazyArgs lz,
-                                                         const SkipArgs sk) {
+template <bool ADAM, int LPR, int CPL, bool EARLY, bool PF>
+__device__ __forceinline__ void skip_rows_body(const unsigned blk, const unsigned nblk, float* __restrict__ p, const float* __restrict__ g,
+                                               float* __restrict__ s0, float* __restrict__ s1, const unsigned nrows,
+                                               const AdamArgs& a, const AdadeltaArgs& da, float* __restrict__ sumsq_partial,
+                                               const uint32_t* __restrict__ bits, const unsigned row_len, const LazyArgs& lz,
+                                               const SkipArgs& sk, float* red) {
     constexpr int GPB = 256 / LPR;
-    constexpr bool kSkipPrefetch = kSkipPrefetchAdam && ADAM;
-    __shared__ float red[GPB];
+    constexpr bool kSkipPrefetch = PF;
     const int lane = threadIdx.x & 63, l = threadIdx.x & (LPR - 1), grp = threadIdx.x / LPR;
     const float omb1 = 1.0f - a.b1, omb2 = 1.0f - a.b2, omr = 1.0f - da.rho;
     const unsigned d4 = row_len >> 2;
-    const unsigned per = (nrows + gridDim.x - 1) / gridDim.x;
-    const unsigned lo = blockIdx.x * per;
+    const unsigned per = (nrows + nblk - 1) / nblk;
+    const unsigned lo = blk * per;
     const unsigned hi = lo + per < nrows ? lo + per : nrows;
     const int slot_now = (lz.t_prev + 1) % kLazyK;
     typedef float nt_f4 __attribute__((ext_vector_type(4)));
@@ -362,9 +362,14 @@
             last_m = lz.last_in ? lz.last_in[row_m] : lz.t_prev;
             const bool hit_m = row_bit(bits, row_m);
             const bool need_m = hit_m || lz.write_all || (lz.next_bits && row_bit(lz.next_bits, row_m));
-            lz.last_out[row_m] = need_m ? lz.t_prev + 1 : last_m;
-            if (!need_m) pred_m = sk.pred[(size_t)slot_now * sk.stride + row_m];
-            flags_m = 1 | (hit_m ? 2 : 0) | (need_m ? 4 : 0);
+            if (EARLY) {
+                flags_m = 1 | ((need_m && !hit_m) ? 4 : 0);
+            } else {
+                const bool proc_m = need_m && (hit_m || !sk.early);
+                lz.last_out[row_m] = need_m ? lz.t_prev + 1 : last_m;
+                if (!proc_m) pred_m = sk.pred[(size_t)slot_now * sk.stride + row_m];
+                flags_m = 1 | (hit_m ? 2 : 0) | (proc_m ? 4 : 0);
+            }
         }
         const unsigned trips = cnt_w - j0 < (unsigned)LPR ? cnt_w - j0 : (unsigned)LPR;
         struct RowRegs { float4 p[CPL], m[CPL], v[CPL], g[CPL]; };
@@ -399,7 +404,7 @@
                 if (jj + 1 < trips) fetch(jj + 1, nxt);
             }
             if (!__any(proc)) {
-                if (valid) acc += predv;
+                if (!EARLY && valid) acc += predv;
                 continue;
             }
             if (!kSkipPrefetch) fetch(jj, cur);
@@ -462,7 +467,9 @@
                 }
             }
             const float rowsum = lane_group_sum<LPR>(s, lane);
-            if (valid) acc += proc ? rowsum : predv;
+            if (EARLY) {
+                if (proc && l == 0) sk.pred[(size_t)slot_now * sk.stride + row] = rowsum;
+            } else if (valid) acc += proc ? rowsum : predv;
             for (int q = 1; q <= sk.npred; ++q) {
                 float s2 = 0.f;
                 if (q < sk.npred) {
@@ -479,14 +486,46 @@
             }
         }
     }
+    if (EARLY) return;
     if (l == 0) red[grp] = acc;
     __syncthreads();
     if (threadIdx.x == 0) {
         float t = red[0];
 #pragma unroll
         for (int i = 1; i < GPB; ++i) t += red[i];
-        sumsq_partial[blockIdx.x] = t;
-    }
+        sumsq_partial[blk] = t;
+    }
+}
+
+template <bool ADAM, int LPR, int CPL>
+__global__ __launch_bounds__(256, SERT_SKIP_WAVES(CPL)) void dense_update_skip(float* __restrict__ p, const float* __restrict__ g,
+                                                         float* __restrict__ s0, float* __restrict__ s1, unsigned nrows,
+                                                         AdamArgs a, AdadeltaArgs da, float* __restrict__ sumsq_partial,
+                                                         const uint32_t* __restrict__ bits, unsigned row_len, const LazyArgs lz,
+                                                         const SkipArgs sk) {
+    __shared__ float red[256 / LPR];
+    skip_rows_body<ADAM, LPR, CPL, false, kSkipPrefetchAdam && ADAM>(blockIdx.x, gridDim.x, p, g, s0, s1, nrows, a, da, sumsq_partial, bits,
+                                                                     row_len, lz, sk, red);
+}
+
+#ifndef SERT_EARLY_BLOCKS_DEFAULT
+#define SERT_EARLY_BLOCKS_DEFAULT 1024
+#endif
+constexpr int kEarlyBlocks = SERT_EARLY_BLOCKS_DEFAULT;
+struct EarlyJob {
+    int nblk;
+    int behind;
+    float *p, *s0, *s1;
+    unsigned nrows, row_len;
+    const uint32_t* bits;
+    AdamArgs a;
+    LazyArgs lz;
+    SkipArgs sk;
+};
+template <int CPL>
+__device__ __forceinline__ void early_rows_body(const unsigned blk, const EarlyJob& ej) {
+    skip_rows_body<true, 32, CPL, true, false>(blk, (unsigned)ej.nblk, ej.p, (const float*)nullptr, ej.s0, ej.s1, ej.nrows, ej.a,
+                                               AdadeltaArgs(), (float*)nullptr, ej.bits, ej.row_len, ej.lz, ej.sk, (float*)nullptr);
 }
 
 struct SmallTensors {
diff --git a/sert_amd/csrc/kernels_seg.h b/sert_amd/csrc/kernels_seg.h
--- a/sert_amd/csrc/kernels_seg.h
+++ b/sert_amd/csrc/kernels_seg.h
@@ -563,18 +563,30 @@
     }
 }
 
+template <int ECPL>
 __global__ __launch_bounds__(256) void segsum_rows_plus(const float* __restrict__ src, const int32_t* __restrict__ rows,
                                                         const int4* __restrict__ items, int nitems, float* __restrict__ final_dst,
-                                                        float* __restrict__ partial_dst, int d, float divisor, const PlusJob job) {
+                                                        float* __restrict__ partial_dst, int d, float divisor, const PlusJob job,
+                                                        const EarlyJob ej) {
     __shared__ float4 plus_lds[2][8][32];
     if ((int)blockIdx.x < job.extra) {
         if (job.kind == 1) heavy_rows_body((int)blockIdx.x, (int)blockIdx.y, job, d, plus_lds);
         else heavy_combine_body((int)blockIdx.x, (int)blockIdx.y, job, d, final_dst, divisor, plus_lds[0]);
         return;
     }
+    int tree_blk = (int)blockIdx.x - job.extra;
+    if constexpr (ECPL > 0) {
+        const int tree_nblk = (int)gridDim.x - job.extra - ej.nblk;
+        const int eblk = ej.behind ? tree_blk - tree_nblk : tree_blk;
+        if (eblk >= 0 && eblk < ej.nblk) {
+            if (blockIdx.y == 0) early_rows_body<ECPL>((unsigned)eblk, ej);
+            return;
+        }
+        if (!ej.behind) tree_blk -= ej.nblk;
+    }
     XcdLists xl = XcdLists();
     xl.slot_is_row = job.slot_is_row;
-    segsum_rows_body<32, false, false, false>((int)blockIdx.x - job.extra, (int)blockIdx.y, (int)gridDim.y, src, rows, items, nitems,
+    segsum_rows_body<32, false, false, false>(tree_blk, (int)blockIdx.y, (int)gridDim.y, src, rows, items, nitems,
                                               final_dst, partial_dst, d, divisor, nullptr, 1, nullptr, nullptr, DenseSlots(), xl);
 }
 
diff --git a/sert_amd/csrc/model.h b/sert_amd/csrc/model.h
--- a/sert_amd/csrc/model.h
+++ b/sert_amd/csrc/model.h
@@ -80,6 +80,15 @@
 };
 
 }
+
+struct WordUpdatePlan {
+    bool valid = false;
+    int64_t u = 0;
+    bool skip = false;
+    bool sparse = false;
+    sert::LazyArgs lz;
+    sert::SkipArgs sk;
+};
 
 struct sert_model {
     sert_config cfg;
@@ -128,6 +137,10 @@
     bool lazy_skip = true;
     float lazy_max = 0.5f;
     int64_t upd_counts[10] = {0, 0, 0, 0, 0, 0, 0, 0, 0, 0};
+    bool early_update = true;
+    bool in_run_ahead = false;
+    WordUpdatePlan wu_plan;
+    int64_t early_counts[2] = {0, 0};
     int64_t projected_batch = -1;
     int64_t spec_fb_batch = -1;
     int64_t spec_fb_step = -1;
```

Result: slower. 301.8 million pairs/s (-1.1%).
